# adthoms/dcora

Hardware: AMD Instinct MI355X
Metric: RBCD iterations/sec, sphere2500 5-agent split (higher is better)
Workload: dtype f64

## Files before the change

dcora_amd/__init__.py:

```python
import ctypes as C
import gzip
import os
import shutil
import tempfile

import numpy as np

from . import capi
from .capi import DcoraError, Dims, ROptParams, ROptResult, RbcdOptions, F, unF, check

__all__ = ["QuadraticProblem", "QuadraticOptimizer", "ROptParameters", "Dataset", "Csr", "RbcdSession", "RaRbcdSession", "DcoraError",
           "build_Q_pgo", "dual_certificate", "is_psd", "min_eig", "fast_verification", "manifold_project",
           "device_count"]


def device_count():
    return capi.lib().dcora_device_count()


class Csr:

    def __init__(self, n, rp, ci, v):
        self.n = int(n)
        self.rp = np.ascontiguousarray(rp, dtype=np.int32)
# ... 217 lines not shown
        nrm = C.c_double()
        check(capi.lib().dcora_problem_riegrad(self.h, F(Y), out.ctypes.data_as(C.c_void_p), C.byref(nrm)))
        return unF(out, self.r, self.k)

    def RieGradNorm(self, Y):
        nrm = C.c_double()
        check(capi.lib().dcora_problem_riegrad(self.h, F(Y), None, C.byref(nrm)))
        return nrm.value

    def HessVec(self, Y, V):
        out = self._out()
        check(capi.lib().dcora_problem_hessvec(self.h, F(Y), F(V), out))
        return unF(out, self.r, self.k)

    def HessVecSolverForm(self, Y, V):
        out = self._out()
        dots = np.zeros(2)
        check(capi.lib().dcora_debug_hessvec_solver_form(self.h, F(Y), F(V), out, dots))
        return unF(out, self.r, self.k), dots

    def PreCondition(self, Y, V):
        out = self._out()
        check(capi.lib().dcora_problem_precondition(self.h, F(Y), F(V), out))
        return unF(out, self.r, self.k)

    def Retract(self, Y, V):
        out = self._out()
        check(capi.lib().dcora_problem_retract(self.h, F(Y), F(V), out))
        return unF(out, self.r, self.k)

    def projectToTangentSpace(self, Y, V):
        out = self._out()
        check(capi.lib().dcora_problem_tangent_project(self.h, F(Y), F(V), out))
        return unF(out, self.r, self.k)

    def escapeSaddle(self, Xopt, theta, v, gradient_tolerance=1e-6, preconditioned_gradient_tolerance=1e-6,
                     isSecondOrder=False):
        out = self._out()
        ok = C.c_int()
        check(capi.lib().dcora_problem_escape_saddle(self.h, F(Xopt), float(theta),
                                                     np.ascontiguousarray(v, np.float64), gradient_tolerance,
                                                     preconditioned_gradient_tolerance, int(isSecondOrder), out,
                                                     C.byref(ok)))
        return (unF(out, self.r, self.k) if ok.value else None)

    def time_qapply(self, reps=100):
        ms, by = C.c_double(), C.c_double()
        check(capi.lib().dcora_problem_time_qapply(self.h, reps, C.byref(ms), C.byref(by)))
        return ms.value, by.value


def _time_precond(self, reps=100):
    ms, by = C.c_double(), C.c_double()
    check(capi.lib().dcora_problem_time_precond(self.h, reps, C.byref(ms), C.byref(by)))
    return ms.value, by.value


QuadraticProblem.time_precond = _time_precond


def _precond_info(self):
    info = np.zeros(5)
    check(capi.lib().dcora_problem_precond_info(self.h, info))
    return {"kind": {0: "none", 1: "dense", 2: "sparse"}[int(info[0])], "launches": int(info[1]),
            "nnzL": int(info[2]), "setup_ms": float(info[3]), "stored_doubles_per_apply": float(info[4])}


QuadraticProblem.precond_info = _precond_info


def _qapply_info(self):
    info = np.zeros(4)
    check(capi.lib().dcora_problem_qapply_info(self.h, info))
    return {"kernel": "k_spmm_bsrq" if info[0] else "k_spmm", "nnz": int(info[1]), "blocks": int(info[2]),
            "stored_matrix_bytes": float(info[3])}


QuadraticProblem.qapply_info = _qapply_info


def _solver_info(self):
    info = np.zeros(2)
    check(capi.lib().dcora_problem_solver_info(self.h, info))
    return {"tcg": {0: "three launches", 1: "two launches", 2: "one launch per run"}[int(info[0])]}


QuadraticProblem.solver_info = _solver_info


def time_qapply_rotating(problems, reps=60):
    arr = (C.c_void_p * len(problems))(*[getattr(p.h, 'value', p.h) for p in problems])
    ms = C.c_double()
    check(capi.lib().dcora_problem_time_qapply_rotating(arr, len(problems), reps, C.byref(ms)))
    return ms.value


def precond_cache_info():
    v = np.zeros(4)
    check(capi.lib().dcora_precond_cache_info(v))
    return {"hits": int(v[0]), "misses": int(v[1]), "entries": int(v[2]), "device_bytes": float(v[3])}


def precond_cache_clear():
    check(capi.lib().dcora_precond_cache_clear())


class QuadraticOptimizer:

    def __init__(self, problem, params=None):
        self.problem = problem
        self.params = params or ROptParameters()
        self.result = ROptResult()

    def optimize(self, Y):
        out = np.zeros(self.problem.r * self.problem.k)
        check(capi.lib().dcora_optimizer_optimize(self.problem.h, C.byref(self.params.c), F(Y), out,
                                                  C.byref(self.result)))
        return unF(out, self.problem.r, self.problem.k)

    def getOptResult(self):
        return self.result.as_dict()


def manifold_project(r, d, n, M, l=0, b=0, device=0, layout=0):
    dims = Dims(r, d, n, l, b, layout)
    k = (d + 1) * n + l + b
    out = np.zeros(r * k)
    check(capi.lib().dcora_manifold_project(C.byref(dims), F(M), out, device))
    return unF(out, r, k)


def dual_certificate(r, d, n, X, Q, l=0, b=0, device=0, layout=0):
    dims = Dims(r, d, n, l, b, layout)
    h = C.c_void_p()
    check(capi.lib().dcora_cert_dual_matrix(C.byref(dims), F(X), Q.rp, Q.ci, Q.v, device, C.byref(h)))
    return Csr(*capi.take_csr(h))


def is_psd(S, block=1):
    out = C.c_int()
    check(capi.lib().dcora_cert_is_psd(S.n, S.rp, S.ci, S.v, block, C.byref(out)))
    return bool(out.value)


def cert_prepare(Q, d, n, l=0, b=0, block=1, device=0, layout=0):
    dims = Dims(1, d, n, l, b, layout)
    check(capi.lib().dcora_cert_prepare(C.byref(dims), Q.rp, Q.ci, block, device))


def is_psd_device(S, block=1, device=0, info=False):
    out = C.c_int()
    i6 = np.zeros(8)
    check(capi.lib().dcora_cert_is_psd_device(S.n, S.rp, S.ci, S.v, block, device, C.byref(out), i6))
    if info:
        return bool(out.value), {"symbolic_ms": i6[0], "numeric_ms": i6[1], "arena_bytes": i6[2], "flops": i6[3],
                                 "levels": int(i6[4]), "launches": int(i6[5]), "logdet": i6[6],
                                 "lookup_ms": i6[7]}
    return bool(out.value)


def chol_host_selftest(S, block=1):
    out, res = C.c_int(), C.c_double()
    i4 = np.zeros(4)
    check(capi.lib().dcora_chol_host_selftest(S.n, S.rp, S.ci, S.v, block, C.byref(out), C.byref(res), i4))
    return bool(out.value), res.value, {"pieces": int(i4[0]), "levels": int(i4[1]), "arena": int(i4[2]),
                                        "flops": i4[3]}

# ... 383 lines not shown
```

dcora_amd/capi.py:

```python
import ctypes as C
import os
import subprocess

import numpy as np

_HERE = os.path.dirname(os.path.abspath(__file__))
LIB_PATH = os.path.join(_HERE, "lib", "libdcora_hip.so")
HEADER_PATH = os.path.join(os.path.dirname(_HERE), "include", "dcora_hip.h")


class DcoraError(RuntimeError):
    def __init__(self, status, msg):
        super().__init__("dcora status %d: %s" % (status, msg))
        self.status = status


class Dims(C.Structure):
    _fields_ = [("r", C.c_int), ("d", C.c_int), ("n", C.c_int), ("l", C.c_int), ("b", C.c_int), ("layout", C.c_int)]


LAYOUT_AUTO, LAYOUT_SE, LAYOUT_RA = 0, 1, 2


class ROptParams(C.Structure):
# ... 59 lines not shown
    "dcora_cert_dual_matrix": (C.c_int, [C.POINTER(Dims), _dp, _ip, _ip, _dp, C.c_int, C.POINTER(_vp)]),
    "dcora_cert_is_psd": (C.c_int, [C.c_int, _ip, _ip, _dp, C.c_int, _PI]),
    "dcora_cert_is_psd_device": (C.c_int, [C.c_int, _ip, _ip, _dp, C.c_int, C.c_int, _PI, _dp]),
    "dcora_chol_host_selftest": (C.c_int, [C.c_int, _ip, _ip, _dp, C.c_int, _PI, _PD, _dp]),
    "dcora_chol_cache_clear": (C.c_int, []),
    "dcora_cert_min_eig": (C.c_int, [C.c_int, _ip, _ip, _dp, C.c_int, C.c_double, C.c_int, C.c_ulonglong, C.c_int,
                                     _PD, _dp, C.POINTER(C.c_long)]),
    "dcora_cert_fast_verification": (C.c_int, [C.c_int, _ip, _ip, _dp, C.c_double, C.c_int, C.c_int, _PI, _PD, _dp,
                                               _PD]),
    "dcora_cert_lambda_min_certified": (C.c_int, [C.c_int, _ip, _ip, _dp, C.c_double, C.c_int, C.c_int, _PD, _PI]),
    "dcora_cert_suboptimality_gap": (C.c_int, [C.POINTER(Dims), _dp, C.c_double, _PD, _PD]),
    "dcora_dataset_load_g2o": (C.c_int, [C.c_char_p, C.POINTER(_vp)]),
    "dcora_dataset_create": (C.c_int, [C.c_int, C.c_int, C.c_int, _ip, _dp, C.POINTER(_vp)]),
    "dcora_dataset_info": (C.c_int, [_vp, _PI, _PI, _PI]),
    "dcora_dataset_copy": (C.c_int, [_vp, _ip, _dp]),
    "dcora_dataset_destroy": (C.c_int, [_vp]),
    "dcora_dataset_chordal_init": (C.c_int, [_vp, _dp]),
    "dcora_dataset_chordal_init_device": (C.c_int, [_vp, C.c_int, _dp]),
    "dcora_graph_build_Q_pgo": (C.c_int, [C.c_int, C.c_int, C.c_int, C.c_int, _ip, _dp, C.POINTER(_vp)]),
    "dcora_radataset_load_pyfg": (C.c_int, [C.c_char_p, C.POINTER(_vp)]),
    "dcora_radataset_info": (C.c_int, [_vp, _ip]),
    "dcora_radataset_create": (C.c_int, [C.c_int] * 5 + [_vp, _vp, C.c_int, _vp, _vp, C.c_int, _vp, _vp, _vp, C.POINTER(_vp)]),
    "dcora_radataset_copy": (C.c_int, [_vp] * 7),
    "dcora_radataset_ground_truth": (C.c_int, [_vp, _dp]),
    "dcora_radataset_build_Q": (C.c_int, [_vp, C.POINTER(_vp)]),
    "dcora_radataset_odometry_init": (C.c_int, [_vp, C.c_ulonglong, _dp]),
    "dcora_radataset_ownership": (C.c_int, [_vp, _vp, _vp, _vp]),
    "dcora_radataset_agent_columns": (C.c_int, [_vp, C.c_int, _ip, _vp, _PI]),
    "dcora_graph_extract_agent_blocks": (C.c_int, [C.c_int, _ip, _ip, _dp, C.c_int, _ip, C.POINTER(_vp),
                                                   C.POINTER(_vp)]),
    "dcora_radataset_destroy": (C.c_int, [_vp]),
    "dcora_graph_precond_regularization": (C.c_int, [C.c_int, _ip, _ip, _dp, C.c_int, _PD]),
    "dcora_rbcd_options_default": (None, [C.POINTER(RbcdOptions)]),
    "dcora_rbcd_create": (C.c_int, [_vp, C.POINTER(RbcdOptions), C.POINTER(_vp)]),
    "dcora_rbcd_destroy": (C.c_int, [_vp]),
    "dcora_rbcd_set_X": (C.c_int, [_vp, _dp]),
    "dcora_rbcd_get_X": (C.c_int, [_vp, _dp]),
    "dcora_rbcd_iterate": (C.c_int, [_vp, C.c_int, _PD, _PD, _vp, _PI]),
    "dcora_rbcd_run": (C.c_int, [_vp, C.c_int, C.c_double, _PI, _vp, _vp, _vp]),
    "dcora_rbcd_iterate_set": (C.c_int, [_vp, _ip, C.c_int, C.c_int]),
    "dcora_rbcd_set_acceleration": (C.c_int, [_vp, C.c_int]),
    "dcora_rbcd_agent_colours": (C.c_int, [_vp, _ip, _PI]),
    "dcora_rbcd_evaluate": (C.c_int, [_vp, _PD, _PD, _vp, _PI]),
    "dcora_rbcd_agent_iterate": (C.c_int, [_vp, C.c_int, C.c_int]),
    "dcora_rbcd_agent_get_X": (C.c_int, [_vp, C.c_int, _dp]),
    "dcora_rbcd_agent_set_X": (C.c_int, [_vp, C.c_int, _dp]),
    "dcora_rbcd_agent_update_neighbor": (C.c_int, [_vp, C.c_int, C.c_int, C.c_int, _ip, _dp, C.c_int]),
    "dcora_rbcd_agent_last_skipped": (C.c_int, [_vp, C.c_int, _PI]),
    "dcora_rbcd_agent_info": (C.c_int, [_vp, C.c_int, _PI, _PI, _PI]),
    "dcora_rbcd_last_result": (C.c_int, [_vp, C.POINTER(ROptResult)]),
    "dcora_rbcd_profile_tcg_runs": (C.c_int, [_vp, C.c_int]),
    "dcora_rbcd_profile_tcg_read": (C.c_int, [_vp, _dp]),
    "dcora_rbcd_X_device_ptr": (C.c_int, [_vp, C.POINTER(_vp)]),
    "dcora_rbcd_public_count": (C.c_int, [_vp, C.c_int, _PI]),
    "dcora_rbcd_public_indices": (C.c_int, [_vp, C.c_int, _ip]),
    "dcora_rbcd_pack_public_dev": (C.c_int, [_vp, C.c_int, _vp]),
    "dcora_rbcd_unpack_public_dev": (C.c_int, [_vp, C.c_int, _vp]),
    "dcora_rbcd_phase_nonselected": (C.c_int, [_vp, C.c_int]),
    "dcora_rbcd_phase_selected": (C.c_int, [_vp, C.c_int]),
    "dcora_rbcd_phase_evaluate_dev": (C.c_int, [_vp, _vp]),
    "dcora_rbcd_synchronize": (C.c_int, [_vp]),
    "dcora_exchange_create": (C.c_int, [_vp, C.c_char_p, C.POINTER(_vp)]),
    "dcora_exchange_destroy": (C.c_int, [_vp]),
    "dcora_exchange_create_ra": (C.c_int, [_vp, C.c_char_p, C.POINTER(_vp)]),
    "dcora_exchange_info": (C.c_int, [_vp, _dp]),
    "dcora_exchange_link_report": (C.c_int, [_vp, _dp]),
    "dcora_exchange_post": (C.c_int, [_vp, _ip, C.c_int]),
    "dcora_exchange_wait": (C.c_int, [_vp, _ip, C.c_int]),
    "dcora_exchange_evaluate": (C.c_int, [_vp, _PD, _PD, _vp, _PI]),
    "dcora_exchange_rbcd_iterate": (C.c_int, [_vp, C.c_int, _PD, _PD, _vp, _PI]),
    "dcora_exchange_rbcd_tick": (C.c_int, [_vp, _ip, C.c_int, C.c_int]),
    "dcora_exchange_set_X": (C.c_int, [_vp, _dp]),
    "dcora_exchange_gather_X": (C.c_int, [_vp, _dp]),
    "dcora_exchange_barrier": (C.c_int, [_vp]),
    "dcora_exchange_all_ready": (C.c_int, [_vp, C.c_int, _PI]),
    "dcora_exchange_certify": (C.c_int, [_vp, C.c_int, _vp, _vp, _vp, C.c_double, _PI, _PD, _PD, _dp,
                                         C.POINTER(C.c_longlong), _PI]),
    "dcora_exchange_host_selftest": (C.c_int, [C.c_char_p, C.c_int, C.c_int, C.c_int, C.c_int, _PD]),
    "dcora_debug_exchange_leave_stale": (C.c_int, [C.c_char_p, C.c_int, C.c_int]),
    "dcora_debug_exchange_probe_fault": (C.c_int, [C.c_int]),
    "dcora_cert_prepare": (C.c_int, [C.POINTER(Dims), _ip, _ip, C.c_int, C.c_int]),
    "dcora_debug_tcg_run_fault": (C.c_int, [C.c_int]),
    "dcora_debug_tcg_run_fault_at": (C.c_int, [C.c_int, C.c_int]),
    "dcora_problem_solver_info": (C.c_int, [_vp, _dp]),
    "dcora_ra_rbcd_create": (C.c_int, [_vp, C.POINTER(RbcdOptions), C.POINTER(_vp)]),
    "dcora_ra_rbcd_destroy": (C.c_int, [_vp]),
    "dcora_ra_rbcd_info": (C.c_int, [_vp, _PI, _vp]),
    "dcora_ra_rbcd_set_X": (C.c_int, [_vp, _dp]),
    "dcora_ra_rbcd_get_X": (C.c_int, [_vp, _dp]),
    "dcora_ra_rbcd_iterate": (C.c_int, [_vp, C.c_int, _PD, _PD, _vp, _PI]),
    "dcora_ra_rbcd_evaluate": (C.c_int, [_vp, _PD, _PD, _vp, _PI]),
    "dcora_ra_rbcd_run": (C.c_int, [_vp, C.c_int, C.c_double, _PI, _vp, _vp, _vp]),
    "dcora_ra_rbcd_last_result": (C.c_int, [_vp, C.POINTER(ROptResult)]),
    "dcora_problem_time_qapply": (C.c_int, [_vp, C.c_int, _PD, _PD]),
    "dcora_problem_time_qapply_rotating": (C.c_int, [C.POINTER(_vp), C.c_int, C.c_int, _PD]),
    "dcora_problem_qapply_info": (C.c_int, [_vp, _dp]),
    "dcora_problem_time_precond": (C.c_int, [_vp, C.c_int, _PD, _PD]),
    "dcora_problem_precond_info": (C.c_int, [_vp, _dp]),
    "dcora_precond_cache_info": (C.c_int, [_dp]),
    "dcora_precond_cache_clear": (C.c_int, []),
    "dcora_robust_params_default": (None, [C.POINTER(RobustParams)]),
    "dcora_robust_weights": (C.c_int, [C.POINTER(RobustParams), C.c_int, C.c_int, _dp, _dp]),
    "dcora_chi2inv": (C.c_int, [C.c_double, C.c_int, _PD]),
    "dcora_robust_error_threshold_at_quantile": (C.c_int, [C.c_double, C.c_int, _PD]),
    "dcora_robust_single_rotation_averaging": (C.c_int, [C.c_int, C.c_int, _dp, _vp, C.c_double, _dp, _ip]),
    "dcora_robust_single_pose_averaging": (C.c_int, [C.c_int, C.c_int, _dp, _dp, _vp, _vp, C.c_double, _dp, _dp, _ip]),
    "dcora_agent_neighbor_transforms": (C.c_int, [C.c_int, C.c_int, _ip, _dp, _dp, _dp, _dp, _dp]),
    "dcora_agent_robust_neighbor_transform": (C.c_int, [C.c_int, C.c_int, _dp, C.c_int, C.c_int, _dp, _PI, _PI]),
    "dcora_log_trajectory": (C.c_int, [C.c_char_p, C.c_int, C.c_int, _dp]),
    "dcora_fixed_stiefel_variable": (C.c_int, [C.c_int, C.c_int, _dp]),
    "dcora_agent_initialize_in_global_frame": (C.c_int, [C.POINTER(Dims), _dp, _dp, _dp, _dp]),
    "dcora_measurement_errors": (C.c_int, [_vp, C.c_int, _dp, _dp, C.c_int]),
    "dcora_solve_pgo": (C.c_int, [_vp, C.POINTER(ROptParams), _vp, _dp, C.POINTER(ROptResult), C.c_int]),
    "dcora_solve_robust_pgo": (C.c_int, [_vp, C.POINTER(ROptParams), C.POINTER(RobustParams), _vp, _vp, _dp, _vp,
                                         C.c_int]),
    "dcora_round_align_trajectory": (C.c_int, [C.POINTER(Dims), _dp, _vp, C.c_int, _dp, _vp, _vp, C.c_int]),
    "dcora_round_project_solution_raslam": (C.c_int, [C.POINTER(Dims), _dp, _dp, C.c_int]),
}

_lib = None


def lib():
    global _lib
    if _lib is None:
        if not os.path.exists(LIB_PATH):
            raise DcoraError(-1, "libdcora_hip.so is not built (run __graft_entry__.build()); there is no fallback")
        L = C.CDLL(LIB_PATH)
        for name, (res, args) in SIGNATURES.items():
            fn = getattr(L, name)
            fn.restype = res
            fn.argtypes = args
        _lib = L
    return _lib


def check(status):
    if status != 0:
        raise DcoraError(status, lib().dcora_last_error().decode() or lib().dcora_status_string(status).decode())


def F(a):
    return np.ascontiguousarray(np.asarray(a, dtype=np.float64).T).reshape(-1)


def unF(flat, rows, cols):
    return np.asarray(flat).reshape(cols, rows).T.copy()


def take_csr(h):
    L = lib()
    n, nnz = C.c_int(), C.c_int()
    check(L.dcora_csr_info(h, C.byref(n), C.byref(nnz)))
    rp = np.zeros(n.value + 1, np.int32)
    ci = np.zeros(max(nnz.value, 1), np.int32)
    v = np.zeros(max(nnz.value, 1), np.float64)
    check(L.dcora_csr_copy(h, rp, ci, v))
    L.dcora_csr_destroy(h)
    return n.value, rp, ci[:nnz.value].copy(), v[:nnz.value].copy()
```

dcora_amd/csrc/capi.hip:

```cpp
#include <cstdio>
#include <cstring>
#include <new>

#include "../../include/dcora_hip.h"
#include "cert.h"
#include "device_chol.h"
#include "device_problem.h"
#include "host_graph.h"
#include "ra_rbcd.h"
#include "rbcd.h"
#include "precond_cache.h"
#include "exchange.h"
#include "host_robust.h"
#include "robust.h"
#include "round.h"

namespace dcora {
const std::string &get_last_error();
}
using namespace dcora;

struct dcora_problem_s {
  DeviceProblem p;
};
// ... 147 lines not shown
}
int dcora_manifold_project(const dcora_dims *dims, const double *M, double *out, int device) {
  if (!dims || !M || !out) return bad("null argument");
  if (!layout_ok(dims)) return bad("dims: layout SE needs l = b = 0");
  int ndev = 0;
  if (hipGetDeviceCount(&ndev) != hipSuccess || ndev <= 0) {
    set_last_error("no HIP device available: libdcora_hip has no CPU fallback");
    return DCORA_ERR_NO_DEVICE;
  }
  DCORA_HIP(hipSetDevice(device));
  const ManiDesc m = make_mani(*dims);
  const size_t N = (size_t)m.r * m.k;
  DevBuf<double> a, b;
  DCORA_HIP(a.alloc(N));
  DCORA_HIP(b.alloc(N));
  DCORA_HIP(hipMemcpy(a.p, M, N * sizeof(double), hipMemcpyHostToDevice));
  launch_polar(nullptr, m, 1.0, a.p, 0.0, nullptr, 0.0, nullptr, b.p);
  DCORA_HIP(hipDeviceSynchronize());
  DCORA_HIP(hipMemcpy(out, b.p, N * sizeof(double), hipMemcpyDeviceToHost));
  return DCORA_OK;
}
int dcora_optimizer_optimize(dcora_problem_t p, const dcora_ropt_params *params, const double *X0, double *Xout,
                             dcora_ropt_result *result) {
  if (!p || !params || !X0 || !Xout) return bad("null argument");
  DCORA_TRY
  return p->p.optimize(*params, X0, Xout, result);
  DCORA_CATCH
}
int dcora_problem_time_qapply(dcora_problem_t p, int reps, double *avg_ms, double *bytes) {
  return p ? p->p.time_qapply(reps, avg_ms, bytes) : bad("null");
}

int dcora_problem_time_qapply_rotating(const dcora_problem_t *ps, int count, int reps, double *avg_ms) {
  if (!ps || count < 1 || !avg_ms) return bad("null");
  for (int i = 0; i < count; ++i)
    if (!ps[i]) return bad("null problem");
  DCORA_TRY
  DeviceProblem &P0 = ps[0]->p;
  DCORA_HIP(hipSetDevice(P0.device));
  std::vector<hipStream_t> keep(count);
  for (int i = 0; i < count; ++i) {
    DCORA_HIP(hipStreamSynchronize(ps[i]->p.st));
    keep[i] = ps[i]->p.st;
    ps[i]->p.st = P0.st;
  }
  hipEvent_t e0, e1;
  DCORA_HIP(hipEventCreate(&e0));
  DCORA_HIP(hipEventCreate(&e1));
  for (int i = 0; i < count; ++i) ps[i]->p.enqueue_egrad(ps[i]->p.X0.p, ps[i]->p.EG0.p, nullptr);
  DCORA_HIP(hipEventRecord(e0, P0.st));
  for (int i = 0; i < reps; ++i) {
    DeviceProblem &P = ps[i % count]->p;
    P.enqueue_egrad(P.X0.p, P.EG0.p, nullptr);
  }
  DCORA_HIP(hipEventRecord(e1, P0.st));
  DCORA_HIP(hipEventSynchronize(e1));
  float ms = 0;
  DCORA_HIP(hipEventElapsedTime(&ms, e0, e1));
  (void)hipEventDestroy(e0);
  (void)hipEventDestroy(e1);
  for (int i = 0; i < count; ++i) ps[i]->p.st = keep[i];
  *avg_ms = (double)ms / reps;
  return DCORA_OK;
  DCORA_CATCH
}
int dcora_problem_qapply_info(dcora_problem_t p, double *info) {
  if (!p || !info) return bad("null");
  const DeviceProblem &P = p->p;
  info[0] = P.has_bsr ? 1 : 0;
  info[1] = (double)P.Q.nnz;
  info[2] = P.has_bsr ? (double)P.Qb.nblocks : 0.0;
  info[3] = P.has_bsr ? P.Qb.nblocks * (8.0 * (P.m.d + 1) * (P.m.d + 1) + 4.0) + 4.0 * (P.m.n + 1)
                      : 12.0 * P.Q.nnz + 4.0 * (P.m.k + 1);
  return DCORA_OK;
}

int dcora_problem_solver_info(dcora_problem_t p, double *info) {
  if (!p || !info) return bad("null");
  const DeviceProblem &P = p->p;
  info[0] = !P.use_pc() ? 0 : (P.tcg_run_ok ? 2 : 1);
  return DCORA_OK;
}
int dcora_debug_tcg_run_fault(int runs) {
  g_tcg_run_fault_skip.store(0);
  g_tcg_run_fault.store(runs < 0 ? 0 : runs);
  return DCORA_OK;
}
int dcora_debug_tcg_run_fault_at(int skip, int runs) {
  g_tcg_run_fault_skip.store(skip < 0 ? 0 : skip);
  g_tcg_run_fault.store(runs < 0 ? 0 : runs);
  return DCORA_OK;
}
int dcora_problem_time_precond(dcora_problem_t p, int reps, double *avg_ms, double *bytes) {
  return p ? p->p.time_precond(reps, avg_ms, bytes) : bad("null");
}
int dcora_problem_precond_info(dcora_problem_t p, double *info) {
  if (!p || !info) return bad("null");
  const DeviceProblem &P = p->p;
  info[0] = !P.has_precond ? 0 : (P.sparse_precond ? 2 : 1);
  info[1] = !P.has_precond ? 0 : (P.sparse_precond ? P.sp.launches() : 1);
  info[2] = (double)P.precond_nnzL;
  info[3] = P.precond_setup_ms;
  info[4] = !P.has_precond ? 0 : (P.sparse_precond ? P.sp.weights_per_apply : (double)P.m.k * P.m.k);
  return DCORA_OK;
}

extern "C" int dcora_debug_sparse_weights_digest(dcora_problem_t p, double *out4) {
  if (!p || !out4) return bad("null");
  const DeviceProblem &P = p->p;
  if (!P.sparse_precond || !P.sp.im) return bad("the problem has no sparse preconditioner");
  const DevBuf<double> &v = P.sp.im->vals;
  std::vector<double> h(v.n);
  DCORA_HIP(hipSetDevice(P.device));
  DCORA_HIP(hipMemcpy(h.data(), v.p, v.n * sizeof(double), hipMemcpyDeviceToHost));
  long double s0 = 0, s1 = 0, s2 = 0;
  for (size_t i = 0; i < h.size(); ++i) {
    s0 += h[i];
    s1 += std::fabs(h[i]);
    s2 += h[i] * (double)(i % 97 + 1);
  }
  out4[0] = (double)h.size();
  out4[1] = (double)s0;
  out4[2] = (double)s1;
  out4[3] = (double)s2;
  return DCORA_OK;
}

namespace {
double tridiag_largest(const std::vector<double> &a, const std::vector<double> &b, int m) {
  double lo = a[0], hi = a[0];
  for (int i = 0; i < m; ++i) {
    const double rad = (i > 0 ? std::fabs(b[i - 1]) : 0.0) + (i + 1 < m ? std::fabs(b[i]) : 0.0);
    lo = std::min(lo, a[i] - rad);
    hi = std::max(hi, a[i] + rad);
  }
  auto count_below = [&](double x) {
    int c = 0;
    double d = a[0] - x;
    if (d < 0) ++c;
    for (int i = 1; i < m; ++i) {
      if (d == 0) d = 1e-300;
      d = a[i] - x - b[i - 1] * b[i - 1] / d;
      if (d < 0) ++c;
    }
    return c;
  };
  for (int it = 0; it < 200 && hi - lo > 1e-15 * std::max(std::fabs(hi), std::fabs(lo)); ++it) {
    const double mid = 0.5 * (lo + hi);
    if (count_below(mid) >= m) hi = mid; else lo = mid;
  }
  return 0.5 * (lo + hi);
}
}
int dcora_cert_lambda_min_certified(int k, const int *rp, const int *ci, const double *v, double eta, int block,
                                    int max_iterations, double *lambda_min, int *iterations) {
  if (!rp || !ci || !v || !lambda_min) return bad("null argument");
  DCORA_TRY
  const HostCsr S = view_csr(k, rp, ci, v);
  SparseChol chol;
  if (!chol.factor(csr_shift_diag(S, eta), block)) {
    set_last_error("lambda_min_certified: S + eta I is not positive definite (the certificate was not accepted)");
    return DCORA_ERR_NOT_PD;
  }
  const int mmax = std::max(2, std::min(max_iterations, k));
  std::vector<std::vector<double>> V;
  std::vector<double> alpha, beta, w((size_t)k);
  std::vector<double> q((size_t)k);
  uint64_t sdd = 0x9E3779B97F4A7C15ull;
  double n2 = 0;
  for (int i = 0; i < k; ++i) {
    sdd = sdd * 6364136223846793005ull + 1442695040888963407ull;
// ... 1404 lines not shown
```

dcora_amd/csrc/device_problem.hip:

```cpp
#include <atomic>

#include "device_problem.h"
#include "env.h"
#include "device_chol.h"
#include "precond_cache.h"

#include <algorithm>
#include <chrono>
#include <cmath>
#include <cstdio>
#include <cstdlib>
#include <cstring>
#include <map>
#include <mutex>
#include <thread>

namespace dcora {

static thread_local std::string g_last_error;
void set_last_error(const std::string &s) { g_last_error = s; }
const std::string &get_last_error() { return g_last_error; }
int hip_fail(hipError_t e, const char *what, const char *file, int line) {
  char buf[512];
  std::snprintf(buf, sizeof buf, "HIP error %d (%s) at %s:%d in %s", (int)e, hipGetErrorString(e), file, line, what);
// ... 147 lines not shown
    set_last_error("Q dimension does not match (d+1) n + l + b");
    return DCORA_ERR_BAD_ARG;
  }
  device = device_;
  int ndev = 0;
  hipError_t e = hipGetDeviceCount(&ndev);
  if (e != hipSuccess || ndev <= 0) {
    set_last_error("no HIP device available: libdcora_hip has no CPU fallback");
    return DCORA_ERR_NO_DEVICE;
  }
  DCORA_HIP(hipSetDevice(device));
  if (shared) {
    st = shared;
    own_stream = false;
  } else {
    const int rcs = stream_acquire(device, &st);
    if (rcs) return rcs;
    own_stream = true;
  }
  lap("stream");
  int rc = Q.upload(Qh);
  if (rc) return rc;
  lap("Q upload");
  const bool want_bsr = m.n >= 8192;
  if (m.se && m.r <= 8 && m.n > 0 && want_bsr && !env::generic_solver()) {
    rc = Qb.upload(bsr_from_csr(Qh, m.d + 1));
    if (rc) return rc;
    has_bsr = true;
  }
  const size_t N = (size_t)nelem();
  const size_t NS = (size_t)m.n * m.d * m.d + m.l + 1;
  fused = fused_supported(m) && Qh.nnz() > 0 && !env::generic_solver();
  group = group_supported(m) && !env::generic_solver();
  {
    struct Slot {
      DevBuf<double> *b;
      size_t n;
    };
    std::vector<Slot> slots;
    for (DevBuf<double> *b : {&G, &X0, &X1, &EG0, &EG1, &RG0, &RG1, &delta, &eta, &Heta, &res, &z, &Hd, &W, &Zt})
      slots.push_back({b, N});
    slots.push_back({&delta2, N});
    if (fused) {
      slots.push_back({&res2, N});
      slots.push_back({&Zpart, (size_t)fused_nsplit(m) * N});
    }
    slots.push_back({&S0, NS});
    slots.push_back({&S1, NS});
    for (DevBuf<double> *b : {&pB, &pC, &p1, &p2, &p3}) slots.push_back({b, (size_t)4 * kMaxPartials});
    slots.push_back({&pA, 2 * (size_t)kBsrMaxGrid});
    slots.push_back({&scal, 64});
    auto pad = [](size_t n) { return (n + 31) & ~(size_t)31; };
    size_t total = 0;
    for (const Slot &sl : slots) total += pad(sl.n);
    DCORA_HIP(arena.alloc(total));
    DCORA_HIP(hipMemsetAsync(arena.p, 0, total * sizeof(double), st));
    size_t off = 0;
    for (const Slot &sl : slots) {
      sl.b->borrow(arena.p + off, sl.n);
      off += pad(sl.n);
    }
  }
  DCORA_HIP(ctl.alloc(1));
  {
    const int rc2 = host_flags_acquire(&hf, &hf_dev, &hf_slot);
    if (rc2) return rc2;
  }
  DCORA_HIP(hipStreamSynchronize(st));
  lap("workspace");
  if (Gh) {
    rc = set_G_host(Gh);
    if (rc) return rc;
  }
  if (reg >= 0) {
    rc = build_preconditioner(Qh, reg);
    if (rc) return rc;
  }
  lap("precond");
  if (fused && has_precond && !sparse_precond && !has_bsr && Q.n_long == 0 && env::solver_tcg() >= 0) {
    hipDeviceProp_t prop;
    DCORA_HIP(hipGetDeviceProperties(&prop, device));
    tcg_run_ok = tcg_run_supported(m, ldm, prop.multiProcessorCount, tcg_run_max_rows_nnz(m, Qh.rp.data()));
    if (tcg_run_ok) {
      DCORA_HIP(tcg_sync.alloc((size_t)tcg_run_sync_words()));
      DCORA_HIP(hipMemsetAsync(tcg_sync.p, 0, sizeof(unsigned) * (size_t)tcg_run_sync_words(), st));
    }
  }
  return DCORA_OK;
}

int DeviceProblem::set_G_host(const double *Gh) {
  DCORA_HIP(hipSetDevice(device));
  if (Gh) {
    DCORA_HIP(hipMemcpy(G.p, Gh, (size_t)nelem() * sizeof(double), hipMemcpyHostToDevice));
    has_G = true;
  } else {
    DCORA_HIP(hipMemset(G.p, 0, (size_t)nelem() * sizeof(double)));
    has_G = false;
  }
  return DCORA_OK;
}

int precond_prebuild_dense(const std::vector<const HostCsr *> &Qs, double reg, int block, int device) {
  if (env::precond_mode() == 2 || env::factor_on_host() || env::precond_cache_mb() <= 0) return DCORA_OK;
  std::map<int, std::vector<size_t>> by_k;
  std::vector<PrecondKey> keys(Qs.size());
  for (size_t i = 0; i < Qs.size(); ++i) {
    const int k = Qs[i]->n;
    const bool want_sparse = env::precond_mode() ? false : (k > kDensePrecondMaxK);
    if (want_sparse || k < 1) continue;
    keys[i] = make_precond_key(*Qs[i], reg, block, device, false);
    PrecondEntry ent;
    if (precond_cache_find(keys[i], &ent, false)) continue;
    bool dup = false;
    for (size_t j : by_k[k]) dup = dup || keys[j] == keys[i];
    if (!dup) by_k[k].push_back(i);
  }
  DCORA_HIP(hipSetDevice(device));
  for (auto &grp : by_k) {
    const std::vector<size_t> &idx = grp.second;
    if (idx.size() < 2) continue;
    const auto t0 = std::chrono::steady_clock::now();
    const int k = grp.first, ldm = ((k + 127) / 128) * 128;
    std::vector<HostCsr> Ms(idx.size());
    std::vector<const HostCsr *> As;
    std::vector<std::shared_ptr<DevBuf<double>>> bufs;
    std::vector<double *> outs;
    std::vector<long> nnzL(idx.size(), 0);
    std::vector<std::thread> th;
    for (size_t q = 0; q < idx.size(); ++q) Ms[q] = csr_shift_diag(*Qs[idx[q]], reg);
    for (size_t q = 0; q < idx.size(); ++q)
      th.emplace_back([&, q] {
        CholSymbolic sym;
        chol_symbolic(Ms[q], block, &sym);
        long nz = 0;
        for (const CholPiece &pc : sym.pieces) nz += (long)pc.c * (pc.c + 1) / 2 + (long)pc.m * pc.c;
        nnzL[q] = nz;
      });
    struct Join {
      std::vector<std::thread> &t;
      ~Join() {
        for (std::thread &x : t)
          if (x.joinable()) x.join();
      }
    } join_guard{th};
    for (size_t q = 0; q < idx.size(); ++q) {
      auto buf = std::make_shared<DevBuf<double>>();
      DCORA_HIP(buf->alloc((size_t)k * ldm + 16));
      bufs.push_back(buf);
      outs.push_back(buf->p);
    }
    for (const HostCsr &M : Ms) As.push_back(&M);
    std::vector<char> pd;
    const int rc = device_dense_spd_inverse_batch(As, device, outs, ldm, &pd);
    if (rc) return rc;
    for (std::thread &x : th) x.join();
    const double ms = std::chrono::duration<double, std::milli>(std::chrono::steady_clock::now() - t0).count();
    for (size_t q = 0; q < idx.size(); ++q) {
      if (!pd[q]) continue;
      PrecondEntry ent;
      ent.ldm = ldm;
      ent.dense = bufs[q];
      ent.bytes = bufs[q]->n * sizeof(double);
      ent.build_ms = ms / (double)idx.size();
      ent.nnzL = nnzL[q];
      ent.prebuilt = true;
      precond_cache_insert(keys[idx[q]], ent);
    }
// ... 356 lines not shown
    enqueue_precond(X0.p, RG0.p, z.p);
    dir = z.p;
  }
  launch_retract(st, m, buf1(X0.p), dir, -prm.RGD_stepsize, buf1(X1.p), 0, buf1(RG0.p), nullptr, nullptr, Gate{});
  double f1 = 0, g1 = 0;
  rc = eval_dev(X1.p, &f1, &g1);
  if (rc) return rc;
  last_res_.success = 1;
  last_res_.fInit = f0;
  last_res_.gradNormInit = g0;
  last_res_.fOpt = f1;
  last_res_.gradNormOpt = g1;
  last_res_.elapsedMs = std::chrono::duration<double, std::milli>(std::chrono::steady_clock::now() - t0).count();
  last_res_.tCGStatus = TR_MAXITER;
  last_res_.outer_iterations = 1;
  last_res_.inner_iterations = 0;
  last_res_.accepted_steps = 1;
  cur_after_fetch_ = 1;
  return DCORA_OK;
}

namespace {
template <class Pred>
bool spin_until(Pred p, double timeout_s) {
  const auto t0 = std::chrono::steady_clock::now();
  unsigned it = 0;
  while (!p()) {
    if ((++it & 1023u) == 0) {
      if (std::chrono::duration<double>(std::chrono::steady_clock::now() - t0).count() > timeout_s) return false;
    }
#if defined(__x86_64__)
    __builtin_ia32_pause();
#endif
  }
  return true;
}
}

int DeviceProblem::profile_tcg_read(double *launches, double *total_us) {
  DCORA_HIP(hipSetDevice(device));
  DCORA_HIP(hipStreamSynchronize(st));
  double us = 0;
  for (size_t i = 0; i + 1 < run_events_used; i += 2) {
    float ms = 0;
    if (hipEventElapsedTime(&ms, run_events[i], run_events[i + 1]) == hipSuccess) us += 1e3 * ms;
  }
  *launches = (double)(run_events_used / 2);
  *total_us = us;
  run_events_used = 0;
  return DCORA_OK;
}

bool DeviceProblem::use_pc() const {
  const int forced = env::solver_bc();
  if (sparse_precond || !has_precond) return false;
  if (forced < 0) return false;
  if (!forced && !fused_pc_preferred(m, ldm)) return false;
  return fused_pc_ready(m, ldm);
}

struct DeviceProblem::RtrForm {
  DeviceProblem &p;
  TcgForm form;
  int &seq;
  const int solve_first;
  SolverCtl *const c;
  const CsrDev Qv;
  const BsrDev Qbv;
  const double *const Gp;
  const long N;
  const int nA, nP, nV, nPB;
  const bool sparse;
  const SpFold sfg;
  const bool hess_fused;
  const int nPG;
  const double *const Mi;
  const bool folded;
  const SpFold sf;
  const int nsl;
  const int nZ;
  const bool gf, gfb;
  unsigned *const sync_p;
  const int nsync;
  double *const dbuf[2];
  double *const rbuf[2];

  RtrForm(DeviceProblem &p_, TcgForm f, int &seq_)
      : p(p_), form(f), seq(seq_), solve_first(seq_ + 1), c(p.ctl.p), Qv(p.Q.view()),
        Qbv(p.has_bsr ? p.Qb.view() : BsrDev{}), Gp(p.has_G ? p.G.p : nullptr), N(p.nelem()), nA(p.npA()),
        nP(p.npPose()), nV(p.npVec()), nPB(fused_pose_blocks(p.m)), sparse(p.sparse_precond),
        sfg(f == TcgForm::generic && sparse ? p.sp.fold_generic() : SpFold()),
        hess_fused(f == TcgForm::generic && p.hess_one_launch()),
        nPG(sparse ? fused_update_grid(p.m) : fused_precond_grid(p.m)), Mi(sparse ? nullptr : p.Minv.p),
        folded(sparse && p.sp.foldable()), sf(folded ? p.sp.fold() : SpFold{}), nsl(sparse ? 1 : -1),
        nZ(f == TcgForm::pc || f == TcgForm::run ? fused_pc_blocks(p.m) : nPB),
        gf(f != TcgForm::generic && !p.has_bsr && p.Q.n_long == 0), gfb(f != TcgForm::generic && p.has_bsr),
        sync_p(f == TcgForm::run ? p.tcg_sync.p : nullptr), nsync(f == TcgForm::run ? tcg_run_sync_words() : 0),
        dbuf{p.delta.p, p.delta2.p}, rbuf{p.res.p, p.res2.p} {}

  bool outer_done() const { return p.hf->outer_done_seq >= solve_first; }
  bool stopped(int tcg_first) const { return p.hf->tcg_done_seq >= tcg_first || outer_done(); }
  int nAe() const { return gf ? nPB : nA; }

  int eval(int sel) {
    const auto g = [&] {
      ++seq;
      return sel ? Gate{c, seq, 1} : Gate{};
    };
    const Buf2 kNoBuf{{nullptr, nullptr}};
    if (form == TcgForm::generic) {
      p.enq_qapply(p.Xb(), sel, Gp, p.EGb(), sel, p.pA.p, g());
      launch_rgrad(p.st, p.m, p.Xb(), p.EGb(), p.RGb(), p.Sb(), sel, p.pB.p, g());
      return nP;
    }
    if (gf) return launch_fused_grad(p.st, p.m, Qv, p.Xb(), Gp, p.EGb(), p.RGb(), p.Sb(), sel, p.pA.p, p.pB.p, nullptr, g());
    if (gfb)
      return launch_fused_grad_bsr(p.st, p.m.r, p.m.d, Qbv, p.Xb(), Gp, kNoBuf, p.RGb(), p.Sb(), sel, p.pA.p, p.pB.p,
                                   nullptr, g());
    p.enq_qapply(p.Xb(), sel, Gp, p.EGb(), sel, p.pA.p, g());
    return p.enq_rgrad(p.Xb(), p.EGb(), p.RGb(), p.Sb(), sel, p.pB.p, g());
  }

  int first() {
    switch (form) {
      case TcgForm::generic: {
        launch_tcg_begin(p.st, N, p.RGb(), p.eta.p, p.Heta.p, p.res.p, c, ++seq);
        const int s = seq;
        p.enq_minv(buf1(p.res.p), p.Zt.p, nullptr, 0, Gate{c, ++seq, 1});
        launch_tangent(p.st, p.m, p.Xb(), p.Zt.p, p.z.p, p.res.p, p.p3.p, nullptr, 0, c, p.hf_dev, ++seq, 1, 0);
        return s;
      }
      case TcgForm::run: {
        const int s = launch_run();
        if (s != 0) return s;
        p.tcg_run_ok = false;
        form = TcgForm::pc;
      }
        [[fallthrough]];
      case TcgForm::pc:
        if (launch_fused_pc(p.st, p.m, p.ldm, Mi, p.RGb(), p.Xb(), nullptr, nullptr, p.eta.p, p.Heta.p, nullptr, rbuf[0],
                            p.z.p, nullptr, 0, p.p3.p, c, p.hf_dev, ++seq, 0, 1) < 0) {
          set_last_error("k_fused_pc could not be launched on this device");
          return -1;
        }
        return seq;
      case TcgForm::split:
        launch_fused_precond(p.st, p.m, p.ldm, Mi, p.RGb(), nullptr, nullptr, p.eta.p, p.Heta.p, nullptr, rbuf[0],
                             p.Zpart.p, nullptr, 0, p.p2.p, c, p.hf_dev, ++seq, 0, 1, sf);
        return seq;
    }
    return -1;
  }
  int launch_run() {
    hipEvent_t e1 = nullptr;
    if (p.profile_tcg_runs) {
      while (p.run_events.size() < p.run_events_used + 2) {
        hipEvent_t e = nullptr;
        if (hipEventCreate(&e) != hipSuccess) {
          set_last_error("hipEventCreate failed (k_tcg_run profile)");
          return -1;
        }
        p.run_events.push_back(e);
      }
      (void)hipEventRecord(p.run_events[p.run_events_used], p.st);
      e1 = p.run_events[p.run_events_used + 1];
      p.run_events_used += 2;
    }
    if (launch_tcg_run(p.st, p.m, p.ldm, Mi, Qv, p.RGb(), p.Xb(), p.Sb(), dbuf[0], dbuf[1], p.Hd.p, p.eta.p, p.Heta.p,
                       p.z.p, p.p1.p, p.p3.p, p.pC.p, p.tcg_sync.p, c, p.hf_dev, ++seq) < 0) {
      if (e1) p.run_events_used -= 2;
      return 0;
    }
    if (e1) (void)hipEventRecord(e1, p.st);
    return seq;
  }
  void rest(bool rejected) {
    if (form != TcgForm::split) return;
    if (sparse && rejected) {
      launch_fused_finish(p.st, p.m, p.Xb(), p.W.p, rbuf[0], p.z.p, nullptr, 0, p.p3.p, c, p.hf_dev, ++seq, 0, 1, 1,
                          SpFold{});
      return;
    }
    if (sparse) p.sp.apply(p.st, p.m.r, buf1(rbuf[0]), p.Zpart.p, Gate{c, ++seq, 1}, folded);
    launch_fused_finish(p.st, p.m, p.Xb(), p.Zpart.p, rbuf[0], p.z.p, nullptr, 0, p.p3.p, c, p.hf_dev, ++seq, 0, 1, nsl,
                        sf, sparse ? p.W.p : nullptr);
  }

  int replay(Buf2 R, double *Z, bool levels_only, int tcg_first) {
    const int seq_step = seq;
    bool timed = false;
    const std::function<bool()> verdict = [&]() {
      if (!spin_until([&] { return p.hf->go_seq >= seq_step || stopped(tcg_first); }, 20.0)) {
        timed = true;
        return false;
      }
      return !stopped(tcg_first);
    };
    p.sp.apply(p.st, p.m.r, R, Z, Gate{c, ++seq, 2}, levels_only, &verdict);
    if (timed) return -1;
    return stopped(tcg_first) ? 0 : 1;
  }

  int tcg_iter(int j, int max_inner, int tcg_first) {
    const int par = j & 1;
    if (form == TcgForm::generic) {
      double *const dcur = dbuf[par];
      int nP1 = nP;
      if (hess_fused) {
        nP1 = launch_spmm_dir_fix(p.st, p.m, Qv, p.Xb(), p.Sb(), p.z.p, dbuf[par ^ 1], dcur, p.Hd.p, p.p3.p, nP, p.p1.p,
                                  c, ++seq, j);
      } else {
        launch_spmm_dir(p.st, p.m.r, Qv, p.z.p, dbuf[par ^ 1], dcur, p.W.p, p.p3.p, nP, c, ++seq, j);
        launch_hessfix(p.st, p.m, p.Xb(), p.Sb(), dcur, p.W.p, p.Hd.p, p.p1.p, Gate{c, ++seq, 2});
      }
      launch_tcg_update1(p.st, N, dcur, p.Hd.p, p.eta.p, p.Heta.p, p.res.p, p.p1.p, nP1, p.p2.p, c, p.hf_dev, ++seq, j,
                         p.m.r, sfg);
      if (sfg.y) {
        const int go = replay(buf1(p.res.p), p.Zt.p, true, tcg_first);
        if (go <= 0) return go;
      } else {
        p.enq_minv(buf1(p.res.p), p.Zt.p, p.p2.p, nV, Gate{c, ++seq, 2});
      }
      launch_tangent(p.st, p.m, p.Xb(), p.Zt.p, p.z.p, p.res.p, p.p3.p, p.p2.p, nV, c, p.hf_dev, ++seq, 2, j, sfg);
      if (j == max_inner - 1) launch_tcg_update2(p.st, N, p.z.p, dcur, p.p3.p, nP, c, p.hf_dev, ++seq, j);
      return 1;
    }
    const int nP1 = launch_fused_hess(p.st, p.m, Qv, p.z.p, dbuf[par ^ 1], dbuf[par], p.Xb(), p.Sb(), p.Hd.p, p.p3.p,
                                      nZ, p.p1.p, c, ++seq, j, p.has_bsr ? &Qbv : nullptr);
    if (form == TcgForm::pc) {
      launch_fused_pc(p.st, p.m, p.ldm, Mi, p.RGb(), p.Xb(), dbuf[par], p.Hd.p, p.eta.p, p.Heta.p, rbuf[par],
                      rbuf[par ^ 1], p.z.p, p.p1.p, nP1, p.p3.p, c, p.hf_dev, ++seq, j, 0, p.pC.p);
      return 1;
    }
    launch_fused_precond(p.st, p.m, p.ldm, Mi, p.RGb(), dbuf[par], p.Hd.p, p.eta.p, p.Heta.p, rbuf[par], rbuf[par ^ 1],
                         p.Zpart.p, p.p1.p, nP1, p.p2.p, c, p.hf_dev, ++seq, j, 0, sf);
    if (sparse) {
      const int go = replay(buf1(rbuf[par ^ 1]), p.Zpart.p, folded, tcg_first);
      if (go <= 0) return go;
    }
    launch_fused_finish(p.st, p.m, p.Xb(), p.Zpart.p, rbuf[par ^ 1], p.z.p, p.p2.p, nPG, p.p3.p, c, p.hf_dev, ++seq, j,
                        0, nsl, sf);
    return 1;
  }

  int trial() {
    switch (form) {
      case TcgForm::generic:
        launch_retract(p.st, p.m, p.Xb(), p.eta.p, 1.0, p.Xb(), 1, p.RGb(), p.Heta.p, p.pC.p, Gate{c, ++seq, 1});
        return nP;
      case TcgForm::split:
        return p.enq_retract(p.Xb(), p.eta.p, 1.0, p.Xb(), 1, p.RGb(), p.Heta.p, p.pC.p, Gate{c, ++seq, 1});
      default:
        return nZ;
    }
  }
};

int DeviceProblem::rtr_dev(const dcora_ropt_params &prm, TcgForm form) {
  constexpr int kLookahead = 2;
  const auto t0 = std::chrono::steady_clock::now();
  t0_ms_ = std::chrono::duration<double, std::milli>(t0.time_since_epoch()).count();
  const bool single = (prm.RTR_iterations == 1);
  const int max_outer = single ? 12 : prm.RTR_iterations;
  const int max_inner = prm.RTR_tCG_iterations;
  if (seq_ > 1500000000) {
    DCORA_HIP(hipStreamSynchronize(st));
    hf->last_seq_done = 0;
    hf->tcg_done_seq = 0;
    hf->outer_done_seq = 0;
    hf->go_seq = 0;
    hf->reject_seq = 0;
    seq_ = 0;
  }
  int &seq = seq_;
  RtrForm f(*this, form, seq);
  CtlInit ci;
  ci.enable = 1;
  ci.tol = prm.gradnorm_tol;
  ci.Delta = prm.RTR_initial_radius;
  ci.maxDelta = single ? prm.RTR_initial_radius : 5 * prm.RTR_initial_radius;
  ci.max_outer = max_outer;
  ci.stop_on_accept = single ? 1 : 0;
  ci.max_inner = max_inner;
  auto timed_out = [&]() {
    set_last_error("rtr_dev: device did not make progress (spin timeout)");
    return DCORA_ERR_HIP;
  };
  auto first_failed = [&]() -> int {
    DCORA_HIP(hipStreamSynchronize(st));
    return DCORA_ERR_HIP;
  };
  auto time_is_up = [&]() {
    return std::chrono::duration<double>(std::chrono::steady_clock::now() - t0).count() > 5.0;
  };
  auto run_gave_up = [&]() { return f.form == TcgForm::run && hf->tcg_abort_seq >= f.solve_first; };

  int nG = f.eval(0);
  launch_rtr_init(st, pA.p, f.nAe(), pB.p, nG, f.c, hf_dev, ++seq, ci, f.sync_p, f.nsync);
  int last_pace_seq = seq;
  std::vector<int> last_seq((size_t)std::max(1, max_inner));
  int next_first_seq = time_is_up() ? 0 : f.first();
  int last_run_seq = 0;
  for (int outer = 0; outer < max_outer || (f.form == TcgForm::run && last_run_seq > 0); ++outer) {
    const bool tail = outer >= max_outer;
    if (!tail && next_first_seq < 0) return first_failed();
    const int need_seq = tail ? last_run_seq : last_pace_seq;
    if (!spin_until([&] { return hf->last_seq_done >= need_seq || f.outer_done() || run_gave_up(); }, 20.0))
      return timed_out();
    if (tail && !run_gave_up()) break;
    if (run_gave_up()) {
      DCORA_HIP(hipStreamSynchronize(st));
      const int armed = INT_MAX;
      DCORA_HIP(hipMemcpy(&f.c->outer_done_stamp, &armed, sizeof(int), hipMemcpyHostToDevice));
      if (hf->last_seq_done < last_pace_seq) --outer;
      hf->tcg_abort_seq = 0;
      tcg_run_ok = false;
      f.form = TcgForm::pc;
      next_first_seq = f.first();
      if (next_first_seq < 0) return first_failed();
    }
    if (f.outer_done()) break;
    if (next_first_seq == 0) break;
    const int tcg_first_seq = next_first_seq;
    last_run_seq = f.form == TcgForm::run ? tcg_first_seq : 0;
    f.rest(outer > 0 && hf->reject_seq == last_pace_seq);
    for (int j = 0; j < max_inner && f.form != TcgForm::run; ++j) {
      if (j >= kLookahead) {
        const int need = last_seq[j - kLookahead];
        if (!spin_until([&] { return hf->last_seq_done >= need || f.stopped(tcg_first_seq); }, 20.0))
          return timed_out();
      }
      if (hf->tcg_done_seq >= tcg_first_seq) break;
      const int go = f.tcg_iter(j, max_inner, tcg_first_seq);
      if (go < 0) return timed_out();
      if (go == 0) break;
      last_seq[j] = seq;
    }
    const int nR = f.trial();
    nG = f.eval(1);
    launch_rtr_decide(st, pA.p, f.nAe(), pB.p, nG, pC.p, nR, f.c, hf_dev, ++seq, f.sync_p, f.nsync);
    last_pace_seq = seq;
    if (outer + 1 < max_outer) next_first_seq = time_is_up() ? 0 : f.first();
  }
  pending_ = true;
  return DCORA_OK;
}

int DeviceProblem::escape_saddle(const double *Xopt, double theta, const double *v, double gtol, double pgtol,
                                 bool second_order, double *Xout, int *success) {
  if (!has_precond) {
    set_last_error("escapeSaddle needs the preconditioner");
    return DCORA_ERR_NO_PRECONDITIONER;
  }
  DCORA_HIP(hipSetDevice(device));
  const int r = m.r, k = m.k;
  std::vector<double> Xp((size_t)r * k, 0.0), Xd((size_t)r * k, 0.0);
  for (int j = 0; j < k; ++j) {
    for (int t = 0; t < r - 1; ++t) Xp[(size_t)j * r + t] = Xopt[(size_t)j * (r - 1) + t];
    Xd[(size_t)j * r + (r - 1)] = v[j];
  }
  int rc = upload(Xp.data(), X0.p, nelem());
  if (rc) return rc;
  rc = upload(Xd.data(), eta.p, nelem());
  if (rc) return rc;
  DCORA_HIP(hipStreamSynchronize(st));
  double FX = 0;
  rc = eval_dev(X0.p, &FX, nullptr);
  if (rc) return rc;
  const double alpha_min = 1e-6;
  double alpha = second_order ? std::max(16 * alpha_min, 100 * gtol / std::fabs(theta)) : 1.0;
  std::vector<double> alphas, fvals;
  *success = 0;
  while (alpha >= alpha_min) {
    launch_retract(st, m, buf1(X0.p), eta.p, alpha, buf1(X1.p), 0, buf1(RG0.p), nullptr, nullptr, Gate{});
    enqueue_egrad(X1.p, EG1.p, pA.p);
    launch_rgrad(st, m, buf1(X1.p), buf1(EG1.p), buf1(RG1.p), buf1(S1.p), 0, pB.p, Gate{});
    enqueue_precond(X1.p, RG1.p, z.p);
    launch_dot(st, nelem(), z.p, z.p, p3.p);
    launch_sum_partials(st, pA.p, npA(), 2, 2, scal.p);
    launch_sum_partials(st, pB.p, npPose(), 1, 1, scal.p + 2);
    launch_sum_partials(st, p3.p, npVec(), 1, 1, scal.p + 3);
    double s[4];
    rc = download(scal.p, s, 4);
    if (rc) return rc;
    const double FXt = 0.5 * s[0] + s[1], gn = std::sqrt(s[2]), pgn = std::sqrt(s[3]);
    alphas.push_back(alpha);
    fvals.push_back(FXt);
    if (FXt < FX && gn > gtol && pgn > pgtol) {
      *success = 1;
      return download(X1.p, Xout, nelem());
    }
    alpha /= 2;
  }
  const size_t idx = std::min_element(fvals.begin(), fvals.end()) - fvals.begin();
  if (fvals[idx] < FX) {
    launch_retract(st, m, buf1(X0.p), eta.p, alphas[idx], buf1(X1.p), 0, buf1(RG0.p), nullptr, nullptr, Gate{});
    *success = 1;
    return download(X1.p, Xout, nelem());
  }
  return DCORA_OK;
}

int DeviceProblem::time_qapply(int reps, double *avg_ms, double *bytes) {
  DCORA_HIP(hipSetDevice(device));
  hipEvent_t e0, e1;
  DCORA_HIP(hipEventCreate(&e0));
  DCORA_HIP(hipEventCreate(&e1));
  for (int i = 0; i < 3; ++i) enqueue_egrad(X0.p, EG0.p, nullptr);
  DCORA_HIP(hipEventRecord(e0, st));
  for (int i = 0; i < reps; ++i) enqueue_egrad(X0.p, EG0.p, nullptr);
  DCORA_HIP(hipEventRecord(e1, st));
  DCORA_HIP(hipEventSynchronize(e1));
  float ms = 0;
  DCORA_HIP(hipEventElapsedTime(&ms, e0, e1));
  (void)hipEventDestroy(e0);
  (void)hipEventDestroy(e1);
  *avg_ms = (double)ms / reps;
  *bytes = 12.0 * Q.nnz + 4.0 * (m.k + 1) + 16.0 * m.r * m.k + (has_G ? 8.0 * m.r * m.k : 0.0);
  return DCORA_OK;
}

}

namespace dcora {
int DeviceProblem::time_precond(int reps, double *avg_ms, double *bytes) {
// ... 49 lines not shown
```

dcora_amd/csrc/kernels.h:

```cpp
#pragma once
#include <hip/hip_runtime.h>

#include <atomic>
#include <climits>
#include <vector>

namespace dcora {

constexpr int kMaxPartials = 1024;
constexpr int kBsrMaxGrid = 4096;
constexpr int kBlock = 256;

struct ManiDesc {
  int r, d, n, l, b, k, se;
  __host__ __device__ int rot_col(int i) const { return se ? i * (d + 1) : i * d; }
  __host__ __device__ int sphere_col(int i) const { return d * n + i; }
  __host__ __device__ int num_euc() const { return se ? n : n + b; }
  __host__ __device__ int euc_col(int e) const { return se ? e * (d + 1) + d : d * n + l + e; }
};
inline ManiDesc make_mani(int r, int d, int n, int l, int b, int layout = 0) {
  ManiDesc m;
  m.r = r; m.d = d; m.n = n; m.l = l; m.b = b;
  m.se = (layout == 2) ? 0 : ((l == 0 && b == 0) ? 1 : 0);
  m.k = (d + 1) * n + l + b;
// ... 85 lines not shown
struct SpFold {
  double *y = nullptr;
  const int *in_pos = nullptr, *out_pos = nullptr;
  int h = 0;
  const int *hub_idx = nullptr;
  const double *hub_U = nullptr, *hub_x2 = nullptr;
};
void launch_tangent(hipStream_t st, const ManiDesc &m, Buf2 X, const double *V, double *out, const double *R,
                    double *partials, const double *p2, int np2, SolverCtl *ctl, HostFlags *hf, int seq,
                    int gate, int iter, SpFold sf = SpFold());
void launch_hessfix(hipStream_t st, const ManiDesc &m, Buf2 X, Buf2 Sblk, const double *V, const double *W,
                    double *HV, double *partials, Gate g);
void launch_retract(hipStream_t st, const ManiDesc &m, Buf2 X, const double *V, double alpha, Buf2 out,
                    int selOut, Buf2 grad, const double *HV, double *partials, Gate g);
void launch_polar(hipStream_t st, const ManiDesc &m, double c0, const double *A, double c1, const double *B,
                  double c2, const double *C, double *out);

void launch_nesterov(hipStream_t st, const ManiDesc &m, int mode, int restart, int skip_lo, int skip_hi, double alpha,
                     double gamma, double *X, double *V, double *Y, double *XPrev, double *Yloc,
                     const double *Xloc);

void launch_dense_apply(hipStream_t st, int r, int k, int ldm, const double *Minv, Buf2 R, double *Z,
                        const double *p2, int np2, Gate g);

int vec_grid(long nelem);
struct CtlInit {
  int enable = 0;
  double tol = 0, Delta = 0, maxDelta = 0;
  int max_outer = 0, stop_on_accept = 0, max_inner = 0;
};
void launch_rtr_init(hipStream_t st, const double *pA, int npA, const double *pB, int npB, SolverCtl *ctl,
                     HostFlags *hf, int seq, CtlInit ci = CtlInit(), unsigned *tcg_sync = nullptr, int nsync = 0);
void launch_tcg_begin(hipStream_t st, long nelem, Buf2 grad, double *eta, double *Heta, double *res,
                      SolverCtl *ctl, int seq);
void launch_tcg_update1(hipStream_t st, long nelem, const double *delta, const double *Hd, double *eta,
                        double *Heta, double *res, const double *p1, int np1, double *p2, SolverCtl *ctl,
                        HostFlags *hf, int seq, int iter, int r = 1, SpFold sf = SpFold());
void launch_tcg_update2(hipStream_t st, long nelem, const double *z, double *delta, const double *p3, int np3,
                        SolverCtl *ctl, HostFlags *hf, int seq, int iter);
void launch_rtr_decide(hipStream_t st, const double *pA, int npA, const double *pB, int npB, const double *pC,
                       int npC, SolverCtl *ctl, HostFlags *hf, int seq, unsigned *tcg_sync = nullptr, int nsync = 0);

void launch_axpby(hipStream_t st, long nelem, double a, const double *x, double b, const double *y, double *out);
void launch_sum_partials(hipStream_t st, const double *partials, int np, int stride, int count, double *out);
void launch_dot(hipStream_t st, long nelem, const double *x, const double *y, double *partials);
void launch_gather_cols(hipStream_t st, int r, int ncols, const int *src_col, const double *X, double *out);
void launch_scatter_cols(hipStream_t st, int r, int ncols, const int *dst_col, const double *in, double *X);
void launch_block_dots(hipStream_t st, int r, int nagents, const int *col_start, const double *A, const double *B,
                       double *out);

void launch_lambda_blocks(hipStream_t st, const ManiDesc &m, const double *X, const double *XQ, double *Lblk);
void launch_lanczos_proj(hipStream_t st, int n, int nv, const double *V, const double *w, double *partials);
void launch_lanczos_sub(hipStream_t st, int n, int nv, const double *V, const double *h, double *w);
constexpr int kLanczosFuseParts = 256;
void launch_lanczos_sub_sum(hipStream_t st, int n, int nv, const double *V, const double *partials, int npart,
                            double *hout, double *w, double *dotpart);
void launch_lanczos_keep(hipStream_t st, int nv, const double *h, double *hout);
constexpr double kLanczosDead = 1e-10;
void launch_lanczos_next(hipStream_t st, int n, const double *partials, int npart, double *beta_out, int *flag,
                         const double *w, double *vnext, const double *hrow, int nv);
void launch_scale_shift(hipStream_t st, int n, double shift, const double *x, double *y);
void launch_scale(hipStream_t st, int n, const double *alpha_dev_inv_sqrt ,
                  const double *w, double *out);

bool fused_supported(const ManiDesc &m);
bool group_supported(const ManiDesc &m);
int fused_pose_blocks(const ManiDesc &m);
int fused_nsplit(const ManiDesc &m);
int fused_precond_grid(const ManiDesc &m);
int fused_update_grid(const ManiDesc &m);
int launch_fused_hess(hipStream_t st, const ManiDesc &m, const CsrDev &Q, const double *z, const double *d_old,
                       double *d_new, Buf2 X, Buf2 S, double *Hd, const double *p3, int np3, double *p1,
                       SolverCtl *ctl, int seq, int iter,
                      const BsrDev *Ab = nullptr );
void launch_fused_precond(hipStream_t st, const ManiDesc &m, int ldm, const double *Minv, Buf2 grad,
                          const double *delta, const double *Hd, double *eta, double *Heta, const double *res_old,
                          double *res_new, double *Zpart, const double *p1, int np1, double *p2, SolverCtl *ctl,
                          HostFlags *hf, int seq, int iter, int first, SpFold sf = SpFold());
int fused_pc_blocks(const ManiDesc &m);
bool tcg_run_supported(const ManiDesc &m, int ldm, int cus, int max_rows_nnz);
int tcg_run_sync_words();
extern std::atomic<int> g_tcg_run_fault;
extern std::atomic<int> g_tcg_run_fault_skip;
int tcg_run_max_rows_nnz(const ManiDesc &m, const int *rowptr);
int launch_tcg_run(hipStream_t st, const ManiDesc &m, int ldm, const double *Minv, const CsrDev &Q, Buf2 grad, Buf2 X,
                   Buf2 S, double *d0, double *d1, double *Hd, double *eta, double *Heta, double *z, double *p1r,
                   double *p3, double *pC, unsigned *sync, SolverCtl *ctl, HostFlags *hf, int seq);
bool fused_pc_preferred(const ManiDesc &m, int ldm);
bool fused_pc_ready(const ManiDesc &m, int ldm);
int launch_fused_pc(hipStream_t st, const ManiDesc &m, int ldm, const double *Minv, Buf2 grad, Buf2 X,
                    const double *delta, const double *Hd, double *eta, double *Heta, const double *res_old,
                    double *res_new, double *z, const double *p1, int np1, double *p3, SolverCtl *ctl, HostFlags *hf,
                    int seq, int iter, int first, double *pC = nullptr );
void launch_fused_finish(hipStream_t st, const ManiDesc &m, Buf2 X, const double *Zpart, const double *res,
                         double *z, const double *p2, int np2, double *p3, SolverCtl *ctl, HostFlags *hf, int seq,
                         int iter, int first, int nsplit = -1 , SpFold sf = SpFold(),
                         double *zraw = nullptr );
int launch_fused_grad_bsr(hipStream_t st, int r, int d, const BsrDev &A, Buf2 X, const double *G, Buf2 EG, Buf2 RG, Buf2 S,
                          int sel, double *pA, double *pB, double *posenorm, Gate g,
                          const int *agent_start = nullptr, int agents = 0, int *wg_per_agent = nullptr);
int launch_fused_grad(hipStream_t st, const ManiDesc &m, const CsrDev &Q, Buf2 X, const double *G, Buf2 EG, Buf2 RG,
                      Buf2 Sblk, int sel, double *pA, double *pB, double *posenorm, Gate g);
int launch_g_rgrad(hipStream_t st, const ManiDesc &m, Buf2 X, Buf2 EG, Buf2 RG, Buf2 Sblk, int sel, double *partials,
                   double *posenorm, Gate g);
void launch_ctl_init(hipStream_t st, SolverCtl *c, double tol, double Delta, double maxDelta, int max_outer,
                     int stop_on_accept, int max_inner);
void launch_eval_finish(hipStream_t st, int R, const int *pose_start, const double *posenorm, const double *pA,
                        int npA, EvalOut *out_dev, int seq, double *split_scratch = nullptr, int nposes = 0,
                        const double *agent_partials = nullptr, int wg_per_agent = 0);
int eval_split_doubles();
int launch_g_retract(hipStream_t st, const ManiDesc &m, Buf2 X, const double *V, double alpha, Buf2 out, int selOut,
                     Buf2 grad, const double *HV, double *partials, Gate g);
void launch_g_nesterov(hipStream_t st, const ManiDesc &m, int mode, int restart, int skip_lo, int skip_hi,
                       double alpha, double gamma, double *X, double *V, double *Y, double *XPrev, double *Yloc,
                       Buf2 Xloc, const SolverCtl *ctl, double *inner_Yloc = nullptr);

#if defined(__HIPCC__)
template <int CTRL>
__device__ __forceinline__ double dpp_move(double v) {
  int lo = __double2loint(v), hi = __double2hiint(v);
  lo = __builtin_amdgcn_update_dpp(0, lo, CTRL, 0xF, 0xF, true);
  hi = __builtin_amdgcn_update_dpp(0, hi, CTRL, 0xF, 0xF, true);
  return __hiloint2double(hi, lo);
}
__device__ __forceinline__ double readlane_f64(double v, int lane) {
  const int lo = __builtin_amdgcn_readlane(__double2loint(v), lane);
  const int hi = __builtin_amdgcn_readlane(__double2hiint(v), lane);
  return __hiloint2double(hi, lo);
}
__device__ __forceinline__ double wave_sum_dpp(double v) {
  v += dpp_move<0xB1>(v);
  v += dpp_move<0x4E>(v);
  v += dpp_move<0x141>(v);
  v += dpp_move<0x140>(v);
  return (readlane_f64(v, 0) + readlane_f64(v, 16)) + (readlane_f64(v, 32) + readlane_f64(v, 48));
}
__device__ __forceinline__ double wave_sum(double v) { return wave_sum_dpp(v); }
__device__ __forceinline__ double block_sum(double v, double *sm) {
  v = wave_sum(v);
  const int w = threadIdx.x >> 6, nw = (blockDim.x + 63) >> 6;
  __syncthreads();
  if ((threadIdx.x & 63) == 0) sm[w] = v;
  __syncthreads();
  double t = 0;
  for (int i = 0; i < nw; ++i) t += sm[i];
  return t;
}
__device__ __forceinline__ double sum_partials(const double *p, int np, int stride, int off, double *sm) {
  double v = 0;
  for (int i = threadIdx.x; i < np; i += blockDim.x) v += p[(size_t)i * stride + off];
  return block_sum(v, sm);
}
__device__ __forceinline__ void host_store(volatile int *p, int v) {
  __hip_atomic_store(const_cast<int *>(p), v, __ATOMIC_RELAXED, __HIP_MEMORY_SCOPE_SYSTEM);
}

__device__ __forceinline__ bool gated(const SolverCtl *ctl, int seq, int gate) {
  if (ctl == nullptr || gate == 0) return false;
  if (seq > ctl->outer_done_stamp) return true;
  if (gate == 2 && seq > ctl->tcg_done_stamp) return true;
  return false;
}
struct GateWords {
  int outer, tcg;
};
__device__ __forceinline__ GateWords gate_words(const SolverCtl *ctl) {
  GateWords w{0x7fffffff, 0x7fffffff};
  if (ctl) {
    w.outer = ctl->outer_done_stamp;
    w.tcg = ctl->tcg_done_stamp;
// ... 16 lines not shown
```

dcora_amd/csrc/kernels.hip:

```cpp
#include "kernels.h"
#include "tcg_rules.h"

namespace dcora {

template <int N>
__device__ __forceinline__ void sum_partials_n(const double *const (&p)[N], const int (&np)[N], const int (&st)[N],
                                               const int (&off)[N], double *sm, double (&out)[N]) {
  double v[N];
#pragma unroll
  for (int q = 0; q < N; ++q) v[q] = ((int)threadIdx.x < np[q]) ? p[q][(size_t)threadIdx.x * st[q] + off[q]] : 0.0;
#pragma unroll
  for (int q = 0; q < N; ++q)
    for (int i = threadIdx.x + blockDim.x; i < np[q]; i += blockDim.x) v[q] += p[q][(size_t)i * st[q] + off[q]];
#pragma unroll
  for (int q = 0; q < N; ++q) v[q] = wave_sum(v[q]);
  const int w = threadIdx.x >> 6, nw = (blockDim.x + 63) >> 6;
  __syncthreads();
  if ((threadIdx.x & 63) == 0)
#pragma unroll
    for (int q = 0; q < N; ++q) sm[q * 4 + w] = v[q];
  __syncthreads();
#pragma unroll
  for (int q = 0; q < N; ++q) {
    double t = 0;
    for (int i = 0; i < nw; ++i) t += sm[q * 4 + i];
    out[q] = t;
  }
}

int vec_grid(long nelem) {
  long g = (nelem + kBlock - 1) / kBlock;
  if (g < 1) g = 1;
  if (g > kMaxPartials) g = kMaxPartials;
  return (int)g;
}

constexpr int kSpmmTile = 1536;

int spmm_grid(int nrows, int r) {
  const int RB = kBlock / r;
  long nrb = (nrows + RB - 1) / RB;
  if (nrb < 1) nrb = 1;
  if (nrb > kMaxPartials) nrb = kMaxPartials;
  return (int)nrb;
}

template <bool DOTS>
__global__ __launch_bounds__(kBlock) void k_spmm(int r, CsrDev A, Buf2 Xb, int selX, const double *__restrict__ G,
                                                 Buf2 Yb, int selY, double *__restrict__ partials, Gate g,
                                                 int main_grid) {
  if (gated(g.ctl, g.seq, g.gate)) return;
  __shared__ int s_ci[kSpmmTile];
  __shared__ double s_v[kSpmmTile];
  __shared__ double s_red[16];
  const double *__restrict__ X = pick(Xb, g.ctl, selX);
  double *__restrict__ Y = pick(Yb, g.ctl, selY);
  const int RB = kBlock / r;
  const int nrb = (A.nrows + RB - 1) / RB;
  const int lj = threadIdx.x / r, t = threadIdx.x - lj * r;
  double d0 = 0, d1 = 0;
  if ((int)blockIdx.x >= main_grid) {
    const int li = ((int)blockIdx.x - main_grid) / kLongSplit, sl = ((int)blockIdx.x - main_grid) % kLongSplit;
    const int j = A.long_rows[li];
    const int rb0 = A.rp[j], re0 = A.rp[j + 1];
    const int per = (re0 - rb0 + kLongSplit - 1) / kLongSplit;
    const int pb = rb0 + sl * per, pe = min(re0, pb + per);
    double acc = 0;
    if (lj < RB) {
      for (int p = pb + lj; p < pe; p += 8 * RB) {
        int c8[8];
        double w8[8], x8[8];
#pragma unroll
        for (int q = 0; q < 8; ++q) {
          const int pp = p + q * RB;
          const bool ok = pp < pe;
          c8[q] = A.ci[ok ? pp : rb0];
          w8[q] = ok ? A.v[pp] : 0.0;
        }
#pragma unroll
        for (int q = 0; q < 8; ++q) x8[q] = X[(size_t)c8[q] * r + t];
#pragma unroll
        for (int q = 0; q < 8; ++q) acc += w8[q] * x8[q];
      }
    }
    double *s_part = s_v;
    __shared__ int s_last;
    __syncthreads();
    s_part[threadIdx.x] = (lj < RB) ? acc : 0.0;
    __syncthreads();
    if ((int)threadIdx.x < r) {
      double y = 0;
      for (int q = 0; q < RB; ++q) y += s_part[q * r + threadIdx.x];
      __hip_atomic_store(A.long_part + ((size_t)li * kLongSplit + sl) * 16 + threadIdx.x, y, __ATOMIC_RELAXED,
                         __HIP_MEMORY_SCOPE_AGENT);
    }
    __threadfence();
    __syncthreads();
    if (threadIdx.x == 0)
      s_last = (__hip_atomic_fetch_add(A.long_cnt + li, 1, __ATOMIC_ACQ_REL, __HIP_MEMORY_SCOPE_AGENT) ==
                kLongSplit - 1);
    __syncthreads();
    if (!s_last) return;
    if (threadIdx.x == 0) __hip_atomic_store(A.long_cnt + li, 0, __ATOMIC_RELAXED, __HIP_MEMORY_SCOPE_AGENT);
    if ((int)threadIdx.x < r) {
      double y = 0;
      for (int q = 0; q < kLongSplit; ++q)
        y += __hip_atomic_load(A.long_part + ((size_t)li * kLongSplit + q) * 16 + threadIdx.x, __ATOMIC_RELAXED,
                               __HIP_MEMORY_SCOPE_AGENT);
      const size_t o = (size_t)j * r + threadIdx.x;
      if (DOTS) {
        const double x = X[o];
// ... 1333 lines not shown
  const double Delta = ctl->Delta;
  double h0 = 0, dl0 = 0, et0 = 0, he0 = 0, rs0 = 0;
  int jp0 = -1;
  const long col0 = in0 ? i0 / r : 0;
  if (in0) {
    h0 = Hd[i0];
    dl0 = delta[i0];
    et0 = eta[i0];
    he0 = Heta[i0];
    rs0 = res[i0];
    if (sf.y) jp0 = sf.in_pos[col0];
  }
  asm volatile("" ::"v"(pv), "v"(h0), "v"(dl0), "v"(et0), "v"(he0), "v"(rs0), "v"(jp0), "s"(gw.outer), "s"(gw.tcg));
  if (gated(gw, ctl, seq, 2)) return;
  for (int i = threadIdx.x + blockDim.x; i < np1; i += blockDim.x) pv += p1[i];
  const double d_Hd = block_sum(pv, s_red);
  const double alpha = tcg_alpha(z_r, d_Hd);
  const double e_Pe_new = tcg_e_Pe_new(alpha, d_Pd, e_Pe, e_Pd);
  const bool boundary = tcg_boundary(d_Hd, e_Pe_new, Delta);
  const double step = boundary ? tcg_tau(d_Pd, e_Pe, e_Pd, Delta) : alpha;
  if (!boundary && blockIdx.x == 0 && threadIdx.x == 0) host_store(&hf->go_seq, seq);
  double acc = 0;
  if (in0) {
    eta[i0] = et0 + step * dl0;
    Heta[i0] = he0 + step * h0;
    if (!boundary) {
      const double rr = rs0 + alpha * h0;
      res[i0] = rr;
      acc += rr * rr;
      if (sf.y && jp0 >= 0) sf.y[(size_t)jp0 * r + (i0 - col0 * r)] = rr;
    }
  }
  for (long i = i0 + (long)gridDim.x * kBlock; i < nelem; i += (long)gridDim.x * kBlock) {
    const double h = Hd[i];
    eta[i] += step * delta[i];
    Heta[i] += step * h;
    if (!boundary) {
      const double rr = res[i] + alpha * h;
      res[i] = rr;
      acc += rr * rr;
      if (sf.y) {
        const long col = i / r;
        const int jp = sf.in_pos[col];
        if (jp >= 0) sf.y[(size_t)jp * r + (i - col * r)] = rr;
      }
    }
  }
  const double tot = block_sum(acc, s_red);
  if (threadIdx.x == 0) p2[blockIdx.x] = tot;
  if (blockIdx.x == 0 && threadIdx.x == 0) {
    ctl->alpha = alpha;
    ctl->e_Pe_n = e_Pe_new;
    if (boundary) tcg_end_run(ctl, hf, seq, tcg_boundary_status(d_Hd), iter + 1);
  }
}

__global__ __launch_bounds__(kBlock) void k_tcg_update2(long nelem, const double *__restrict__ z,
                                                        double *__restrict__ delta, const double *__restrict__ p3,
                                                        int np3, SolverCtl *ctl, HostFlags *hf, int seq, int iter) {
  if (gated(ctl, seq, 2)) return;
  __shared__ double s_red[16];
  const int par = iter & 1;
  const double z_r_new = sum_partials(p3, np3, 1, 0, s_red);
  const double beta = tcg_beta(z_r_new, ctl->z_r[par]);
  for (long i = (long)blockIdx.x * kBlock + threadIdx.x; i < nelem; i += (long)gridDim.x * kBlock)
    delta[i] = -z[i] + beta * delta[i];
  if (blockIdx.x == 0 && threadIdx.x == 0) {
    tcg_put_dir(ctl, par ^ 1, tcg_dir_next(z_r_new, beta, ctl->alpha, ctl->d_Pd[par], ctl->e_Pd[par]), ctl->e_Pe_n);
    if (iter + 1 >= ctl->max_inner) tcg_end_run_at_cap(ctl, hf, seq, iter + 1);
    host_store(&hf->last_seq_done, seq);
  }
}

__global__ __launch_bounds__(kBlock) void k_rtr_decide(const double *pA, int npA, const double *pB, int npB,
                                                       const double *pC, int npC, SolverCtl *ctl, HostFlags *hf,
                                                       int seq, unsigned *tcg_sync, int nsync) {
  if (gated(ctl, seq, 1)) return;
  __shared__ double s_red[20];
  for (int i = threadIdx.x; i < nsync; i += kBlock) tcg_sync[i] = 0u;
  const double *const ps[5] = {pA, pA, pB, pC, pC};
  const int nps[5] = {npA, npA, npB, npC, npC}, sts[5] = {2, 2, 1, 2, 2}, offs[5] = {0, 1, 0, 0, 1};
  double sums[5];
  sum_partials_n<5>(ps, nps, sts, offs, s_red, sums);
  const double fq = sums[0], fg = sums[1], g2 = sums[2], eg = sums[3], eh = sums[4];
  if (threadIdx.x == 0) {
    const double f2 = 0.5 * fq + fg;
    const double rho = (ctl->f1 - f2) / (-(eg + 0.5 * eh));
    ctl->f2 = f2;
    ctl->rho = rho;
    if (rho > 0.75) {
      if (ctl->tcg_status == TR_NEGCURVTURE || ctl->tcg_status == TR_EXCREGION) ctl->Delta = fmin(2.0 * ctl->Delta, ctl->maxDelta);
    } else if (rho < 0.25) {
      ctl->Delta *= 0.25;
    }
    const bool accept = (rho > 0.1) && isfinite(rho);
    if (accept) {
      ctl->cur ^= 1;
      ctl->f1 = f2;
      ctl->ngf = sqrt(g2);
      ctl->accepted += 1;
      ctl->last_accepted = 1;
    } else {
      ctl->last_accepted = 0;
      host_store(&hf->reject_seq, seq);
    }
    ctl->outer_it += 1;
    if (ctl->ngf < ctl->tol || ctl->outer_it >= ctl->max_outer || (ctl->stop_on_accept && accept)) {
      ctl->outer_done_stamp = seq;
      host_store(&hf->outer_done_seq, seq);
    }
    host_store(&hf->last_seq_done, seq);
  }
}

void launch_rtr_init(hipStream_t st, const double *pA, int npA, const double *pB, int npB, SolverCtl *ctl,
                     HostFlags *hf, int seq, CtlInit ci, unsigned *tcg_sync, int nsync) {
  hipLaunchKernelGGL(k_rtr_init, dim3(1), dim3(kBlock), 0, st, pA, npA, pB, npB, ctl, hf, seq, ci, tcg_sync, nsync);
}
void launch_tcg_begin(hipStream_t st, long nelem, Buf2 grad, double *eta, double *Heta, double *res,
                      SolverCtl *ctl, int seq) {
  hipLaunchKernelGGL(k_tcg_begin, dim3(vec_grid(nelem)), dim3(kBlock), 0, st, nelem, grad, eta, Heta, res, ctl,
                     seq);
}
void launch_tcg_update1(hipStream_t st, long nelem, const double *delta, const double *Hd, double *eta,
                        double *Heta, double *res, const double *p1, int np1, double *p2, SolverCtl *ctl,
                        HostFlags *hf, int seq, int iter, int r, SpFold sf) {
  hipLaunchKernelGGL(k_tcg_update1, dim3(vec_grid(nelem)), dim3(kBlock), 0, st, nelem, delta, Hd, eta, Heta, res,
                     p1, np1, p2, ctl, hf, seq, iter, r, sf);
}
void launch_tcg_update2(hipStream_t st, long nelem, const double *z, double *delta, const double *p3, int np3,
                        SolverCtl *ctl, HostFlags *hf, int seq, int iter) {
  hipLaunchKernelGGL(k_tcg_update2, dim3(vec_grid(nelem)), dim3(kBlock), 0, st, nelem, z, delta, p3, np3, ctl, hf,
                     seq, iter);
}
void launch_rtr_decide(hipStream_t st, const double *pA, int npA, const double *pB, int npB, const double *pC,
                       int npC, SolverCtl *ctl, HostFlags *hf, int seq, unsigned *tcg_sync, int nsync) {
  hipLaunchKernelGGL(k_rtr_decide, dim3(1), dim3(kBlock), 0, st, pA, npA, pB, npB, pC, npC, ctl, hf, seq, tcg_sync,
                     nsync);
}

__global__ __launch_bounds__(kBlock) void k_axpby(long nelem, double a, const double *__restrict__ x, double b,
                                                  const double *__restrict__ y, double *__restrict__ out) {
  for (long i = (long)blockIdx.x * kBlock + threadIdx.x; i < nelem; i += (long)gridDim.x * kBlock)
    out[i] = a * x[i] + (y ? b * y[i] : 0.0);
}
void launch_axpby(hipStream_t st, long nelem, double a, const double *x, double b, const double *y, double *out) {
  hipLaunchKernelGGL(k_axpby, dim3(vec_grid(nelem)), dim3(kBlock), 0, st, nelem, a, x, b, y, out);
}

__global__ __launch_bounds__(kBlock) void k_sum_partials(const double *partials, int np, int stride, int count,
                                                         double *out) {
  __shared__ double s_red[16];
  for (int c = 0; c < count; ++c) {
    const double s = sum_partials(partials, np, stride, c, s_red);
    if (threadIdx.x == 0) out[c] = s;
  }
}
void launch_sum_partials(hipStream_t st, const double *partials, int np, int stride, int count, double *out) {
  hipLaunchKernelGGL(k_sum_partials, dim3(1), dim3(kBlock), 0, st, partials, np, stride, count, out);
}

__global__ __launch_bounds__(kBlock) void k_dot(long nelem, const double *__restrict__ x,
                                                const double *__restrict__ y, double *__restrict__ partials) {
  __shared__ double s_red[16];
  double acc = 0;
  for (long i = (long)blockIdx.x * kBlock + threadIdx.x; i < nelem; i += (long)gridDim.x * kBlock)
    acc += x[i] * y[i];
  const double t = block_sum(acc, s_red);
  if (threadIdx.x == 0) partials[blockIdx.x] = t;
}
void launch_dot(hipStream_t st, long nelem, const double *x, const double *y, double *partials) {
  hipLaunchKernelGGL(k_dot, dim3(vec_grid(nelem)), dim3(kBlock), 0, st, nelem, x, y, partials);
}

__global__ __launch_bounds__(kBlock) void k_gather_cols(int r, int ncols, const int *__restrict__ src,
                                                        const double *__restrict__ X, double *__restrict__ out) {
  const long N = (long)ncols * r;
  for (long i = (long)blockIdx.x * kBlock + threadIdx.x; i < N; i += (long)gridDim.x * kBlock) {
    const int c = (int)(i / r), t = (int)(i - (long)c * r);
    out[i] = X[(size_t)src[c] * r + t];
  }
}
__global__ __launch_bounds__(kBlock) void k_scatter_cols(int r, int ncols, const int *__restrict__ dst,
                                                         const double *__restrict__ in, double *__restrict__ X) {
  const long N = (long)ncols * r;
  for (long i = (long)blockIdx.x * kBlock + threadIdx.x; i < N; i += (long)gridDim.x * kBlock) {
    const int c = (int)(i / r), t = (int)(i - (long)c * r);
    X[(size_t)dst[c] * r + t] = in[i];
  }
}
void launch_gather_cols(hipStream_t st, int r, int ncols, const int *src_col, const double *X, double *out) {
  if (ncols <= 0) return;
  hipLaunchKernelGGL(k_gather_cols, dim3(vec_grid((long)ncols * r)), dim3(kBlock), 0, st, r, ncols, src_col, X, out);
}
void launch_scatter_cols(hipStream_t st, int r, int ncols, const int *dst_col, const double *in, double *X) {
// ... 147 lines not shown
```

dcora_amd/csrc/solver_fused.hip:

```cpp
#include <algorithm>
#include <stdexcept>
#include <atomic>
#include <type_traits>
#include <vector>
#include <cstdlib>
#include <cstring>

#include "kernels.h"
#include "tcg_rules.h"

namespace dcora {

namespace {

constexpr int GW = 8;

__device__ __forceinline__ double f_partial4_load(const double *__restrict__ p, int np) {
  const int l = (int)(threadIdx.x & 63u);
  const double a = (l < np) ? p[l] : 0.0, b = (l + 64 < np) ? p[l + 64] : 0.0;
  const double c = (l + 128 < np) ? p[l + 128] : 0.0, d = (l + 192 < np) ? p[l + 192] : 0.0;
  return (a + b) + (c + d);
}
__device__ __forceinline__ int f_partial_index(int np) { return np <= 64 ? (int)(threadIdx.x & 63u) : (int)threadIdx.x; }
__device__ __forceinline__ double f_partial_total(double v, int np, double *sm) {
// ... 265 lines not shown
  ld_row<D>(X + o, r, tt, pact, Y);
  double S[D][D];
#pragma unroll
  for (int a = 0; a < D; ++a)
#pragma unroll
    for (int b = 0; b < D; ++b) S[a][b] = (g < npose) ? Sblk[(size_t)(pose0 + g) * D * D + a + b * D] : 0.0;
  for (int i = threadIdx.x + kBlock; i < np3; i += kBlock) myp += p3[i];
  if (seq > st_o || seq > st_t) return;
  __syncthreads();
  constexpr int GB = 16;
  double ga[GB], gz[GB], gw[GB];
  const int lo0 = myb - pbeg;
  const int hi0 = min(mye, pbeg + kHessTile) - pbeg;
#pragma unroll
  for (int q = 0; q < GB; ++q) {
    const bool ok = act && (lo0 + q < hi0);
    const size_t oo = ok ? (size_t)s_ci[lo0 + q] * r + t : 0;
    gw[q] = ok ? s_v[lo0 + q] : 0.0;
    gz[q] = z[oo];
    ga[q] = (iter > 0) ? d_old[oo] : 0.0;
  }
  const double z_r_new = p3_wave ? wave_sum(myp) : f_partial_total(myp, np3, s_red);
  double beta = 0;
  if (iter > 0) beta = tcg_beta(z_r_new, c_zr);
  if (blockIdx.x == 0 && threadIdx.x == 0) {
    if (iter == 0)
      tcg_put_dir(ctl, 0, tcg_dir_start(z_r_new), 0.0);
    else
      tcg_put_dir(ctl, par, tcg_dir_next(z_r_new, beta, c_alpha, c_dPd, c_ePd), c_ePen);
  }
  double acc = 0;
#pragma unroll
  for (int q = 0; q < GB; ++q) acc += gw[q] * (beta * ga[q] - gz[q]);
  for (int base = pbeg; base < pend; base += kHessTile) {
    const int cnt = min(kHessTile, pend - base);
    if (base != pbeg) {
      __syncthreads();
      for (int i = threadIdx.x; i < cnt; i += kBlock) {
        s_ci[i] = Q.ci[base + i];
        s_v[i] = Q.v[base + i];
      }
      __syncthreads();
    }
    int lo = max(myb, base) - base;
    const int hi = min(mye, base + cnt) - base;
    if (base == pbeg) lo += GB;
    for (int p = lo; p < hi; p += 8) {
      double a8[8], b8[8], w8[8];
#pragma unroll
      for (int q = 0; q < 8; ++q) {
        const bool ok = p + q < hi;
        const size_t oo = ok ? (size_t)s_ci[p + q] * r + t : 0;
        w8[q] = ok ? s_v[p + q] : 0.0;
        b8[q] = z[oo];
        a8[q] = (iter > 0) ? d_old[oo] : 0.0;
      }
#pragma unroll
      for (int q = 0; q < 8; ++q) acc += w8[q] * (beta * a8[q] - b8[q]);
    }
  }
  if (act) {
    const double dn = (iter > 0) ? beta * d_own - z_own : -z_own;
    d_new[oown] = dn;
    s_W[e] = acc;
    s_D[e] = dn;
  }
  __syncthreads();
  Row<D> V, W;
#pragma unroll
  for (int a = 0; a < DH; ++a) {
    W.e[a] = pact ? s_W[(g * DH + a) * r + tt] : 0.0;
    V.e[a] = pact ? s_D[(g * DH + a) * r + tt] : 0.0;
  }
  row_sub_AS<D>(W, V, S);
  row_tangent<D>(Y, W);
  st_row<D>(Hd + o, r, tt, pact, W);
  double dacc = 0;
#pragma unroll
  for (int a = 0; a < DH; ++a) dacc += V.e[a] * W.e[a];
  const double tot = block_sum(dacc, s_red);
  if (threadIdx.x == 0) p1[blockIdx.x] = tot;
}

template <int D>
__global__ __launch_bounds__(kBlock) void k_fused_grad(ManiDesc m, CsrDev Q, Buf2 Xb, const double *__restrict__ G,
                                                       Buf2 EGb, Buf2 RGb, Buf2 Sb, int sel,
                                                       double *__restrict__ pA, double *__restrict__ pB,
                                                       double *__restrict__ posenorm, Gate g) {
  if (gated(g.ctl, g.seq, g.gate)) return;
  __shared__ int s_ci[kHessTile];
  __shared__ double s_v[kHessTile];
  __shared__ double s_W[kBlock], s_X[kBlock];
  __shared__ double s_red[16];
  constexpr int DH = D + 1;
  const int idx = g.ctl ? ((g.ctl->cur ^ sel) & 1) : 0;
  const double *__restrict__ X = Xb.p[idx];
  double *__restrict__ EG = EGb.p[idx];
  double *__restrict__ RG = RGb.p[idx];
  double *__restrict__ Sblk = Sb.p[idx];
  const int r = m.r;
  const int PB = fused_pb(r, DH);
  const int pose0 = blockIdx.x * PB;
  const int npose = min(PB, m.n - pose0);
  const int j0 = pose0 * DH, ncol = npose * DH, nout = ncol * r;
  const int e = threadIdx.x;
  const bool act = e < nout;
  const int lc = e / r, t = e - lc * r;
  const int j = j0 + lc;
  const int pbeg = Q.rp[j0], pend = Q.rp[j0 + ncol];
  const int myb = act ? Q.rp[j] : 0, mye = act ? Q.rp[j + 1] : 0;
  const size_t oown = (size_t)j * r + t;
  const double x_own = act ? X[oown] : 0.0;
  const double g_own = (act && G) ? G[oown] : 0.0;
  double acc = 0;
  for (int base = pbeg; base < pend; base += kHessTile) {
    const int cnt = min(kHessTile, pend - base);
    if (base != pbeg) __syncthreads();
    {
      constexpr int SU = kHessTile / kBlock;
      int ci_r[SU];
      double v_r[SU];
      const int last = max(pend - 1, 0);
#pragma unroll
      for (int u = 0; u < SU; ++u) {
        const int i = min(base + (int)threadIdx.x + u * kBlock, last);
        ci_r[u] = Q.ci[i];
        v_r[u] = Q.v[i];
      }
#pragma unroll
      for (int u = 0; u < SU; ++u) {
        const int i = threadIdx.x + u * kBlock;
        if (i < cnt) {
          s_ci[i] = ci_r[u];
          s_v[i] = v_r[u];
        }
      }
    }
    __syncthreads();
    const int lo = max(myb, base) - base, hi = min(mye, base + cnt) - base;
    for (int p = lo; p < hi; p += 8) {
      double b8[8], w8[8];
#pragma unroll
      for (int q = 0; q < 8; ++q) {
        const bool ok = p + q < hi;
        const size_t oo = ok ? (size_t)s_ci[p + q] * r + t : 0;
        w8[q] = ok ? s_v[p + q] : 0.0;
        b8[q] = X[oo];
      }
#pragma unroll
      for (int q = 0; q < 8; ++q) acc += w8[q] * b8[q];
    }
  }
  double d0 = 0, d1 = 0;
  if (act) {
    const double eg = acc + g_own;
    EG[oown] = eg;
    s_W[e] = eg;
    s_X[e] = x_own;
    d0 = acc * x_own;
    d1 = x_own * g_own;
  }
  __syncthreads();
  const int gp = threadIdx.x >> 3, tt = threadIdx.x & (GW - 1);
  const bool pact = (gp < npose) && (tt < r);
  const int pose = pose0 + gp;
  const size_t o = (size_t)pose * DH * r;
  Row<D> Y, E;
#pragma unroll
  for (int a = 0; a < DH; ++a) {
    E.e[a] = pact ? s_W[(gp * DH + a) * r + tt] : 0.0;
    Y.e[a] = pact ? s_X[(gp * DH + a) * r + tt] : 0.0;
  }
  double S[D][D];
  grp_sym_gram<D>(Y, E, S);
  if (Sblk && gp < npose && tt == 0)
#pragma unroll
    for (int a = 0; a < D; ++a)
#pragma unroll
      for (int b = 0; b < D; ++b) Sblk[(size_t)pose * D * D + a + b * D] = S[a][b];
  row_sub_AS<D>(E, Y, S);
  double pa = 0;
#pragma unroll
  for (int a = 0; a < DH; ++a) pa += E.e[a] * E.e[a];
  if (posenorm) {
    const double ps = grp_sum(pa);
    if (gp < npose && tt == 0) posenorm[pose] = ps;
  }
  st_row<D>(RG + o, r, tt, pact, E);
  const double t0 = block_sum(d0, s_red);
  const double t1 = block_sum(d1, s_red);
  const double t2 = block_sum(pact ? pa : 0.0, s_red);
  if (threadIdx.x == 0) {
    pA[2 * blockIdx.x] = t0;
    pA[2 * blockIdx.x + 1] = t1;
    pB[blockIdx.x] = t2;
  }
}

template <int D>
__global__ __launch_bounds__(kBlock) void k_fused_hess_bsr(ManiDesc m, BsrDev A, const double *__restrict__ z,
                                                           const double *__restrict__ d_old,
                                                           double *__restrict__ d_new, Buf2 Xb, Buf2 Sb,
                                                           double *__restrict__ Hd, const double *__restrict__ p3,
                                                           int np3, double *__restrict__ p1, SolverCtl *ctl, int seq,
                                                           int iter) {
  const int par = iter & 1;
  const int st_o = ctl->outer_done_stamp, st_t = ctl->tcg_done_stamp, cur = ctl->cur & 1;
  const double c_zr = ctl->z_r[par ^ 1], c_alpha = ctl->alpha, c_dPd = ctl->d_Pd[par ^ 1], c_ePd = ctl->e_Pd[par ^ 1],
               c_ePen = ctl->e_Pe_n;
  constexpr int DH = D + 1, BS = DH * DH;
  __shared__ double s_bv[kBsrTile * BS];
  __shared__ int s_bc[kBsrTile];
  __shared__ double s_red[16];
  const int r = m.r;
  const int pose0 = blockIdx.x * kPosesPerBlock;
  const int g = threadIdx.x >> 3, tt = threadIdx.x & (GW - 1);
  const int pose = pose0 + g;
  const bool inr = pose < m.n;
  const bool pact = inr && (tt < r);
  const size_t o = (size_t)pose * DH * r;
  const int pi3 = f_partial_index(np3);
  double myp = (pi3 < np3) ? p3[pi3] : 0.0;
  const int pend_pose = min(m.n, pose0 + kPosesPerBlock);
  const int bbeg = A.bp[pose0], bend = A.bp[pend_pose];
  const int myb = inr ? A.bp[pose] : 0, mye = inr ? A.bp[pose + 1] : 0;
  Row<D> Zo, Do, Y;
  ld_row<D>(z + o, r, tt, pact, Zo);
  if (iter > 0) {
    ld_row<D>(d_old + o, r, tt, pact, Do);
  } else {
#pragma unroll
    for (int a = 0; a < DH; ++a) Do.e[a] = 0.0;
  }
  const double *__restrict__ X = Xb.p[cur];
  const double *__restrict__ Sblk = Sb.p[cur];
  ld_row<D>(X + o, r, tt, pact, Y);
  double S[D][D];
#pragma unroll
  for (int a = 0; a < D; ++a)
#pragma unroll
    for (int b = 0; b < D; ++b) S[a][b] = inr ? Sblk[(size_t)pose * D * D + a + b * D] : 0.0;
  for (int i = threadIdx.x + kBlock; i < np3; i += kBlock) myp += p3[i];
  if (seq > st_o || seq > st_t) return;
  const double z_r_new = f_partial_total(myp, np3, s_red);
  double beta = 0;
  if (iter > 0) beta = tcg_beta(z_r_new, c_zr);
  if (blockIdx.x == 0 && threadIdx.x == 0) {
    if (iter == 0)
      tcg_put_dir(ctl, 0, tcg_dir_start(z_r_new), 0.0);
    else
      tcg_put_dir(ctl, par, tcg_dir_next(z_r_new, beta, c_alpha, c_dPd, c_ePd), c_ePen);
  }
  Row<D> W, V;
#pragma unroll
  for (int a = 0; a < DH; ++a) W.e[a] = 0.0;
  for (int base = bbeg; base < bend; base += kBsrTile) {
    const int cnt = min(kBsrTile, bend - base);
    __syncthreads();
    {
      constexpr int SU = (kBsrTile * BS / 2 + kBlock - 1) / kBlock;
      const double2 *__restrict__ src = reinterpret_cast<const double2 *>(A.bv + (size_t)base * BS);
      const int n2 = cnt * BS / 2;
      double2 v_r[SU];
      const int bc_r = A.bc[base + min((int)threadIdx.x, cnt - 1)];
      if ((BS & 1) == 0) {
#pragma unroll
        for (int u = 0; u < SU; ++u) v_r[u] = src[min((int)threadIdx.x + u * kBlock, n2 - 1)];
#pragma unroll
        for (int u = 0; u < SU; ++u) {
          const int i = threadIdx.x + u * kBlock;
          if (i < n2) reinterpret_cast<double2 *>(s_bv)[i] = v_r[u];
        }
      } else {
        for (int i = threadIdx.x; i < cnt * BS; i += kBlock) s_bv[i] = A.bv[(size_t)base * BS + i];
      }
      if ((int)threadIdx.x < cnt) s_bc[threadIdx.x] = bc_r;
      for (int i = threadIdx.x + kBlock; i < cnt; i += kBlock) s_bc[i] = A.bc[base + i];
    }
    __syncthreads();
    const int lo = max(myb, base) - base, hi = min(mye, base + cnt) - base;
// ... 558 lines not shown
    const int nu = (nstep + kPcNW - 1) / kPcNW;
    int u0 = 0;
    if constexpr (FIRST) {
      rows(pre, 0, nstep);
      u0 = MB;
    }
#pragma unroll 1
    for (; u0 < nu; u0 += MB) {
      double2 mm[MB][NR];
#pragma unroll
      for (int u = 0; u < MB; ++u) {
#pragma unroll
        for (int q = 0; q < NR; ++q)
          mm[u][q] = pc_ld16(rs_m, voff_l,
                             (unsigned)(((size_t)(j0 + q) * ldm + c0 + (size_t)(wave_u + kPcNW * (u0 + u)) * 128) * 8));
      }
      rows(mm, u0, nstep);
    }
  };
  chunk(0, std::true_type{});
  if constexpr (MULTI) {
#pragma unroll 1
    for (int c0 = chk; c0 < k; c0 += chk) chunk(c0, std::false_type{});
  }
#pragma unroll
  for (int q = 0; q < NR; ++q)
#pragma unroll
    for (int t = 0; t < RM; ++t) {
      const double v = row16_sum_dpp(acc[q][t]);
      if ((lane & 15) == 0) s_P[q * RM + t][wave * 4 + (lane >> 4)] = v;
    }
  {
    const double v = row16_sum_dpp(nrm2);
    if ((lane & 15) == 0) s_P[NR * RM][wave * 4 + (lane >> 4)] = v;
  }
  __syncthreads();
  if ((int)threadIdx.x <= NR * RM) {
    double v = 0;
#pragma unroll
    for (int w = 0; w < 4 * kPcNW; ++w) v += s_P[threadIdx.x][w];
    s_Z[threadIdx.x] = v;
  }
  __syncthreads();
  if (!first) {
    const double nr = sqrt(s_Z[NR * RM]);
    if (tcg_residual_done(nr, c_n0)) {
      if (blockIdx.x == 0 && threadIdx.x == 0) tcg_end_run(ctl, hf, seq, tcg_residual_status(c_n0), iter + 1);
      retract_tail();
      return;
    }
  }
  if (wave == 0) {
    Row<D> Zr, Rr;
#pragma unroll
    for (int a = 0; a < DH; ++a) {
      Zr.e[a] = pact ? s_Z[(g * DH + a) * RM + tt] : 0.0;
      Rr.e[a] = pact ? s_R[(g * DH + a) * RM + tt] : 0.0;
    }
    row_tangent<D>(Y, Zr);
    st_row<D>(z + o, r, tt, pact, Zr);
    double zacc = 0;
#pragma unroll
    for (int a = 0; a < DH; ++a) zacc += Zr.e[a] * Rr.e[a];
    const double tot = wave_sum(zacc);
    if (lane == 0) p3[blockIdx.x] = tot;
  }
  if (blockIdx.x == 0 && threadIdx.x == 0) {
    if (!first && iter + 1 >= c_max_inner) tcg_end_run_at_cap(ctl, hf, seq, iter + 1);
    host_store(&hf->last_seq_done, seq);
  }
  if (!first && iter + 1 >= c_max_inner) retract_tail();
}

constexpr int kRunShards = 32, kRunCopies = 64, kRunStride = 32;
constexpr int kRunSyncWords = (kRunShards + 1 + kRunCopies + 1) * kRunStride;
constexpr int kRunQCap = 1024;
struct TcgRunArgs {
  ManiDesc m;
  int ldm;
  const double *Minv;
  CsrDev Q;
  Buf2 grad, X, S;
  double *d0, *d1, *Hd, *eta, *Heta, *z, *p1r, *p3, *pC;
  unsigned *sync;
  SolverCtl *ctl;
  HostFlags *hf;
  int seq, pbA;
  int fault;
#ifdef DCORA_RUN_STAMPS
  long long *stamps;
#endif
};
#ifdef DCORA_RUN_STAMPS
#define RUN_STAMP(i)                                                            \
  do {                                                                          \
    if (a.stamps && blockIdx.x == 0 && threadIdx.x == 0 && (i) < 64) a.stamps[(i)] = wall_clock64(); \
  } while (0)
#else
#define RUN_STAMP(i) \
  do {                \
  } while (0)
#endif
__device__ __forceinline__ double ld_coh(const double *p) {
  return __hip_atomic_load(p, __ATOMIC_RELAXED, __HIP_MEMORY_SCOPE_AGENT);
}
__device__ __forceinline__ void st_coh(double *p, double v) {
  __hip_atomic_store(p, v, __ATOMIC_RELAXED, __HIP_MEMORY_SCOPE_AGENT);
}
__device__ __forceinline__ double2 pc_ld16_coh(__amdgpu_buffer_rsrc_t rs, unsigned voff, unsigned soff) {
  const pc_v4u v = __builtin_amdgcn_raw_buffer_load_b128(rs, voff, soff, 16);
  return __builtin_bit_cast(double2, v);
}
constexpr unsigned kRunAbortBit = 0x80000000u;
__device__ __forceinline__ bool run_grid_step(unsigned *sync, unsigned step, int *s_ok) {
  __builtin_amdgcn_s_waitcnt(0);
  __syncthreads();
  if (threadIdx.x == 0) {
    unsigned *shard = sync, *top = sync + kRunShards * kRunStride, *done = top + kRunStride,
             *abort_w = done + kRunCopies * kRunStride;
    const int i = blockIdx.x, G = gridDim.x, sh = i % kRunShards;
    const unsigned in_shard = (unsigned)((G - sh + kRunShards - 1) / kRunShards), want = step + 1;
    const unsigned shards_used = (unsigned)(G < kRunShards ? G : kRunShards);
    const unsigned a = __hip_atomic_fetch_add(shard + sh * kRunStride, 1u, __ATOMIC_RELAXED, __HIP_MEMORY_SCOPE_AGENT);
    if (a + 1 == want * in_shard) {
      const unsigned b = __hip_atomic_fetch_add(top, 1u, __ATOMIC_RELAXED, __HIP_MEMORY_SCOPE_AGENT);
      if (!(b & kRunAbortBit) && b + 1 == want * shards_used)
        for (int c = 0; c < kRunCopies; ++c)
          __hip_atomic_store(done + c * kRunStride, want, __ATOMIC_RELAXED, __HIP_MEMORY_SCOPE_AGENT);
    }
    long long t0 = wall_clock64();
    const unsigned *p = done + (i % kRunCopies) * kRunStride;
    int ok = 1;
    unsigned spins = 0;
    while (__hip_atomic_load(p, __ATOMIC_RELAXED, __HIP_MEMORY_SCOPE_AGENT) < want) {
      __builtin_amdgcn_s_sleep(1);
      if ((++spins & 63u) == 0) {
        if (__hip_atomic_load(abort_w, __ATOMIC_RELAXED, __HIP_MEMORY_SCOPE_AGENT) != 0u) {
          ok = 0;
          break;
        }
        if (wall_clock64() - t0 > 200000) {
          unsigned cur = __hip_atomic_load(top, __ATOMIC_RELAXED, __HIP_MEMORY_SCOPE_AGENT);
          bool gave_up = false;
          for (;;) {
            if (cur & kRunAbortBit) {
              gave_up = true;
              break;
            }
            if (cur >= want * shards_used) break;
            if (__hip_atomic_compare_exchange_strong(top, &cur, cur | kRunAbortBit, __ATOMIC_RELAXED, __ATOMIC_RELAXED,
                                                     __HIP_MEMORY_SCOPE_AGENT)) {
              gave_up = true;
              break;
            }
          }
          if (gave_up) {
            __hip_atomic_store(abort_w, 1u, __ATOMIC_RELAXED, __HIP_MEMORY_SCOPE_AGENT);
            ok = 0;
            break;
          }
          t0 = wall_clock64();
        }
      }
    }
    *s_ok = ok;
  }
  __syncthreads();
  return *s_ok != 0;
}

template <int D, int R, int NS>
__global__ __launch_bounds__(kPcBlock) void k_tcg_run(TcgRunArgs a) {
  constexpr int DH = D + 1, PB = 2, NR = PB * DH, RM = R;
  extern __shared__ double s_res[];
  __shared__ double s_P[NR * RM + 1][4 * kPcNW];
  __shared__ double s_Z[NR * RM + 1], s_R[NR * RM], s_W[NR * RM], s_D[NR * RM], s_H[NR * RM];
  __shared__ double s_red[16];
  __shared__ int s_ci[kRunQCap];
  __shared__ double s_v[kRunQCap];
  __shared__ int s_ok;
  SolverCtl *ctl = a.ctl;
  const int seq = a.seq;
  RUN_STAMP(0);
  const int st_o = ctl->outer_done_stamp, cur = ctl->cur & 1;
  if (seq > st_o) return;
  const double c_Delta = ctl->Delta, c_ngf = ctl->ngf;
  const int c_max_inner = ctl->max_inner;
  const ManiDesc m = a.m;
  constexpr int r = R;
  const int k = m.k, ldm = a.ldm;
  const int pose0 = blockIdx.x * PB;
  const int npose = min(PB, m.n - pose0);
  const int j0 = pose0 * DH, nrow = npose * DH;
  const int wave = threadIdx.x >> 6, lane = threadIdx.x & 63;
  const int wave_u = __builtin_amdgcn_readfirstlane(wave);
  const int e = threadIdx.x;
  const bool own = e < nrow * r;
  const size_t oown = (size_t)j0 * r + e;
  const int lc = e / r, t = e - lc * r;
  const int g = threadIdx.x >> 3, tt = threadIdx.x & (GW - 1);
  const bool pact = (g < npose) && (tt < r);
  const size_t o = (size_t)(pose0 + min(g, npose - 1)) * DH * r;
  const double *__restrict__ grad = a.grad.p[cur];
  const double *__restrict__ X = a.X.p[cur];
  const unsigned vec_bytes = (unsigned)((size_t)r * k * sizeof(double));
  const __amdgpu_buffer_rsrc_t rs_g = __builtin_amdgcn_make_buffer_rsrc(const_cast<double *>(grad), 0, vec_bytes, 0x00020000);
  const __amdgpu_buffer_rsrc_t rs_h = __builtin_amdgcn_make_buffer_rsrc(a.Hd, 0, vec_bytes, 0x00020000);
  const __amdgpu_buffer_rsrc_t rs_m = __builtin_amdgcn_make_buffer_rsrc(
      const_cast<double *>(a.Minv), 0, (unsigned)((size_t)k * ldm * sizeof(double)), 0x00020000);
  const unsigned voff_t = threadIdx.x * 16u, voff_l = (unsigned)lane * 16u;
  double2 mreg[NS][NR];
#pragma unroll
  for (int u = 0; u < NS; ++u)
#pragma unroll
    for (int q = 0; q < NR; ++q)
      mreg[u][q] = pc_ld16(rs_m, voff_l, (unsigned)(((size_t)(j0 + q) * ldm + (size_t)(wave_u + kPcNW * u) * 128) * 8));
  double2 xg[kPcSB];
#pragma unroll
  for (int u = 0; u < kPcSB; ++u) xg[u] = pc_ld16(rs_g, voff_t, (unsigned)u * kPcBlock * 16u);
  const int pbeg = a.Q.rp[j0], pend = a.Q.rp[j0 + nrow];
  for (int i = threadIdx.x; i < pend - pbeg; i += kPcBlock) {
    s_ci[i] = a.Q.ci[pbeg + i];
    s_v[i] = a.Q.v[pbeg + i];
  }
  const int myb = own ? a.Q.rp[j0 + lc] - pbeg : 0, mye = own ? a.Q.rp[j0 + lc + 1] - pbeg : 0;
  Row<D> Y;
  ld_row<D>(X + o, r, tt, pact, Y);
  double S[D][D];
  {
    const double *__restrict__ Sblk = a.S.p[cur];
#pragma unroll
    for (int aa = 0; aa < D; ++aa)
#pragma unroll
      for (int b = 0; b < D; ++b) S[aa][b] = (g < npose) ? Sblk[(size_t)(pose0 + g) * D * D + aa + b * D] : 0.0;
  }
  double o_r = own ? grad[oown] : 0.0, o_eta = 0, o_Heta = 0, o_d = 0, o_h = 0;
  const int cpad = ((k + 127) / 128) * 128;
  const long Nc = (long)k * r;
  const int npair = (int)((Nc + 1) >> 1);
  const int nstep = cpad / 128;
  double zr = 0, dPd = 0, ePe = 0, ePd = 0, alpha = 0, ePen = 0;
  const double n0 = c_ngf;
  int status = TR_MAXITER, iters_done = 0;
  unsigned gstep = 0;
  double acc[NR][RM];
  double nrm2 = 0;
  auto product = [&]() {
#pragma unroll
    for (int q = 0; q < NR; ++q)
#pragma unroll
      for (int tq = 0; tq < RM; ++tq) acc[q][tq] = 0;
#pragma unroll
    for (int u = 0; u < NS; ++u) {
      const int sidx = wave_u + kPcNW * u;
      if (sidx < nstep) {
        const double *__restrict__ xs = s_res + (size_t)(sidx * 128 + 2 * lane) * r;
        double x0[RM], x1[RM];
#pragma unroll
        for (int tq = 0; tq < RM; ++tq) {
          x0[tq] = xs[tq];
          x1[tq] = xs[r + tq];
        }
#pragma unroll
        for (int tq = 0; tq < RM; ++tq)
#pragma unroll
          for (int q = 0; q < NR; ++q) acc[q][tq] = fma(x0[tq], mreg[u][q].x, fma(x1[tq], mreg[u][q].y, acc[q][tq]));
      }
    }
#pragma unroll
    for (int q = 0; q < NR; ++q)
#pragma unroll
      for (int tq = 0; tq < RM; ++tq) {
        const double v = row16_sum_dpp(acc[q][tq]);
        if ((lane & 15) == 0) s_P[q * RM + tq][wave * 4 + (lane >> 4)] = v;
      }
    {
      const double v = row16_sum_dpp(nrm2);
      if ((lane & 15) == 0) s_P[NR * RM][wave * 4 + (lane >> 4)] = v;
    }
    __syncthreads();
    if ((int)threadIdx.x <= NR * RM) {
      double v = 0;
#pragma unroll
      for (int w = 0; w < 4 * kPcNW; ++w) v += s_P[threadIdx.x][w];
      s_Z[threadIdx.x] = v;
    }
    __syncthreads();
  };
  auto project_z = [&]() {
    if (wave == 0) {
      Row<D> Zr, Rr;
#pragma unroll
      for (int aa = 0; aa < DH; ++aa) {
        Zr.e[aa] = pact ? s_Z[(g * DH + aa) * RM + tt] : 0.0;
        Rr.e[aa] = pact ? s_R[(g * DH + aa) * RM + tt] : 0.0;
      }
      row_tangent<D>(Y, Zr);
      if (pact)
#pragma unroll
        for (int aa = 0; aa < DH; ++aa) st_coh(a.z + o + aa * r + tt, Zr.e[aa]);
      double zacc = 0;
#pragma unroll
      for (int aa = 0; aa < DH; ++aa) zacc += Zr.e[aa] * Rr.e[aa];
      const double tot = wave_sum(zacc);
      if (lane == 0) st_coh(a.p3 + blockIdx.x, tot);
    }
  };
  auto finish = [&]() {
    if (blockIdx.x == 0 && threadIdx.x == 0) {
      ctl->alpha = alpha;
      ctl->e_Pe_n = ePen;
      ctl->norm_r0 = n0;
      ctl->z_r[0] = ctl->z_r[1] = zr;
      ctl->d_Pd[0] = ctl->d_Pd[1] = dPd;
      ctl->e_Pe[0] = ctl->e_Pe[1] = ePe;
      ctl->e_Pd[0] = ctl->e_Pd[1] = ePd;
      tcg_end_run(ctl, a.hf, seq, status, iters_done);
      host_store(&a.hf->last_seq_done, seq);
    }
    __syncthreads();
    double a0 = 0, a1 = 0;
    if (own) {
      a.eta[oown] = o_eta;
      a.Heta[oown] = o_Heta;
      const double gr = grad[oown];
      a0 = o_eta * gr;
      a1 = o_eta * o_Heta;
      s_R[lc * RM + t] = o_eta;
    }
    __syncthreads();
    if (wave == 0) {
      Row<D> Yn = Y;
#pragma unroll
      for (int aa = 0; aa < DH; ++aa) Yn.e[aa] += 1.0 * (pact ? s_R[(g * DH + aa) * RM + tt] : 0.0);
      row_qf<D>(Yn);
      st_row<D>(a.X.p[cur ^ 1] + o, r, tt, pact, Yn);
    }
    const double t0 = block_sum(a0, s_red);
    const double t1 = block_sum(a1, s_red);
    if (threadIdx.x == 0) {
      a.pC[2 * blockIdx.x] = t0;
      a.pC[2 * blockIdx.x + 1] = t1;
    }
  };
  auto give_up = [&]() {
    if (threadIdx.x == 0) {
      ctl->outer_done_stamp = seq - 1;
      host_store(&a.hf->tcg_abort_seq, seq);
    }
  };
#pragma unroll
  for (int u = 0; u < kPcSB; ++u) {
    const int i = u * kPcBlock + (int)threadIdx.x;
    if (i < npair) {
      const double2 x = xg[u];
      nrm2 = fma(x.x, x.x, nrm2);
      nrm2 = fma(x.y, x.y, nrm2);
      reinterpret_cast<double2 *>(s_res)[i] = x;
    }
  }
  for (long i = 2L * npair + threadIdx.x; i < (long)cpad * r; i += kPcBlock) s_res[i] = 0.0;
  if (own) s_R[lc * RM + t] = o_r;
  __syncthreads();
  RUN_STAMP(1);
  product();
  project_z();
  RUN_STAMP(2);
  if (c_max_inner <= 0) {
    status = TR_MAXITER;
    finish();
    return;
  }
  if (a.fault && blockIdx.x == 0) return;
  if (!run_grid_step(a.sync, gstep++, &s_ok)) return give_up();
  RUN_STAMP(3);
  for (int iter = 0;; ++iter) {
    const int par = iter & 1;
    double *__restrict__ d_new = par ? a.d1 : a.d0;
    const double *__restrict__ d_old = par ? a.d0 : a.d1;
    {
      constexpr int kRunGB = 24;
      double ga[kRunGB], gz[kRunGB];
      double z_own = 0;
      if (own) {
        z_own = ld_coh(a.z + oown);
#pragma unroll
        for (int q = 0; q < kRunGB; ++q) {
          const bool ok = myb + q < mye;
          const size_t oo = ok ? (size_t)s_ci[myb + q] * r + t : 0;
          gz[q] = ld_coh(a.z + oo);
          ga[q] = (iter > 0) ? ld_coh(d_old + oo) : 0.0;
        }
      }
      const int np3 = gridDim.x;
      const int l = lane;
      const double pa = (l < np3) ? ld_coh(a.p3 + l) : 0.0, pb = (l + 64 < np3) ? ld_coh(a.p3 + l + 64) : 0.0;
      const double pcc = (l + 128 < np3) ? ld_coh(a.p3 + l + 128) : 0.0, pd = (l + 192 < np3) ? ld_coh(a.p3 + l + 192) : 0.0;
      const double z_r_new = wave_sum((pa + pb) + (pcc + pd));
      double beta = 0;
      if (iter > 0) beta = tcg_beta(z_r_new, zr);
      const TcgDir dir = iter == 0 ? tcg_dir_start(z_r_new) : tcg_dir_next(z_r_new, beta, alpha, dPd, ePd);
      zr = dir.z_r;
      ePd = dir.e_Pd;
      dPd = dir.d_Pd;
      ePe = iter == 0 ? 0.0 : ePen;
      double accw = 0, dn = 0;
      if (own) {
#pragma unroll
        for (int q = 0; q < kRunGB; ++q) {
          const double w = (myb + q < mye) ? s_v[myb + q] : 0.0;
          accw += w * (beta * ga[q] - gz[q]);
        }
        for (int p = myb + kRunGB; p < mye; p += 8) {
          double a8[8], b8[8], w8[8];
#pragma unroll
          for (int q = 0; q < 8; ++q) {
            const bool ok = p + q < mye;
            const size_t oo = ok ? (size_t)s_ci[p + q] * r + t : 0;
            w8[q] = ok ? s_v[p + q] : 0.0;
            b8[q] = ld_coh(a.z + oo);
            a8[q] = (iter > 0) ? ld_coh(d_old + oo) : 0.0;
          }
#pragma unroll
          for (int q = 0; q < 8; ++q) accw += w8[q] * (beta * a8[q] - b8[q]);
        }
        dn = (iter > 0) ? beta * o_d - z_own : -z_own;
        st_coh(d_new + oown, dn);
        o_d = dn;
        s_W[e] = accw;
        s_D[e] = dn;
      }
      __syncthreads();
      if (wave == 0) {
        Row<D> V, W;
#pragma unroll
        for (int aa = 0; aa < DH; ++aa) {
          W.e[aa] = pact ? s_W[(g * DH + aa) * r + tt] : 0.0;
          V.e[aa] = pact ? s_D[(g * DH + aa) * r + tt] : 0.0;
        }
        row_sub_AS<D>(W, V, S);
        row_tangent<D>(Y, W);
        if (pact)
#pragma unroll
          for (int aa = 0; aa < DH; ++aa) {
            st_coh(a.Hd + o + aa * r + tt, W.e[aa]);
            s_H[(g * DH + aa) * r + tt] = W.e[aa];
          }
        double dacc = 0;
#pragma unroll
        for (int aa = 0; aa < DH; ++aa) dacc += V.e[aa] * W.e[aa];
        if (!pact) dacc = 0;
        const double rs = row16_sum_dpp(dacc);
        if (lane == 0) st_coh(a.p1r + blockIdx.x, rs);
      }
      __syncthreads();
      if (own) o_h = s_H[e];
    }
    RUN_STAMP(4 + 7 * iter);
    if (!run_grid_step(a.sync, gstep++, &s_ok)) return give_up();
    RUN_STAMP(5 + 7 * iter);
    double2 xh[kPcSB];
#pragma unroll
    for (int u = 0; u < kPcSB; ++u) xh[u] = pc_ld16_coh(rs_h, voff_t, (unsigned)u * kPcBlock * 16u);
    double d_Hd;
    {
      const int rows_per = a.pbA / 2, nrows = gridDim.x, nblk = (nrows + rows_per - 1) / rows_per;
      double part = 0;
      if (lane < nblk) {
        const int b0 = lane * rows_per;
        double wsum[4] = {0, 0, 0, 0};
#pragma unroll
        for (int w = 0; w < 4; ++w) {
          double rs4[4];
#pragma unroll
          for (int q = 0; q < 4; ++q) {
            const int ri = w * 4 + q;
            rs4[q] = (ri < rows_per && b0 + ri < nrows) ? ld_coh(a.p1r + b0 + ri) : 0.0;
          }
          wsum[w] = (rs4[0] + rs4[1]) + (rs4[2] + rs4[3]);
        }
        double tsum = 0;
#pragma unroll
        for (int w = 0; w < 4; ++w) tsum += wsum[w];
        part = tsum;
      }
      d_Hd = wave_sum(part);
    }
    const double c_zr = zr, c_dPd = dPd, c_ePe = ePe, c_ePd = ePd;
    alpha = tcg_alpha(c_zr, d_Hd);
    const double e_Pe_new = tcg_e_Pe_new(alpha, c_dPd, c_ePe, c_ePd);
    const bool boundary = tcg_boundary(d_Hd, e_Pe_new, c_Delta);
    const double step = boundary ? tcg_tau(c_dPd, c_ePe, c_ePd, c_Delta) : alpha;
    ePen = e_Pe_new;
    if (own) {
      o_eta = o_eta + step * o_d;
      o_Heta = o_Heta + step * o_h;
    }
    if (boundary) {
      status = tcg_boundary_status(d_Hd);
      iters_done = iter + 1;
      finish();
      return;
    }
    if (own) {
      const double rr = fma(alpha, o_h, o_r);
      o_r = rr;
      s_R[lc * RM + t] = rr;
    }
    RUN_STAMP(6 + 7 * iter);
    nrm2 = 0;
#pragma unroll
    for (int u = 0; u < kPcSB; ++u) {
      const int i = u * kPcBlock + (int)threadIdx.x;
      if (i < npair) {
        double2 x = reinterpret_cast<double2 *>(s_res)[i];
        x.x = fma(alpha, xh[u].x, x.x);
        x.y = fma(alpha, xh[u].y, x.y);
        nrm2 = fma(x.x, x.x, nrm2);
        nrm2 = fma(x.y, x.y, nrm2);
        reinterpret_cast<double2 *>(s_res)[i] = x;
      }
    }
    __syncthreads();
    RUN_STAMP(7 + 7 * iter);
    product();
    RUN_STAMP(8 + 7 * iter);
    {
      if (tcg_residual_done(sqrt(s_Z[NR * RM]), n0)) {
        status = tcg_residual_status(n0);
        iters_done = iter + 1;
        finish();
        return;
      }
    }
    project_z();
    if (iter + 1 >= c_max_inner) {
      iters_done = iter + 1;
      finish();
      return;
    }
    RUN_STAMP(9 + 7 * iter);
    if (!run_grid_step(a.sync, gstep++, &s_ok)) return give_up();
    RUN_STAMP(10 + 7 * iter);
  }
}


template <int D>
__global__ __launch_bounds__(kBlock) void k_g_rgrad(ManiDesc m, Buf2 Xb, Buf2 EGb, Buf2 RGb, Buf2 Sb, int sel,
                                                    double *__restrict__ partials, double *__restrict__ posenorm,
                                                    Gate g) {
  if (gated(g.ctl, g.seq, g.gate)) return;
  __shared__ double s_red[16];
  constexpr int DH = D + 1;
  const int idx = g.ctl ? ((g.ctl->cur ^ sel) & 1) : 0;
  const double *__restrict__ X = Xb.p[idx];
  const double *__restrict__ EG = EGb.p[idx];
  double *__restrict__ RG = RGb.p[idx];
  double *__restrict__ Sblk = Sb.p[idx];
  const int r = m.r;
  const int t = threadIdx.x & (GW - 1);
  double acc = 0;
  for (int pose0 = blockIdx.x * kPosesPerBlock; pose0 < m.n; pose0 += gridDim.x * kPosesPerBlock) {
    const int pose = pose0 + (threadIdx.x >> 3);
    const bool active = (pose < m.n) && (t < r);
    const size_t o = (size_t)pose * DH * r;
    Row<D> Y, E;
    ld_row<D>(X + o, r, t, active, Y);
    ld_row<D>(EG + o, r, t, active, E);
    double S[D][D];
    grp_sym_gram<D>(Y, E, S);
    if (Sblk && pose < m.n && t == 0)
#pragma unroll
      for (int a = 0; a < D; ++a)
#pragma unroll
        for (int b = 0; b < D; ++b) Sblk[(size_t)pose * D * D + a + b * D] = S[a][b];
    row_sub_AS<D>(E, Y, S);
    double pa = 0;
#pragma unroll
    for (int a = 0; a < DH; ++a) pa += E.e[a] * E.e[a];
    acc += pa;
    if (posenorm) {
      const double ps = grp_sum(pa);
      if (pose < m.n && t == 0) posenorm[pose] = ps;
    }
    if (RG) st_row<D>(RG + o, r, t, active, E);
  }
  const double tot = block_sum(acc, s_red);
  if (threadIdx.x == 0 && partials) partials[blockIdx.x] = tot;
}

template <int D>
__global__ __launch_bounds__(kBlock) void k_g_retract(ManiDesc m, Buf2 Xb, const double *__restrict__ V,
                                                      double alpha, Buf2 Ob, int selOut, Buf2 gradb,
                                                      const double *__restrict__ HV, double *__restrict__ partials,
                                                      Gate g) {
  if (gated(g.ctl, g.seq, g.gate)) return;
  __shared__ double s_red[16];
  constexpr int DH = D + 1;
  const int cur = g.ctl ? (g.ctl->cur & 1) : 0;
  const double *__restrict__ X = Xb.p[cur];
  double *__restrict__ out = Ob.p[g.ctl ? ((cur ^ selOut) & 1) : 0];
  const double *__restrict__ grad = partials ? gradb.p[cur] : nullptr;
  const int r = m.r;
  const int t = threadIdx.x & (GW - 1);
  double a0 = 0, a1 = 0;
  for (int pose0 = blockIdx.x * kPosesPerBlock; pose0 < m.n; pose0 += gridDim.x * kPosesPerBlock) {
    const int pose = pose0 + (threadIdx.x >> 3);
    const bool active = (pose < m.n) && (t < r);
    const size_t o = (size_t)pose * DH * r;
    Row<D> Y, Vr;
    ld_row<D>(X + o, r, t, active, Y);
    ld_row<D>(V + o, r, t, active, Vr);
    if (partials) {
      Row<D> Gr, Hr;
      ld_row<D>(grad + o, r, t, active, Gr);
      ld_row<D>(HV + o, r, t, active, Hr);
#pragma unroll
      for (int a = 0; a < DH; ++a) {
        a0 += Vr.e[a] * Gr.e[a];
        a1 += Vr.e[a] * Hr.e[a];
      }
    }
#pragma unroll
    for (int a = 0; a < DH; ++a) Y.e[a] += alpha * Vr.e[a];
    row_qf<D>(Y);
    st_row<D>(out + o, r, t, active, Y);
// ... 520 lines not shown
  }
#undef DCORA_LAUNCH_PRECOND
}
int fused_pc_pb(const ManiDesc &m) { return m.n <= 768 ? 2 : 4; }
int fused_pc_blocks(const ManiDesc &m) {
  const int pb = fused_pc_pb(m);
  return (m.n + pb - 1) / pb;
}
constexpr int kPcLdsCap = 128 * 1024;
static int pc_chunk(const ManiDesc &m, int ldm) { return std::min((kPcLdsCap / (8 * m.r)) / 128 * 128, ldm); }
bool fused_pc_preferred(const ManiDesc &m, int ldm) {
  return m.k <= pc_chunk(m, ldm) && (long)m.r * m.k <= 2L * kPcSB * kPcBlock && m.r <= 7;
}
template <int D, int PB, int R, bool MULTI>
static int pc_launch(hipStream_t st, const ManiDesc &m, int ldm, const double *Minv, Buf2 grad, Buf2 X,
                     const double *delta, const double *Hd, double *eta, double *Heta, const double *res_old,
                     double *res_new, double *z, const double *p1, int np1, double *p3, SolverCtl *ctl, HostFlags *hf,
                     int seq, int iter, int first, double *pC, bool prepare_only) {
  static std::atomic<unsigned long long> tried{0}, ok{0};
  int dev = 0;
  if (hipGetDevice(&dev) != hipSuccess || dev < 0 || dev >= 64) return -1;
  const unsigned long long bit = 1ull << dev;
  if (!(tried.load(std::memory_order_acquire) & bit)) {
    const hipError_t e = hipFuncSetAttribute(reinterpret_cast<const void *>(&k_fused_pc<D, PB, R, MULTI>),
                                             hipFuncAttributeMaxDynamicSharedMemorySize, kPcLdsCap);
    if (e == hipSuccess)
      ok.fetch_or(bit, std::memory_order_release);
    else
      (void)hipGetLastError();
    tried.fetch_or(bit, std::memory_order_release);
  }
  const int chk = pc_chunk(m, ldm);
  const size_t lds = (size_t)chk * m.r * sizeof(double);
  if (!(ok.load(std::memory_order_acquire) & bit) && lds > 64 * 1024) return -1;
  const int grid = (m.n + PB - 1) / PB;
  if (prepare_only) return grid;
  hipLaunchKernelGGL((k_fused_pc<D, PB, R, MULTI>), dim3(grid), dim3(kPcBlock), lds, st, m, ldm, chk, Minv, grad, X,
                     delta, Hd, eta, Heta, res_old, res_new, z, p1, np1, p3, ctl, hf, seq, iter, first, pC);
  if (hipGetLastError() != hipSuccess) return -1;
  return grid;
}
static int fused_pc_dispatch(hipStream_t st, const ManiDesc &m, int ldm, const double *Minv, Buf2 grad, Buf2 X,
                             const double *delta, const double *Hd, double *eta, double *Heta, const double *res_old,
                             double *res_new, double *z, const double *p1, int np1, double *p3, SolverCtl *ctl,
                             HostFlags *hf, int seq, int iter, int first, double *pC, bool prepare_only) {
#define DCORA_PC(D_, PB_, R_, MULTI_)                                                                                \
  return pc_launch<D_, PB_, R_, MULTI_>(st, m, ldm, Minv, grad, X, delta, Hd, eta, Heta, res_old, res_new, z, p1, np1, \
                                        p3, ctl, hf, seq, iter, first, pC, prepare_only)
#define DCORA_PC_FIXED_R(D_, PB_, MULTI_)      \
  do {                                          \
    if (D_ == 3 && m.r == 3) DCORA_PC(D_, PB_, 3, MULTI_); \
    if (D_ == 3 && m.r == 4) DCORA_PC(D_, PB_, 4, MULTI_); \
    if (D_ == 3 && m.r == 5) DCORA_PC(D_, PB_, 5, MULTI_); \
    if (D_ == 3 && m.r == 6) DCORA_PC(D_, PB_, 6, MULTI_); \
    if (D_ == 3 && m.r == 7) DCORA_PC(D_, PB_, 7, MULTI_); \
  } while (0)
#define DCORA_PC_R(D_, PB_, MULTI_)             \
  do {                                          \
    DCORA_PC_FIXED_R(D_, PB_, MULTI_);          \
    DCORA_PC(D_, PB_, 0, MULTI_);               \
  } while (0)
  const int pb = fused_pc_pb(m);
  const bool multi = m.k > pc_chunk(m, ldm);
  if (m.d == 3) {
    if (pb == 2 && !multi) DCORA_PC_R(3, 2, false);
    if (pb == 2) DCORA_PC_R(3, 2, true);
    if (m.r == 3) DCORA_PC(3, 4, 3, true);
    if (m.r == 4) DCORA_PC(3, 4, 4, true);
    if (m.r == 5) DCORA_PC(3, 4, 5, true);
    if (m.r == 6) DCORA_PC(3, 4, 6, true);
    return -1;
  }
  if (pb == 2 && !multi) DCORA_PC(2, 2, 0, false);
  if (pb == 2) DCORA_PC(2, 2, 0, true);
  DCORA_PC(2, 4, 0, true);
#undef DCORA_PC_R
#undef DCORA_PC_FIXED_R
#undef DCORA_PC
}
constexpr int kRunNS = 4;
int tcg_run_sync_words() { return kRunSyncWords; }
std::atomic<int> g_tcg_run_fault{0};
std::atomic<int> g_tcg_run_fault_skip{0};
int tcg_run_max_rows_nnz(const ManiDesc &m, const int *rp) {
  const int dh = m.d + 1;
  int worst = 0;
  for (int p0 = 0; p0 < m.n; p0 += 2) {
    const int j0 = p0 * dh, j1 = std::min(m.n, p0 + 2) * dh;
    worst = std::max(worst, rp[j1] - rp[j0]);
  }
  return worst;
}
bool tcg_run_supported(const ManiDesc &m, int ldm, int cus, int max_rows_nnz) {
  if (!m.se || m.d != 3 || m.r < 4 || m.r > 6) return false;
  if (fused_pb(m.r, m.d + 1) % 2 != 0) return false;
  if (!fused_pc_preferred(m, ldm) || fused_pc_pb(m) != 2) return false;
  const int grid = (m.n + 1) / 2;
  if (grid > cus || grid > 256) return false;
  if (m.k > kRunNS * kPcNW * 128) return false;
  const int rows_per = fused_pb(m.r, m.d + 1) / 2;
  if ((grid + rows_per - 1) / rows_per > 64) return false;
  return max_rows_nnz <= kRunQCap;
}
template <int R>
static int tcg_run_launch(hipStream_t st, const TcgRunArgs &a) {
  static std::atomic<unsigned long long> tried{0}, ok{0};
  int dev = 0;
  if (hipGetDevice(&dev) != hipSuccess || dev < 0 || dev >= 64) return -1;
  const unsigned long long bit = 1ull << dev;
  if (!(tried.load(std::memory_order_acquire) & bit)) {
    const hipError_t e = hipFuncSetAttribute(reinterpret_cast<const void *>(&k_tcg_run<3, R, kRunNS>),
                                             hipFuncAttributeMaxDynamicSharedMemorySize, kPcLdsCap);
    if (e == hipSuccess)
      ok.fetch_or(bit, std::memory_order_release);
    else
      (void)hipGetLastError();
    tried.fetch_or(bit, std::memory_order_release);
  }
  const int cpad = ((a.m.k + 127) / 128) * 128;
  const size_t lds = (size_t)cpad * R * sizeof(double);
  if (!(ok.load(std::memory_order_acquire) & bit) && lds > 40 * 1024) return -1;
  const int grid = (a.m.n + 1) / 2;
  hipLaunchKernelGGL((k_tcg_run<3, R, kRunNS>), dim3(grid), dim3(kPcBlock), lds, st, a);
  if (hipGetLastError() != hipSuccess) return -1;
  return grid;
}
int launch_tcg_run(hipStream_t st, const ManiDesc &m, int ldm, const double *Minv, const CsrDev &Q, Buf2 grad, Buf2 X,
                   Buf2 S, double *d0, double *d1, double *Hd, double *eta, double *Heta, double *z, double *p1r,
                   double *p3, double *pC, unsigned *sync, SolverCtl *ctl, HostFlags *hf, int seq) {
  int fault = 0;
  bool skipped = false;
  for (int sk = g_tcg_run_fault_skip.load(); sk > 0;)
    if (g_tcg_run_fault_skip.compare_exchange_weak(sk, sk - 1)) {
      skipped = true;
      break;
    }
  for (int left = skipped ? 0 : g_tcg_run_fault.load(); left > 0;)
    if (g_tcg_run_fault.compare_exchange_weak(left, left - 1)) {
      fault = 1;
      break;
    }
  TcgRunArgs a{m, ldm, Minv, Q, grad, X, S, d0, d1, Hd, eta, Heta, z, p1r, p3, pC, sync, ctl, hf, seq,
               fused_pb(m.r, m.d + 1), fault};
#ifdef DCORA_RUN_STAMPS
  {
    static long long *buf = nullptr;
    if (!buf) (void)hipHostMalloc((void **)&buf, 64 * sizeof(long long), hipHostMallocMapped);
    static int count = 0;
    if (buf && count > 0) {
      static double acc[64];
      static int n = 0;
      long long s0 = buf[0];
      if (buf[3] > s0 && buf[5 + 7 * 3] > 0) {
        for (int i = 0; i < 40; ++i) acc[i] += (double)(buf[i] - s0) * 0.01;
        ++n;
      }
      for (int i = 0; i < 64; ++i) buf[i] = 0;
      if (n == 500) {
        fprintf(stderr, "k_tcg_run stamps (us from start, workgroup 0, mean of %d runs with >= 4 iterations):", n);
        for (int i = 0; i < 34; ++i) fprintf(stderr, " %.2f", acc[i] / n);
        fprintf(stderr, "\n");
        n = -1000000;
      }
    }
    ++count;
    a.stamps = buf;
  }
#endif
  if (m.r == 4) return tcg_run_launch<4>(st, a);
  if (m.r == 5) return tcg_run_launch<5>(st, a);
  if (m.r == 6) return tcg_run_launch<6>(st, a);
  return -1;
}
int launch_fused_pc(hipStream_t st, const ManiDesc &m, int ldm, const double *Minv, Buf2 grad, Buf2 X,
                    const double *delta, const double *Hd, double *eta, double *Heta, const double *res_old,
                    double *res_new, double *z, const double *p1, int np1, double *p3, SolverCtl *ctl, HostFlags *hf,
                    int seq, int iter, int first, double *pC) {
  return fused_pc_dispatch(st, m, ldm, Minv, grad, X, delta, Hd, eta, Heta, res_old, res_new, z, p1, np1, p3, ctl, hf,
                           seq, iter, first, pC, false);
}
bool fused_pc_ready(const ManiDesc &m, int ldm) {
  Buf2 none{};
  return fused_pc_dispatch(nullptr, m, ldm, nullptr, none, none, nullptr, nullptr, nullptr, nullptr, nullptr, nullptr,
                           nullptr, nullptr, 0, nullptr, nullptr, nullptr, 0, 0, 0, nullptr, true) >= 0;
}
void launch_fused_finish(hipStream_t st, const ManiDesc &m, Buf2 X, const double *Zpart, const double *res,
                         double *z, const double *p2, int np2, double *p3, SolverCtl *ctl, HostFlags *hf, int seq,
                         int iter, int first, int nsplit, SpFold sf, double *zraw) {
  const int grid = fused_pose_blocks(m);
  const int ns = nsplit > 0 ? nsplit : fused_nsplit(m);
  if (m.d == 3)
    hipLaunchKernelGGL(k_fused_finish<3>, dim3(grid), dim3(kBlock), 0, st, m, ns, X, Zpart, res, z, p2, np2, p3, ctl,
                       hf, seq, iter, first, sf, zraw);
  else
    hipLaunchKernelGGL(k_fused_finish<2>, dim3(grid), dim3(kBlock), 0, st, m, ns, X, Zpart, res, z, p2, np2, p3, ctl,
                       hf, seq, iter, first, sf, zraw);
}

int launch_g_rgrad(hipStream_t st, const ManiDesc &m, Buf2 X, Buf2 EG, Buf2 RG, Buf2 Sblk, int sel, double *partials,
                   double *posenorm, Gate g) {
  const int grid = group_grid(m.n);
  if (m.d == 3)
    hipLaunchKernelGGL(k_g_rgrad<3>, dim3(grid), dim3(kBlock), 0, st, m, X, EG, RG, Sblk, sel, partials, posenorm, g);
  else
    hipLaunchKernelGGL(k_g_rgrad<2>, dim3(grid), dim3(kBlock), 0, st, m, X, EG, RG, Sblk, sel, partials, posenorm, g);
  return grid;
}
int launch_fused_grad(hipStream_t st, const ManiDesc &m, const CsrDev &Q, Buf2 X, const double *G, Buf2 EG, Buf2 RG,
                      Buf2 Sblk, int sel, double *pA, double *pB, double *posenorm, Gate g) {
  const int grid = fused_pose_blocks(m);
  if (m.d == 3)
    hipLaunchKernelGGL(k_fused_grad<3>, dim3(grid), dim3(kBlock), 0, st, m, Q, X, G, EG, RG, Sblk, sel, pA, pB, posenorm,
                       g);
  else
    hipLaunchKernelGGL(k_fused_grad<2>, dim3(grid), dim3(kBlock), 0, st, m, Q, X, G, EG, RG, Sblk, sel, pA, pB, posenorm,
                       g);
  return grid;
}
int launch_g_retract(hipStream_t st, const ManiDesc &m, Buf2 X, const double *V, double alpha, Buf2 out, int selOut,
                     Buf2 grad, const double *HV, double *partials, Gate g) {
  const int grid = group_grid(m.n);
  if (m.d == 3)
    hipLaunchKernelGGL(k_g_retract<3>, dim3(grid), dim3(kBlock), 0, st, m, X, V, alpha, out, selOut, grad, HV,
                       partials, g);
  else
    hipLaunchKernelGGL(k_g_retract<2>, dim3(grid), dim3(kBlock), 0, st, m, X, V, alpha, out, selOut, grad, HV,
                       partials, g);
  return grid;
}
void launch_g_nesterov(hipStream_t st, const ManiDesc &m, int mode, int restart, int skip_lo, int skip_hi,
                       double alpha, double gamma, double *X, double *V, double *Y, double *XPrev, double *Yloc,
                       Buf2 Xloc, const SolverCtl *ctl, double *inner_Yloc) {
  GNesterovArgs a{mode, restart, skip_lo, skip_hi, alpha, gamma, X, V, Y, XPrev, Yloc, inner_Yloc, Xloc, ctl};
  const int grid = group_grid(m.n);
  if (m.d == 3)
    hipLaunchKernelGGL(k_g_nesterov<3>, dim3(grid), dim3(kBlock), 0, st, m, a);
  else
    hipLaunchKernelGGL(k_g_nesterov<2>, dim3(grid), dim3(kBlock), 0, st, m, a);
}

}
```

dcora_amd/csrc/tcg_rules.h:

```cpp
#pragma once
#include "kernels.h"

namespace dcora {

constexpr double kTcgKappa = 0.1;
constexpr double kTcgTheta = 1.0;
static_assert(kTcgTheta == 1.0, "tcg_residual_done takes |r0|^theta as |r0|");

struct TcgDir {
  double z_r, e_Pd, d_Pd;
};
__device__ __forceinline__ TcgDir tcg_dir_start(double z_r) { return TcgDir{z_r, 0.0, z_r}; }
__device__ __forceinline__ double tcg_beta(double z_r_new, double z_r_old) { return z_r_new / z_r_old; }
__device__ __forceinline__ TcgDir tcg_dir_next(double z_r_new, double beta, double alpha, double d_Pd, double e_Pd) {
  return TcgDir{z_r_new, beta * (e_Pd + alpha * d_Pd), z_r_new + beta * beta * d_Pd};
}
__device__ __forceinline__ void tcg_put_dir(SolverCtl *ctl, int slot, const TcgDir &v, const double &e_Pe) {
  ctl->z_r[slot] = v.z_r;
  ctl->e_Pd[slot] = v.e_Pd;
  ctl->d_Pd[slot] = v.d_Pd;
  ctl->e_Pe[slot] = e_Pe;
}

__device__ __forceinline__ double tcg_alpha(double z_r, double d_Hd) { return z_r / d_Hd; }
__device__ __forceinline__ double tcg_e_Pe_new(double alpha, double d_Pd, double e_Pe, double e_Pd) {
  return e_Pe + 2.0 * alpha * e_Pd + alpha * alpha * d_Pd;
}
__device__ __forceinline__ bool tcg_boundary(double d_Hd, double e_Pe_new, double Delta) {
  return (d_Hd <= 0) || (e_Pe_new >= Delta * Delta);
}
__device__ __forceinline__ double tcg_tau(double d_Pd, double e_Pe, double e_Pd, double Delta) {
  return (-e_Pd + sqrt(e_Pd * e_Pd + d_Pd * (Delta * Delta - e_Pe))) / d_Pd;
}
__device__ __forceinline__ int tcg_boundary_status(double d_Hd) { return d_Hd <= 0 ? TR_NEGCURVTURE : TR_EXCREGION; }

__device__ __forceinline__ bool tcg_residual_done(double norm_r, double norm_r0) {
  return norm_r <= norm_r0 * fmin(norm_r0, kTcgKappa);
}
__device__ __forceinline__ int tcg_residual_status(double norm_r0) { return kTcgKappa < norm_r0 ? TR_LCON : TR_SCON; }

__device__ __forceinline__ void tcg_begin_run(SolverCtl *ctl, double norm_r0) {
  ctl->norm_r0 = norm_r0;
  ctl->tcg_status = TR_MAXITER;
  ctl->tcg_iters = 0;
  ctl->tcg_done_stamp = INT_MAX;
}
__device__ __forceinline__ void tcg_end_run_at_cap(SolverCtl *ctl, HostFlags *hf, int seq, int iters) {
  ctl->tcg_iters = iters;
  ctl->inner_total += iters;
  ctl->tcg_done_stamp = seq;
  host_store(&hf->tcg_done_seq, seq);
}
__device__ __forceinline__ void tcg_end_run(SolverCtl *ctl, HostFlags *hf, int seq, int status, int iters) {
  ctl->tcg_status = status;
  tcg_end_run_at_cap(ctl, hf, seq, iters);
}

__device__ __forceinline__ void ctl_arm(SolverCtl *c, const CtlInit &ci) {
  c->f2 = c->rho = 0;
  c->Delta = ci.Delta;
  c->maxDelta = ci.maxDelta;
  c->tol = ci.tol;
  c->cur = 0;
  c->outer_it = 0;
  c->max_outer = ci.max_outer;
  c->accepted = 0;
  c->last_accepted = 0;
  c->stop_on_accept = ci.stop_on_accept;
  c->outer_done_stamp = INT_MAX;
  c->alpha = c->e_Pe_n = c->norm_r0 = 0;
  c->tcg_done_stamp = INT_MAX;
  c->tcg_status = TR_MAXITER;
  c->tcg_iters = 0;
  c->inner_total = 0;
  c->max_inner = ci.max_inner;
}

}
```

include/dcora_hip.h:

```cpp
#ifndef DCORA_HIP_H_
#define DCORA_HIP_H_

#ifdef __cplusplus
extern "C" {
#endif

typedef enum {
  DCORA_OK = 0,
  DCORA_ERR_BAD_ARG = 1,
  DCORA_ERR_NO_DEVICE = 2,
  DCORA_ERR_HIP = 3,
  DCORA_ERR_NOT_PD = 4,
  DCORA_ERR_NO_CONVERGENCE = 5,
  DCORA_ERR_NO_PRECONDITIONER = 6,
  DCORA_ERR_IO = 7,
  DCORA_ERR_UNSUPPORTED = 8,
  DCORA_ERR_EXCHANGE_LINK = 9
} dcora_status;

const char *dcora_status_string(int status);
const char *dcora_last_error(void);
int dcora_device_count(void);

enum {
  DCORA_LAYOUT_AUTO = 0,
  DCORA_LAYOUT_SE = 1,
  DCORA_LAYOUT_RA = 2
};
typedef struct {
  int r;
  int d;
  int n;
  int l;
  int b;
  int layout;
} dcora_dims;

typedef struct {
  int method;
  int verbose;
  double gradnorm_tol;
  double RGD_stepsize;
  int RGD_use_preconditioner;
  int RTR_iterations;
  int RTR_tCG_iterations;
  double RTR_initial_radius;
} dcora_ropt_params;
void dcora_ropt_params_default(dcora_ropt_params *p);

typedef struct {
  int success;
  double fInit, gradNormInit, fOpt, gradNormOpt, elapsedMs;
  int tCGStatus;
  int outer_iterations, inner_iterations, accepted_steps;
} dcora_ropt_result;

typedef struct dcora_problem_s *dcora_problem_t;

int dcora_problem_create(const dcora_dims *dims, const int *rowptr, const int *colidx, const double *vals,
                         const double *G, double precond_reg, int device, dcora_problem_t *out);
int dcora_problem_destroy(dcora_problem_t p);
int dcora_problem_set_linear_term(dcora_problem_t p, const double *G);
int dcora_problem_cost(dcora_problem_t p, const double *X, double *f);
int dcora_problem_eucgrad(dcora_problem_t p, const double *X, double *out);
int dcora_problem_riegrad(dcora_problem_t p, const double *X, double *out, double *norm);
int dcora_problem_hessvec(dcora_problem_t p, const double *X, const double *V, double *out);
int dcora_debug_hessvec_solver_form(dcora_problem_t p, const double *X, const double *V, double *out, double *dots);
int dcora_problem_solver_info(dcora_problem_t p, double *info);
int dcora_debug_tcg_run_fault(int runs);
int dcora_debug_tcg_run_fault_at(int skip, int runs);
int dcora_problem_precondition(dcora_problem_t p, const double *X, const double *V, double *out);
int dcora_problem_retract(dcora_problem_t p, const double *X, const double *V, double *out);
int dcora_problem_tangent_project(dcora_problem_t p, const double *X, const double *V, double *out);
int dcora_problem_escape_saddle(dcora_problem_t p, const double *Xopt, double theta, const double *v,
                                double gradient_tolerance, double preconditioned_gradient_tolerance,
                                int is_second_order, double *Xout, int *success);
int dcora_manifold_project(const dcora_dims *dims, const double *M, double *out, int device);

int dcora_optimizer_optimize(dcora_problem_t p, const dcora_ropt_params *params, const double *X0, double *Xout,
                             dcora_ropt_result *result);

typedef struct dcora_csr_s *dcora_csr_t;
int dcora_csr_info(dcora_csr_t m, int *n, int *nnz);
int dcora_csr_copy(dcora_csr_t m, int *rowptr, int *colidx, double *vals);
int dcora_csr_destroy(dcora_csr_t m);

int dcora_cert_dual_matrix(const dcora_dims *dims, const double *X, const int *rowptr, const int *colidx,
                           const double *vals, int device, dcora_csr_t *S);
int dcora_cert_is_psd(int k, const int *rowptr, const int *colidx, const double *vals, int block, int *is_psd);
int dcora_cert_is_psd_device(int k, const int *rowptr, const int *colidx, const double *vals, int block, int device,
                             int *is_psd, double *info8);
int dcora_chol_host_selftest(int k, const int *rowptr, const int *colidx, const double *vals, int block, int *is_pd,
                             double *resid, double *info4);
int dcora_chol_cache_clear(void);
int dcora_cert_min_eig(int k, const int *rowptr, const int *colidx, const double *vals, int max_iterations,
                       double min_eig_num_tol, int num_lanczos_vectors, unsigned long long seed, int device,
                       double *lambda_min, double *v, long *num_matvecs);
int dcora_cert_fast_verification(int k, const int *rowptr, const int *colidx, const double *vals, double eta,
                                 int block, int device, int *is_psd, double *theta, double *x, double *lambda_min);

int dcora_cert_suboptimality_gap(const dcora_dims *dims, const double *X, double lambda_lower_bound, double *gap,
                                 double *n_eff);
int dcora_cert_lambda_min_certified(int k, const int *rowptr, const int *colidx, const double *vals, double eta,
                                    int block, int max_iterations, double *lambda_min, int *iterations);

typedef struct dcora_dataset_s *dcora_dataset_t;
int dcora_dataset_load_g2o(const char *path, dcora_dataset_t *out);
int dcora_dataset_create(int d, int n, int m, const int *ids, const double *vals, dcora_dataset_t *out);
int dcora_dataset_info(dcora_dataset_t ds, int *d, int *n, int *m);
int dcora_dataset_copy(dcora_dataset_t ds, int *ids, double *vals);
int dcora_dataset_destroy(dcora_dataset_t ds);
int dcora_dataset_chordal_init(dcora_dataset_t ds, double *T);
int dcora_dataset_chordal_init_device(dcora_dataset_t ds, int device, double *T);
int dcora_graph_build_Q_pgo(int d, int n, int agent_id, int m, const int *ids, const double *vals, dcora_csr_t *Q);

typedef struct dcora_radataset_s *dcora_radataset_t;
int dcora_radataset_load_pyfg(const char *path, dcora_radataset_t *out);
int dcora_radataset_info(dcora_radataset_t ds, int *info);
int dcora_radataset_create(int d, int n, int l, int b, int m_pp, const int *pp_ids, const double *pp_vals, int m_pl,
                           const int *pl_ids, const double *pl_vals, int m_rg, const int *rg_ids, const double *rg_vals,
                           const double *gt, dcora_radataset_t *out);
int dcora_radataset_copy(dcora_radataset_t ds, int *pp_ids, double *pp_vals, int *pl_ids, double *pl_vals, int *rg_ids,
                         double *rg_vals);
int dcora_radataset_ground_truth(dcora_radataset_t ds, double *gt);
int dcora_radataset_build_Q(dcora_radataset_t ds, dcora_csr_t *Q);
int dcora_radataset_odometry_init(dcora_radataset_t ds, unsigned long long seed, double *X0);
int dcora_radataset_ownership(dcora_radataset_t ds, int *pose_robot, int *sphere_robot, int *landmark_robot);
int dcora_radataset_agent_columns(dcora_radataset_t ds, int robot, int *dims3, int *own, int *k_a);
int dcora_graph_extract_agent_blocks(int k, const int *rowptr, const int *colidx, const double *vals, int k_a,
                                     const int *own, dcora_csr_t *Qaa, dcora_csr_t *C);
int dcora_radataset_destroy(dcora_radataset_t ds);
int dcora_graph_precond_regularization(int k, const int *rowptr, const int *colidx, const double *vals, int device,
                                       double *reg);

typedef struct dcora_rbcd_s *dcora_rbcd_t;
typedef struct {
  int num_robots;
  int r;
  int acceleration;
  int restart_interval;
  dcora_ropt_params local;
  int rank, world_size;
  int device;
  void *stream;
} dcora_rbcd_options;
void dcora_rbcd_options_default(dcora_rbcd_options *o);

int dcora_rbcd_create(dcora_dataset_t ds, const dcora_rbcd_options *opt, dcora_rbcd_t *out);
int dcora_rbcd_destroy(dcora_rbcd_t s);
int dcora_rbcd_set_X(dcora_rbcd_t s, const double *X);
int dcora_rbcd_get_X(dcora_rbcd_t s, double *X);
int dcora_rbcd_iterate(dcora_rbcd_t s, int selected, double *cost2, double *gradnorm, double *block_norms,
                       int *next_selected);
// ... 121 lines not shown
```

Measured before the change: 4266.

## Fold RTR trial evaluation and accept/reject decision into the persistent tCG run kernel

The persistent tCG run kernel now also evaluates the trial point's gradient and cost partials, then does a grid-wide step and makes the trust-region accept/reject decision on-device. When this path is active the host skips its separate trial, evaluation and decide launches. This removes several kernel launches and their dependencies per RTR outer iteration. In exchange, sync words are double-buffered across runs, LDS use grows to fit the fused gradient, the kernel gets more arguments and coherent atomic loads, and fault-injection phases are added for testing.

```diff
diff --git a/dcora_amd/__init__.py b/dcora_amd/__init__.py
--- a/dcora_amd/__init__.py
+++ b/dcora_amd/__init__.py
@@ -323,7 +323,9 @@
 def _solver_info(self):
     info = np.zeros(2)
     check(capi.lib().dcora_problem_solver_info(self.h, info))
-    return {"tcg": {0: "three launches", 1: "two launches", 2: "one launch per run"}[int(info[0])]}
+    form = int(info[0])
+    return {"tcg": {0: "three launches", 1: "two launches", 2: "one launch per run"}[form],
+            "rtr": "one launch per iteration" if form == 2 else "launches"}
 
 
 QuadraticProblem.solver_info = _solver_info
diff --git a/dcora_amd/capi.py b/dcora_amd/capi.py
--- a/dcora_amd/capi.py
+++ b/dcora_amd/capi.py
@@ -165,6 +165,7 @@
     "dcora_cert_prepare": (C.c_int, [C.POINTER(Dims), _ip, _ip, C.c_int, C.c_int]),
     "dcora_debug_tcg_run_fault": (C.c_int, [C.c_int]),
     "dcora_debug_tcg_run_fault_at": (C.c_int, [C.c_int, C.c_int]),
+    "dcora_debug_tcg_run_fault_phase_at": (C.c_int, [C.c_int, C.c_int, C.c_int]),
     "dcora_problem_solver_info": (C.c_int, [_vp, _dp]),
     "dcora_ra_rbcd_create": (C.c_int, [_vp, C.POINTER(RbcdOptions), C.POINTER(_vp)]),
     "dcora_ra_rbcd_destroy": (C.c_int, [_vp]),
diff --git a/dcora_amd/csrc/capi.hip b/dcora_amd/csrc/capi.hip
--- a/dcora_amd/csrc/capi.hip
+++ b/dcora_amd/csrc/capi.hip
@@ -253,11 +253,15 @@
   return DCORA_OK;
 }
 int dcora_debug_tcg_run_fault(int runs) {
+  g_tcg_run_fault_phase.store(0);
   g_tcg_run_fault_skip.store(0);
   g_tcg_run_fault.store(runs < 0 ? 0 : runs);
   return DCORA_OK;
 }
-int dcora_debug_tcg_run_fault_at(int skip, int runs) {
+int dcora_debug_tcg_run_fault_at(int skip, int runs) { return dcora_debug_tcg_run_fault_phase_at(skip, runs, 0); }
+int dcora_debug_tcg_run_fault_phase_at(int skip, int runs, int phase) {
+  if (phase < 0 || phase > 2) return bad("phase: 0 tCG run, 1 evaluation, 2 decision");
+  g_tcg_run_fault_phase.store(phase);
   g_tcg_run_fault_skip.store(skip < 0 ? 0 : skip);
   g_tcg_run_fault.store(runs < 0 ? 0 : runs);
   return DCORA_OK;
diff --git a/dcora_amd/csrc/device_problem.hip b/dcora_amd/csrc/device_problem.hip
--- a/dcora_amd/csrc/device_problem.hip
+++ b/dcora_amd/csrc/device_problem.hip
@@ -253,8 +253,8 @@
     DCORA_HIP(hipGetDeviceProperties(&prop, device));
     tcg_run_ok = tcg_run_supported(m, ldm, prop.multiProcessorCount, tcg_run_max_rows_nnz(m, Qh.rp.data()));
     if (tcg_run_ok) {
-      DCORA_HIP(tcg_sync.alloc((size_t)tcg_run_sync_words()));
-      DCORA_HIP(hipMemsetAsync(tcg_sync.p, 0, sizeof(unsigned) * (size_t)tcg_run_sync_words(), st));
+      DCORA_HIP(tcg_sync.alloc(2 * (size_t)tcg_run_sync_words()));
+      DCORA_HIP(hipMemsetAsync(tcg_sync.p, 0, 2 * sizeof(unsigned) * (size_t)tcg_run_sync_words(), st));
     }
   }
   return DCORA_OK;
@@ -777,6 +777,9 @@
   const bool gf, gfb;
   unsigned *const sync_p;
   const int nsync;
+  int runs = 0;
+  int max_outer = 0;
+  bool run_decides = false;
   double *const dbuf[2];
   double *const rbuf[2];
 
@@ -790,7 +793,7 @@
         folded(sparse && p.sp.foldable()), sf(folded ? p.sp.fold() : SpFold{}), nsl(sparse ? 1 : -1),
         nZ(f == TcgForm::pc || f == TcgForm::run ? fused_pc_blocks(p.m) : nPB),
         gf(f != TcgForm::generic && !p.has_bsr && p.Q.n_long == 0), gfb(f != TcgForm::generic && p.has_bsr),
-        sync_p(f == TcgForm::run ? p.tcg_sync.p : nullptr), nsync(f == TcgForm::run ? tcg_run_sync_words() : 0),
+        sync_p(f == TcgForm::run ? p.tcg_sync.p : nullptr), nsync(f == TcgForm::run ? 2 * tcg_run_sync_words() : 0),
         dbuf{p.delta.p, p.delta2.p}, rbuf{p.res.p, p.res2.p} {}
 
   bool outer_done() const { return p.hf->outer_done_seq >= solve_first; }
@@ -816,7 +819,7 @@
     return p.enq_rgrad(p.Xb(), p.EGb(), p.RGb(), p.Sb(), sel, p.pB.p, g());
   }
 
-  int first() {
+  int first(int outer) {
     switch (form) {
       case TcgForm::generic: {
         launch_tcg_begin(p.st, N, p.RGb(), p.eta.p, p.Heta.p, p.res.p, c, ++seq);
@@ -826,7 +829,7 @@
         return s;
       }
       case TcgForm::run: {
-        const int s = launch_run();
+        const int s = launch_run(outer + 1 < max_outer);
         if (s != 0) return s;
         p.tcg_run_ok = false;
         form = TcgForm::pc;
@@ -846,7 +849,7 @@
     }
     return -1;
   }
-  int launch_run() {
+  int launch_run(bool decide) {
     hipEvent_t e1 = nullptr;
     if (p.profile_tcg_runs) {
       while (p.run_events.size() < p.run_events_used + 2) {
@@ -861,11 +864,16 @@
       e1 = p.run_events[p.run_events_used + 1];
       p.run_events_used += 2;
     }
+    const int words = tcg_run_sync_words();
+    unsigned *const mine = p.tcg_sync.p + (runs & 1) * words, *const next = p.tcg_sync.p + ((runs + 1) & 1) * words;
     if (launch_tcg_run(p.st, p.m, p.ldm, Mi, Qv, p.RGb(), p.Xb(), p.Sb(), dbuf[0], dbuf[1], p.Hd.p, p.eta.p, p.Heta.p,
-                       p.z.p, p.p1.p, p.p3.p, p.pC.p, p.tcg_sync.p, c, p.hf_dev, ++seq) < 0) {
+                       p.z.p, p.p1.p, p.p3.p, p.pC.p, Gp, p.EGb(), p.pA.p, p.pB.p, mine, next, c, p.hf_dev, ++seq,
+                       decide) < 0) {
       if (e1) p.run_events_used -= 2;
       return 0;
     }
+    ++runs;
+    run_decides = decide;
     if (e1) (void)hipEventRecord(e1, p.st);
     return seq;
   }
@@ -969,6 +977,7 @@
   }
   int &seq = seq_;
   RtrForm f(*this, form, seq);
+  f.max_outer = max_outer;
   CtlInit ci;
   ci.enable = 1;
   ci.tol = prm.gradnorm_tol;
@@ -994,7 +1003,7 @@
   launch_rtr_init(st, pA.p, f.nAe(), pB.p, nG, f.c, hf_dev, ++seq, ci, f.sync_p, f.nsync);
   int last_pace_seq = seq;
   std::vector<int> last_seq((size_t)std::max(1, max_inner));
-  int next_first_seq = time_is_up() ? 0 : f.first();
+  int next_first_seq = time_is_up() ? 0 : f.first(0);
   int last_run_seq = 0;
   for (int outer = 0; outer < max_outer || (f.form == TcgForm::run && last_run_seq > 0); ++outer) {
     const bool tail = outer >= max_outer;
@@ -1011,7 +1020,7 @@
       hf->tcg_abort_seq = 0;
       tcg_run_ok = false;
       f.form = TcgForm::pc;
-      next_first_seq = f.first();
+      next_first_seq = f.first(outer);
       if (next_first_seq < 0) return first_failed();
     }
     if (f.outer_done()) break;
@@ -1031,11 +1040,15 @@
       if (go == 0) break;
       last_seq[j] = seq;
     }
-    const int nR = f.trial();
-    nG = f.eval(1);
-    launch_rtr_decide(st, pA.p, f.nAe(), pB.p, nG, pC.p, nR, f.c, hf_dev, ++seq, f.sync_p, f.nsync);
-    last_pace_seq = seq;
-    if (outer + 1 < max_outer) next_first_seq = time_is_up() ? 0 : f.first();
+    if (f.form == TcgForm::run && f.run_decides) {
+      last_pace_seq = tcg_first_seq;
+    } else {
+      const int nR = f.trial();
+      nG = f.eval(1);
+      launch_rtr_decide(st, pA.p, f.nAe(), pB.p, nG, pC.p, nR, f.c, hf_dev, ++seq, f.sync_p, f.nsync);
+      last_pace_seq = seq;
+    }
+    if (outer + 1 < max_outer) next_first_seq = time_is_up() ? 0 : f.first(outer + 1);
   }
   pending_ = true;
   return DCORA_OK;
diff --git a/dcora_amd/csrc/kernels.h b/dcora_amd/csrc/kernels.h
--- a/dcora_amd/csrc/kernels.h
+++ b/dcora_amd/csrc/kernels.h
@@ -191,10 +191,12 @@
 int tcg_run_sync_words();
 extern std::atomic<int> g_tcg_run_fault;
 extern std::atomic<int> g_tcg_run_fault_skip;
+extern std::atomic<int> g_tcg_run_fault_phase;
 int tcg_run_max_rows_nnz(const ManiDesc &m, const int *rowptr);
 int launch_tcg_run(hipStream_t st, const ManiDesc &m, int ldm, const double *Minv, const CsrDev &Q, Buf2 grad, Buf2 X,
                    Buf2 S, double *d0, double *d1, double *Hd, double *eta, double *Heta, double *z, double *p1r,
-                   double *p3, double *pC, unsigned *sync, SolverCtl *ctl, HostFlags *hf, int seq);
+                   double *p3, double *pC, const double *G, Buf2 EG, double *pA, double *pB, unsigned *sync,
+                   unsigned *sync_next, SolverCtl *ctl, HostFlags *hf, int seq, bool decide);
 bool fused_pc_preferred(const ManiDesc &m, int ldm);
 bool fused_pc_ready(const ManiDesc &m, int ldm);
 int launch_fused_pc(hipStream_t st, const ManiDesc &m, int ldm, const double *Minv, Buf2 grad, Buf2 X,
diff --git a/dcora_amd/csrc/kernels.hip b/dcora_amd/csrc/kernels.hip
--- a/dcora_amd/csrc/kernels.hip
+++ b/dcora_amd/csrc/kernels.hip
@@ -2,31 +2,6 @@
 #include "tcg_rules.h"
 
 namespace dcora {
-
-template <int N>
-__device__ __forceinline__ void sum_partials_n(const double *const (&p)[N], const int (&np)[N], const int (&st)[N],
-                                               const int (&off)[N], double *sm, double (&out)[N]) {
-  double v[N];
-#pragma unroll
-  for (int q = 0; q < N; ++q) v[q] = ((int)threadIdx.x < np[q]) ? p[q][(size_t)threadIdx.x * st[q] + off[q]] : 0.0;
-#pragma unroll
-  for (int q = 0; q < N; ++q)
-    for (int i = threadIdx.x + blockDim.x; i < np[q]; i += blockDim.x) v[q] += p[q][(size_t)i * st[q] + off[q]];
-#pragma unroll
-  for (int q = 0; q < N; ++q) v[q] = wave_sum(v[q]);
-  const int w = threadIdx.x >> 6, nw = (blockDim.x + 63) >> 6;
-  __syncthreads();
-  if ((threadIdx.x & 63) == 0)
-#pragma unroll
-    for (int q = 0; q < N; ++q) sm[q * 4 + w] = v[q];
-  __syncthreads();
-#pragma unroll
-  for (int q = 0; q < N; ++q) {
-    double t = 0;
-    for (int i = 0; i < nw; ++i) t += sm[q * 4 + i];
-    out[q] = t;
-  }
-}
 
 int vec_grid(long nelem) {
   long g = (nelem + kBlock - 1) / kBlock;
@@ -1526,35 +1501,7 @@
   const int nps[5] = {npA, npA, npB, npC, npC}, sts[5] = {2, 2, 1, 2, 2}, offs[5] = {0, 1, 0, 0, 1};
   double sums[5];
   sum_partials_n<5>(ps, nps, sts, offs, s_red, sums);
-  const double fq = sums[0], fg = sums[1], g2 = sums[2], eg = sums[3], eh = sums[4];
-  if (threadIdx.x == 0) {
-    const double f2 = 0.5 * fq + fg;
-    const double rho = (ctl->f1 - f2) / (-(eg + 0.5 * eh));
-    ctl->f2 = f2;
-    ctl->rho = rho;
-    if (rho > 0.75) {
-      if (ctl->tcg_status == TR_NEGCURVTURE || ctl->tcg_status == TR_EXCREGION) ctl->Delta = fmin(2.0 * ctl->Delta, ctl->maxDelta);
-    } else if (rho < 0.25) {
-      ctl->Delta *= 0.25;
-    }
-    const bool accept = (rho > 0.1) && isfinite(rho);
-    if (accept) {
-      ctl->cur ^= 1;
-      ctl->f1 = f2;
-      ctl->ngf = sqrt(g2);
-      ctl->accepted += 1;
-      ctl->last_accepted = 1;
-    } else {
-      ctl->last_accepted = 0;
-      host_store(&hf->reject_seq, seq);
-    }
-    ctl->outer_it += 1;
-    if (ctl->ngf < ctl->tol || ctl->outer_it >= ctl->max_outer || (ctl->stop_on_accept && accept)) {
-      ctl->outer_done_stamp = seq;
-      host_store(&hf->outer_done_seq, seq);
-    }
-    host_store(&hf->last_seq_done, seq);
-  }
+  if (threadIdx.x == 0) rtr_decide(ctl, hf, seq, sums, ctl->tcg_status);
 }
 
 void launch_rtr_init(hipStream_t st, const double *pA, int npA, const double *pB, int npB, SolverCtl *ctl,
diff --git a/dcora_amd/csrc/solver_fused.hip b/dcora_amd/csrc/solver_fused.hip
--- a/dcora_amd/csrc/solver_fused.hip
+++ b/dcora_amd/csrc/solver_fused.hip
@@ -371,6 +371,124 @@
   if (threadIdx.x == 0) p1[blockIdx.x] = tot;
 }
 
+template <int D, bool Coh>
+__device__ __forceinline__ void fused_grad_block(const ManiDesc &m, const CsrDev &Q, const double *__restrict__ X,
+                                                 const double *__restrict__ G, double *__restrict__ EG,
+                                                 double *__restrict__ RG, double *__restrict__ Sblk,
+                                                 double *__restrict__ pA, double *__restrict__ pB,
+                                                 double *__restrict__ posenorm, int b, int *s_ci, double *s_v,
+                                                 double *s_W, double *s_X, double *s_red) {
+  const auto ldx = [](const double *q) {
+    if constexpr (Coh)
+      return __hip_atomic_load(q, __ATOMIC_RELAXED, __HIP_MEMORY_SCOPE_AGENT);
+    else
+      return *q;
+  };
+  constexpr int DH = D + 1;
+  const int r = m.r;
+  const int PB = fused_pb(r, DH);
+  const int pose0 = b * PB;
+  const int npose = min(PB, m.n - pose0);
+  const int j0 = pose0 * DH, ncol = npose * DH, nout = ncol * r;
+  const int e = threadIdx.x;
+  const bool act = e < nout;
+  const int lc = e / r, t = e - lc * r;
+  const int j = j0 + lc;
+  const int pbeg = Q.rp[j0], pend = Q.rp[j0 + ncol];
+  const int myb = act ? Q.rp[j] : 0, mye = act ? Q.rp[j + 1] : 0;
+  const size_t oown = (size_t)j * r + t;
+  const double x_own = act ? ldx(X + oown) : 0.0;
+  const double g_own = (act && G) ? G[oown] : 0.0;
+  double acc = 0;
+  for (int base = pbeg; base < pend; base += kHessTile) {
+    const int cnt = min(kHessTile, pend - base);
+    if (base != pbeg) __syncthreads();
+    {
+      constexpr int SU = kHessTile / kBlock;
+      int ci_r[SU];
+      double v_r[SU];
+      const int last = max(pend - 1, 0);
+#pragma unroll
+      for (int u = 0; u < SU; ++u) {
+        const int i = min(base + (int)threadIdx.x + u * kBlock, last);
+        ci_r[u] = Q.ci[i];
+        v_r[u] = Q.v[i];
+      }
+#pragma unroll
+      for (int u = 0; u < SU; ++u) {
+        const int i = threadIdx.x + u * kBlock;
+        if (i < cnt) {
+          s_ci[i] = ci_r[u];
+          s_v[i] = v_r[u];
+        }
+      }
+    }
+    __syncthreads();
+    const int lo = max(myb, base) - base, hi = min(mye, base + cnt) - base;
+    for (int p = lo; p < hi; p += 8) {
+      double b8[8], w8[8];
+#pragma unroll
+      for (int q = 0; q < 8; ++q) {
+        const bool ok = p + q < hi;
+        const size_t oo = ok ? (size_t)s_ci[p + q] * r + t : 0;
+        w8[q] = ok ? s_v[p + q] : 0.0;
+        b8[q] = ldx(X + oo);
+      }
+#pragma unroll
+      for (int q = 0; q < 8; ++q) acc += w8[q] * b8[q];
+    }
+  }
+  double d0 = 0, d1 = 0;
+  if (act) {
+    const double eg = acc + g_own;
+    EG[oown] = eg;
+    s_W[e] = eg;
+    s_X[e] = x_own;
+    d0 = acc * x_own;
+    d1 = x_own * g_own;
+  }
+  __syncthreads();
+  const int gp = threadIdx.x >> 3, tt = threadIdx.x & (GW - 1);
+  const bool pact = (gp < npose) && (tt < r);
+  const int pose = pose0 + gp;
+  const size_t o = (size_t)pose * DH * r;
+  Row<D> Y, E;
+#pragma unroll
+  for (int a = 0; a < DH; ++a) {
+    E.e[a] = pact ? s_W[(gp * DH + a) * r + tt] : 0.0;
+    Y.e[a] = pact ? s_X[(gp * DH + a) * r + tt] : 0.0;
+  }
+  double S[D][D];
+  grp_sym_gram<D>(Y, E, S);
+  if (Sblk && gp < npose && tt == 0)
+#pragma unroll
+    for (int a = 0; a < D; ++a)
+#pragma unroll
+      for (int c = 0; c < D; ++c) Sblk[(size_t)pose * D * D + a + c * D] = S[a][c];
+  row_sub_AS<D>(E, Y, S);
+  double pa = 0;
+#pragma unroll
+  for (int a = 0; a < DH; ++a) pa += E.e[a] * E.e[a];
+  if (posenorm) {
+    const double ps = grp_sum(pa);
+    if (gp < npose && tt == 0) posenorm[pose] = ps;
+  }
+  st_row<D>(RG + o, r, tt, pact, E);
+  const double t0 = block_sum(d0, s_red);
+  const double t1 = block_sum(d1, s_red);
+  const double t2 = block_sum(pact ? pa : 0.0, s_red);
+  if (threadIdx.x == 0) {
+    if constexpr (Coh) {
+      __hip_atomic_store(pA + 2 * b, t0, __ATOMIC_RELAXED, __HIP_MEMORY_SCOPE_AGENT);
+      __hip_atomic_store(pA + 2 * b + 1, t1, __ATOMIC_RELAXED, __HIP_MEMORY_SCOPE_AGENT);
+      __hip_atomic_store(pB + b, t2, __ATOMIC_RELAXED, __HIP_MEMORY_SCOPE_AGENT);
+    } else {
+      pA[2 * b] = t0;
+      pA[2 * b + 1] = t1;
+      pB[b] = t2;
+    }
+  }
+}
 template <int D>
 __global__ __launch_bounds__(kBlock) void k_fused_grad(ManiDesc m, CsrDev Q, Buf2 Xb, const double *__restrict__ G,
                                                        Buf2 EGb, Buf2 RGb, Buf2 Sb, int sel,
@@ -381,110 +499,11 @@
   __shared__ double s_v[kHessTile];
   __shared__ double s_W[kBlock], s_X[kBlock];
   __shared__ double s_red[16];
-  constexpr int DH = D + 1;
   const int idx = g.ctl ? ((g.ctl->cur ^ sel) & 1) : 0;
-  const double *__restrict__ X = Xb.p[idx];
-  double *__restrict__ EG = EGb.p[idx];
-  double *__restrict__ RG = RGb.p[idx];
-  double *__restrict__ Sblk = Sb.p[idx];
-  const int r = m.r;
-  const int PB = fused_pb(r, DH);
-  const int pose0 = blockIdx.x * PB;
-  const int npose = min(PB, m.n - pose0);
-  const int j0 = pose0 * DH, ncol = npose * DH, nout = ncol * r;
-  const int e = threadIdx.x;
-  const bool act = e < nout;
-  const int lc = e / r, t = e - lc * r;
-  const int j = j0 + lc;
-  const int pbeg = Q.rp[j0], pend = Q.rp[j0 + ncol];
-  const int myb = act ? Q.rp[j] : 0, mye = act ? Q.rp[j + 1] : 0;
-  const size_t oown = (size_t)j * r + t;
-  const double x_own = act ? X[oown] : 0.0;
-  const double g_own = (act && G) ? G[oown] : 0.0;
-  double acc = 0;
-  for (int base = pbeg; base < pend; base += kHessTile) {
-    const int cnt = min(kHessTile, pend - base);
-    if (base != pbeg) __syncthreads();
-    {
-      constexpr int SU = kHessTile / kBlock;
-      int ci_r[SU];
-      double v_r[SU];
-      const int last = max(pend - 1, 0);
-#pragma unroll
-      for (int u = 0; u < SU; ++u) {
-        const int i = min(base + (int)threadIdx.x + u * kBlock, last);
-        ci_r[u] = Q.ci[i];
-        v_r[u] = Q.v[i];
-      }
-#pragma unroll
-      for (int u = 0; u < SU; ++u) {
-        const int i = threadIdx.x + u * kBlock;
-        if (i < cnt) {
-          s_ci[i] = ci_r[u];
-          s_v[i] = v_r[u];
-        }
-      }
-    }
-    __syncthreads();
-    const int lo = max(myb, base) - base, hi = min(mye, base + cnt) - base;
-    for (int p = lo; p < hi; p += 8) {
-      double b8[8], w8[8];
-#pragma unroll
-      for (int q = 0; q < 8; ++q) {
-        const bool ok = p + q < hi;
-        const size_t oo = ok ? (size_t)s_ci[p + q] * r + t : 0;
-        w8[q] = ok ? s_v[p + q] : 0.0;
-        b8[q] = X[oo];
-      }
-#pragma unroll
-      for (int q = 0; q < 8; ++q) acc += w8[q] * b8[q];
-    }
-  }
-  double d0 = 0, d1 = 0;
-  if (act) {
-    const double eg = acc + g_own;
-    EG[oown] = eg;
-    s_W[e] = eg;
-    s_X[e] = x_own;
-    d0 = acc * x_own;
-    d1 = x_own * g_own;
-  }
-  __syncthreads();
-  const int gp = threadIdx.x >> 3, tt = threadIdx.x & (GW - 1);
-  const bool pact = (gp < npose) && (tt < r);
-  const int pose = pose0 + gp;
-  const size_t o = (size_t)pose * DH * r;
-  Row<D> Y, E;
-#pragma unroll
-  for (int a = 0; a < DH; ++a) {
-    E.e[a] = pact ? s_W[(gp * DH + a) * r + tt] : 0.0;
-    Y.e[a] = pact ? s_X[(gp * DH + a) * r + tt] : 0.0;
-  }
-  double S[D][D];
-  grp_sym_gram<D>(Y, E, S);
-  if (Sblk && gp < npose && tt == 0)
-#pragma unroll
-    for (int a = 0; a < D; ++a)
-#pragma unroll
-      for (int b = 0; b < D; ++b) Sblk[(size_t)pose * D * D + a + b * D] = S[a][b];
-  row_sub_AS<D>(E, Y, S);
-  double pa = 0;
-#pragma unroll
-  for (int a = 0; a < DH; ++a) pa += E.e[a] * E.e[a];
-  if (posenorm) {
-    const double ps = grp_sum(pa);
-    if (gp < npose && tt == 0) posenorm[pose] = ps;
-  }
-  st_row<D>(RG + o, r, tt, pact, E);
-  const double t0 = block_sum(d0, s_red);
-  const double t1 = block_sum(d1, s_red);
-  const double t2 = block_sum(pact ? pa : 0.0, s_red);
-  if (threadIdx.x == 0) {
-    pA[2 * blockIdx.x] = t0;
-    pA[2 * blockIdx.x + 1] = t1;
-    pB[blockIdx.x] = t2;
-  }
-}
+  fused_grad_block<D, false>(m, Q, Xb.p[idx], G, EGb.p[idx], RGb.p[idx], Sb.p[idx], pA, pB, posenorm, blockIdx.x, s_ci,
+                             s_v, s_W, s_X, s_red);
+}
+constexpr size_t kFusedGradLds = kHessTile * (sizeof(int) + sizeof(double)) + 2 * kBlock * sizeof(double);
 
 template <int D>
 __global__ __launch_bounds__(kBlock) void k_fused_hess_bsr(ManiDesc m, BsrDev A, const double *__restrict__ z,
@@ -1209,16 +1228,21 @@
   CsrDev Q;
   Buf2 grad, X, S;
   double *d0, *d1, *Hd, *eta, *Heta, *z, *p1r, *p3, *pC;
-  unsigned *sync;
+  const double *G;
+  Buf2 EG;
+  double *pA, *pB;
+  unsigned *sync, *sync_next;
   SolverCtl *ctl;
   HostFlags *hf;
   int seq, pbA;
+  int decide;
   int fault;
 #ifdef DCORA_RUN_STAMPS
   long long *stamps;
 #endif
 };
 #ifdef DCORA_RUN_STAMPS
+constexpr int kRunStampTail = 60;
 #define RUN_STAMP(i)                                                            \
   do {                                                                          \
     if (a.stamps && blockIdx.x == 0 && threadIdx.x == 0 && (i) < 64) a.stamps[(i)] = wall_clock64(); \
@@ -1302,7 +1326,7 @@
   extern __shared__ double s_res[];
   __shared__ double s_P[NR * RM + 1][4 * kPcNW];
   __shared__ double s_Z[NR * RM + 1], s_R[NR * RM], s_W[NR * RM], s_D[NR * RM], s_H[NR * RM];
-  __shared__ double s_red[16];
+  __shared__ double s_red[20];
   __shared__ int s_ci[kRunQCap];
   __shared__ double s_v[kRunQCap];
   __shared__ int s_ok;
@@ -1311,6 +1335,8 @@
   RUN_STAMP(0);
   const int st_o = ctl->outer_done_stamp, cur = ctl->cur & 1;
   if (seq > st_o) return;
+  if (blockIdx.x == 0)
+    for (int i = threadIdx.x; i < kRunSyncWords; i += kPcBlock) a.sync_next[i] = 0u;
   const double c_Delta = ctl->Delta, c_ngf = ctl->ngf;
   const int c_max_inner = ctl->max_inner;
   const ManiDesc m = a.m;
@@ -1433,18 +1459,19 @@
       if (lane == 0) st_coh(a.p3 + blockIdx.x, tot);
     }
   };
+  auto end_run = [&]() {
+    ctl->alpha = alpha;
+    ctl->e_Pe_n = ePen;
+    ctl->norm_r0 = n0;
+    ctl->z_r[0] = ctl->z_r[1] = zr;
+    ctl->d_Pd[0] = ctl->d_Pd[1] = dPd;
+    ctl->e_Pe[0] = ctl->e_Pe[1] = ePe;
+    ctl->e_Pd[0] = ctl->e_Pd[1] = ePd;
+    tcg_end_run(ctl, a.hf, seq, status, iters_done);
+    if (!a.decide) host_store(&a.hf->last_seq_done, seq);
+  };
   auto finish = [&]() {
-    if (blockIdx.x == 0 && threadIdx.x == 0) {
-      ctl->alpha = alpha;
-      ctl->e_Pe_n = ePen;
-      ctl->norm_r0 = n0;
-      ctl->z_r[0] = ctl->z_r[1] = zr;
-      ctl->d_Pd[0] = ctl->d_Pd[1] = dPd;
-      ctl->e_Pe[0] = ctl->e_Pe[1] = ePe;
-      ctl->e_Pd[0] = ctl->e_Pd[1] = ePd;
-      tcg_end_run(ctl, a.hf, seq, status, iters_done);
-      host_store(&a.hf->last_seq_done, seq);
-    }
+    if (!a.decide && blockIdx.x == 0 && threadIdx.x == 0) end_run();
     __syncthreads();
     double a0 = 0, a1 = 0;
     if (own) {
@@ -1461,13 +1488,15 @@
 #pragma unroll
       for (int aa = 0; aa < DH; ++aa) Yn.e[aa] += 1.0 * (pact ? s_R[(g * DH + aa) * RM + tt] : 0.0);
       row_qf<D>(Yn);
-      st_row<D>(a.X.p[cur ^ 1] + o, r, tt, pact, Yn);
+      if (pact)
+#pragma unroll
+        for (int aa = 0; aa < DH; ++aa) st_coh(a.X.p[cur ^ 1] + o + aa * r + tt, Yn.e[aa]);
     }
     const double t0 = block_sum(a0, s_red);
     const double t1 = block_sum(a1, s_red);
     if (threadIdx.x == 0) {
-      a.pC[2 * blockIdx.x] = t0;
-      a.pC[2 * blockIdx.x + 1] = t1;
+      st_coh(a.pC + 2 * blockIdx.x, t0);
+      st_coh(a.pC + 2 * blockIdx.x + 1, t1);
     }
   };
   auto give_up = [&]() {
@@ -1493,183 +1522,207 @@
   product();
   project_z();
   RUN_STAMP(2);
-  if (c_max_inner <= 0) {
-    status = TR_MAXITER;
-    finish();
-    return;
-  }
-  if (a.fault && blockIdx.x == 0) return;
+  if (c_max_inner > 0) {
+    if (a.fault == 1 && blockIdx.x == 0) return;
+    if (!run_grid_step(a.sync, gstep++, &s_ok)) return give_up();
+    RUN_STAMP(3);
+    for (int iter = 0;; ++iter) {
+      const int par = iter & 1;
+      double *__restrict__ d_new = par ? a.d1 : a.d0;
+      const double *__restrict__ d_old = par ? a.d0 : a.d1;
+      {
+        constexpr int kRunGB = 24;
+        double ga[kRunGB], gz[kRunGB];
+        double z_own = 0;
+        if (own) {
+          z_own = ld_coh(a.z + oown);
+#pragma unroll
+          for (int q = 0; q < kRunGB; ++q) {
+            const bool ok = myb + q < mye;
+            const size_t oo = ok ? (size_t)s_ci[myb + q] * r + t : 0;
+            gz[q] = ld_coh(a.z + oo);
+            ga[q] = (iter > 0) ? ld_coh(d_old + oo) : 0.0;
+          }
+        }
+        const int np3 = gridDim.x;
+        const int l = lane;
+        const double pa = (l < np3) ? ld_coh(a.p3 + l) : 0.0, pb = (l + 64 < np3) ? ld_coh(a.p3 + l + 64) : 0.0;
+        const double pcc = (l + 128 < np3) ? ld_coh(a.p3 + l + 128) : 0.0, pd = (l + 192 < np3) ? ld_coh(a.p3 + l + 192) : 0.0;
+        const double z_r_new = wave_sum((pa + pb) + (pcc + pd));
+        double beta = 0;
+        if (iter > 0) beta = tcg_beta(z_r_new, zr);
+        const TcgDir dir = iter == 0 ? tcg_dir_start(z_r_new) : tcg_dir_next(z_r_new, beta, alpha, dPd, ePd);
+        zr = dir.z_r;
+        ePd = dir.e_Pd;
+        dPd = dir.d_Pd;
+        ePe = iter == 0 ? 0.0 : ePen;
+        double accw = 0, dn = 0;
+        if (own) {
+#pragma unroll
+          for (int q = 0; q < kRunGB; ++q) {
+            const double w = (myb + q < mye) ? s_v[myb + q] : 0.0;
+            accw += w * (beta * ga[q] - gz[q]);
+          }
+          for (int p = myb + kRunGB; p < mye; p += 8) {
+            double a8[8], b8[8], w8[8];
+#pragma unroll
+            for (int q = 0; q < 8; ++q) {
+              const bool ok = p + q < mye;
+              const size_t oo = ok ? (size_t)s_ci[p + q] * r + t : 0;
+              w8[q] = ok ? s_v[p + q] : 0.0;
+              b8[q] = ld_coh(a.z + oo);
+              a8[q] = (iter > 0) ? ld_coh(d_old + oo) : 0.0;
+            }
+#pragma unroll
+            for (int q = 0; q < 8; ++q) accw += w8[q] * (beta * a8[q] - b8[q]);
+          }
+          dn = (iter > 0) ? beta * o_d - z_own : -z_own;
+          st_coh(d_new + oown, dn);
+          o_d = dn;
+          s_W[e] = accw;
+          s_D[e] = dn;
+        }
+        __syncthreads();
+        if (wave == 0) {
+          Row<D> V, W;
+#pragma unroll
+          for (int aa = 0; aa < DH; ++aa) {
+            W.e[aa] = pact ? s_W[(g * DH + aa) * r + tt] : 0.0;
+            V.e[aa] = pact ? s_D[(g * DH + aa) * r + tt] : 0.0;
+          }
+          row_sub_AS<D>(W, V, S);
+          row_tangent<D>(Y, W);
+          if (pact)
+#pragma unroll
+            for (int aa = 0; aa < DH; ++aa) {
+              st_coh(a.Hd + o + aa * r + tt, W.e[aa]);
+              s_H[(g * DH + aa) * r + tt] = W.e[aa];
+            }
+          double dacc = 0;
+#pragma unroll
+          for (int aa = 0; aa < DH; ++aa) dacc += V.e[aa] * W.e[aa];
+          if (!pact) dacc = 0;
+          const double rs = row16_sum_dpp(dacc);
+          if (lane == 0) st_coh(a.p1r + blockIdx.x, rs);
+        }
+        __syncthreads();
+        if (own) o_h = s_H[e];
+      }
+      RUN_STAMP(4 + 7 * iter);
+      if (!run_grid_step(a.sync, gstep++, &s_ok)) return give_up();
+      RUN_STAMP(5 + 7 * iter);
+      double2 xh[kPcSB];
+#pragma unroll
+      for (int u = 0; u < kPcSB; ++u) xh[u] = pc_ld16_coh(rs_h, voff_t, (unsigned)u * kPcBlock * 16u);
+      double d_Hd;
+      {
+        const int rows_per = a.pbA / 2, nrows = gridDim.x, nblk = (nrows + rows_per - 1) / rows_per;
+        double part = 0;
+        if (lane < nblk) {
+          const int b0 = lane * rows_per;
+          double wsum[4] = {0, 0, 0, 0};
+#pragma unroll
+          for (int w = 0; w < 4; ++w) {
+            double rs4[4];
+#pragma unroll
+            for (int q = 0; q < 4; ++q) {
+              const int ri = w * 4 + q;
+              rs4[q] = (ri < rows_per && b0 + ri < nrows) ? ld_coh(a.p1r + b0 + ri) : 0.0;
+            }
+            wsum[w] = (rs4[0] + rs4[1]) + (rs4[2] + rs4[3]);
+          }
+          double tsum = 0;
+#pragma unroll
+          for (int w = 0; w < 4; ++w) tsum += wsum[w];
+          part = tsum;
+        }
+        d_Hd = wave_sum(part);
+      }
+      const double c_zr = zr, c_dPd = dPd, c_ePe = ePe, c_ePd = ePd;
+      alpha = tcg_alpha(c_zr, d_Hd);
+      const double e_Pe_new = tcg_e_Pe_new(alpha, c_dPd, c_ePe, c_ePd);
+      const bool boundary = tcg_boundary(d_Hd, e_Pe_new, c_Delta);
+      const double step = boundary ? tcg_tau(c_dPd, c_ePe, c_ePd, c_Delta) : alpha;
+      ePen = e_Pe_new;
+      if (own) {
+        o_eta = o_eta + step * o_d;
+        o_Heta = o_Heta + step * o_h;
+      }
+      if (boundary) {
+        status = tcg_boundary_status(d_Hd);
+        iters_done = iter + 1;
+        break;
+      }
+      if (own) {
+        const double rr = fma(alpha, o_h, o_r);
+        o_r = rr;
+        s_R[lc * RM + t] = rr;
+      }
+      RUN_STAMP(6 + 7 * iter);
+      nrm2 = 0;
+#pragma unroll
+      for (int u = 0; u < kPcSB; ++u) {
+        const int i = u * kPcBlock + (int)threadIdx.x;
+        if (i < npair) {
+          double2 x = reinterpret_cast<double2 *>(s_res)[i];
+          x.x = fma(alpha, xh[u].x, x.x);
+          x.y = fma(alpha, xh[u].y, x.y);
+          nrm2 = fma(x.x, x.x, nrm2);
+          nrm2 = fma(x.y, x.y, nrm2);
+          reinterpret_cast<double2 *>(s_res)[i] = x;
+        }
+      }
+      __syncthreads();
+      RUN_STAMP(7 + 7 * iter);
+      product();
+      RUN_STAMP(8 + 7 * iter);
+      {
+        if (tcg_residual_done(sqrt(s_Z[NR * RM]), n0)) {
+          status = tcg_residual_status(n0);
+          iters_done = iter + 1;
+          break;
+        }
+      }
+      project_z();
+      if (iter + 1 >= c_max_inner) {
+        iters_done = iter + 1;
+        break;
+      }
+      RUN_STAMP(9 + 7 * iter);
+      if (!run_grid_step(a.sync, gstep++, &s_ok)) return give_up();
+      RUN_STAMP(10 + 7 * iter);
+    }
+  }
+  finish();
+  if (!a.decide) return;
+  RUN_STAMP(kRunStampTail);
+  if (a.fault == 2 && blockIdx.x == 0) return;
   if (!run_grid_step(a.sync, gstep++, &s_ok)) return give_up();
-  RUN_STAMP(3);
-  for (int iter = 0;; ++iter) {
-    const int par = iter & 1;
-    double *__restrict__ d_new = par ? a.d1 : a.d0;
-    const double *__restrict__ d_old = par ? a.d0 : a.d1;
-    {
-      constexpr int kRunGB = 24;
-      double ga[kRunGB], gz[kRunGB];
-      double z_own = 0;
-      if (own) {
-        z_own = ld_coh(a.z + oown);
-#pragma unroll
-        for (int q = 0; q < kRunGB; ++q) {
-          const bool ok = myb + q < mye;
-          const size_t oo = ok ? (size_t)s_ci[myb + q] * r + t : 0;
-          gz[q] = ld_coh(a.z + oo);
-          ga[q] = (iter > 0) ? ld_coh(d_old + oo) : 0.0;
-        }
-      }
-      const int np3 = gridDim.x;
-      const int l = lane;
-      const double pa = (l < np3) ? ld_coh(a.p3 + l) : 0.0, pb = (l + 64 < np3) ? ld_coh(a.p3 + l + 64) : 0.0;
-      const double pcc = (l + 128 < np3) ? ld_coh(a.p3 + l + 128) : 0.0, pd = (l + 192 < np3) ? ld_coh(a.p3 + l + 192) : 0.0;
-      const double z_r_new = wave_sum((pa + pb) + (pcc + pd));
-      double beta = 0;
-      if (iter > 0) beta = tcg_beta(z_r_new, zr);
-      const TcgDir dir = iter == 0 ? tcg_dir_start(z_r_new) : tcg_dir_next(z_r_new, beta, alpha, dPd, ePd);
-      zr = dir.z_r;
-      ePd = dir.e_Pd;
-      dPd = dir.d_Pd;
-      ePe = iter == 0 ? 0.0 : ePen;
-      double accw = 0, dn = 0;
-      if (own) {
-#pragma unroll
-        for (int q = 0; q < kRunGB; ++q) {
-          const double w = (myb + q < mye) ? s_v[myb + q] : 0.0;
-          accw += w * (beta * ga[q] - gz[q]);
-        }
-        for (int p = myb + kRunGB; p < mye; p += 8) {
-          double a8[8], b8[8], w8[8];
-#pragma unroll
-          for (int q = 0; q < 8; ++q) {
-            const bool ok = p + q < mye;
-            const size_t oo = ok ? (size_t)s_ci[p + q] * r + t : 0;
-            w8[q] = ok ? s_v[p + q] : 0.0;
-            b8[q] = ld_coh(a.z + oo);
-            a8[q] = (iter > 0) ? ld_coh(d_old + oo) : 0.0;
-          }
-#pragma unroll
-          for (int q = 0; q < 8; ++q) accw += w8[q] * (beta * a8[q] - b8[q]);
-        }
-        dn = (iter > 0) ? beta * o_d - z_own : -z_own;
-        st_coh(d_new + oown, dn);
-        o_d = dn;
-        s_W[e] = accw;
-        s_D[e] = dn;
-      }
-      __syncthreads();
-      if (wave == 0) {
-        Row<D> V, W;
-#pragma unroll
-        for (int aa = 0; aa < DH; ++aa) {
-          W.e[aa] = pact ? s_W[(g * DH + aa) * r + tt] : 0.0;
-          V.e[aa] = pact ? s_D[(g * DH + aa) * r + tt] : 0.0;
-        }
-        row_sub_AS<D>(W, V, S);
-        row_tangent<D>(Y, W);
-        if (pact)
-#pragma unroll
-          for (int aa = 0; aa < DH; ++aa) {
-            st_coh(a.Hd + o + aa * r + tt, W.e[aa]);
-            s_H[(g * DH + aa) * r + tt] = W.e[aa];
-          }
-        double dacc = 0;
-#pragma unroll
-        for (int aa = 0; aa < DH; ++aa) dacc += V.e[aa] * W.e[aa];
-        if (!pact) dacc = 0;
-        const double rs = row16_sum_dpp(dacc);
-        if (lane == 0) st_coh(a.p1r + blockIdx.x, rs);
-      }
-      __syncthreads();
-      if (own) o_h = s_H[e];
-    }
-    RUN_STAMP(4 + 7 * iter);
-    if (!run_grid_step(a.sync, gstep++, &s_ok)) return give_up();
-    RUN_STAMP(5 + 7 * iter);
-    double2 xh[kPcSB];
-#pragma unroll
-    for (int u = 0; u < kPcSB; ++u) xh[u] = pc_ld16_coh(rs_h, voff_t, (unsigned)u * kPcBlock * 16u);
-    double d_Hd;
-    {
-      const int rows_per = a.pbA / 2, nrows = gridDim.x, nblk = (nrows + rows_per - 1) / rows_per;
-      double part = 0;
-      if (lane < nblk) {
-        const int b0 = lane * rows_per;
-        double wsum[4] = {0, 0, 0, 0};
-#pragma unroll
-        for (int w = 0; w < 4; ++w) {
-          double rs4[4];
-#pragma unroll
-          for (int q = 0; q < 4; ++q) {
-            const int ri = w * 4 + q;
-            rs4[q] = (ri < rows_per && b0 + ri < nrows) ? ld_coh(a.p1r + b0 + ri) : 0.0;
-          }
-          wsum[w] = (rs4[0] + rs4[1]) + (rs4[2] + rs4[3]);
-        }
-        double tsum = 0;
-#pragma unroll
-        for (int w = 0; w < 4; ++w) tsum += wsum[w];
-        part = tsum;
-      }
-      d_Hd = wave_sum(part);
-    }
-    const double c_zr = zr, c_dPd = dPd, c_ePe = ePe, c_ePd = ePd;
-    alpha = tcg_alpha(c_zr, d_Hd);
-    const double e_Pe_new = tcg_e_Pe_new(alpha, c_dPd, c_ePe, c_ePd);
-    const bool boundary = tcg_boundary(d_Hd, e_Pe_new, c_Delta);
-    const double step = boundary ? tcg_tau(c_dPd, c_ePe, c_ePd, c_Delta) : alpha;
-    ePen = e_Pe_new;
-    if (own) {
-      o_eta = o_eta + step * o_d;
-      o_Heta = o_Heta + step * o_h;
-    }
-    if (boundary) {
-      status = tcg_boundary_status(d_Hd);
-      iters_done = iter + 1;
-      finish();
-      return;
-    }
-    if (own) {
-      const double rr = fma(alpha, o_h, o_r);
-      o_r = rr;
-      s_R[lc * RM + t] = rr;
-    }
-    RUN_STAMP(6 + 7 * iter);
-    nrm2 = 0;
-#pragma unroll
-    for (int u = 0; u < kPcSB; ++u) {
-      const int i = u * kPcBlock + (int)threadIdx.x;
-      if (i < npair) {
-        double2 x = reinterpret_cast<double2 *>(s_res)[i];
-        x.x = fma(alpha, xh[u].x, x.x);
-        x.y = fma(alpha, xh[u].y, x.y);
-        nrm2 = fma(x.x, x.x, nrm2);
-        nrm2 = fma(x.y, x.y, nrm2);
-        reinterpret_cast<double2 *>(s_res)[i] = x;
-      }
-    }
-    __syncthreads();
-    RUN_STAMP(7 + 7 * iter);
-    product();
-    RUN_STAMP(8 + 7 * iter);
-    {
-      if (tcg_residual_done(sqrt(s_Z[NR * RM]), n0)) {
-        status = tcg_residual_status(n0);
-        iters_done = iter + 1;
-        finish();
-        return;
-      }
-    }
-    project_z();
-    if (iter + 1 >= c_max_inner) {
-      iters_done = iter + 1;
-      finish();
-      return;
-    }
-    RUN_STAMP(9 + 7 * iter);
-    if (!run_grid_step(a.sync, gstep++, &s_ok)) return give_up();
-    RUN_STAMP(10 + 7 * iter);
-  }
+  RUN_STAMP(kRunStampTail + 1);
+  const int nG = (m.n + a.pbA - 1) / a.pbA;
+  if ((int)blockIdx.x < nG) {
+    char *const lds = reinterpret_cast<char *>(s_res);
+    fused_grad_block<D, true>(m, a.Q, a.X.p[cur ^ 1], a.G, a.EG.p[cur ^ 1], a.grad.p[cur ^ 1], a.S.p[cur ^ 1], a.pA,
+                              a.pB, nullptr, blockIdx.x, reinterpret_cast<int *>(lds),
+                              reinterpret_cast<double *>(lds + kHessTile * sizeof(int)),
+                              reinterpret_cast<double *>(lds + kHessTile * (sizeof(int) + sizeof(double))),
+                              reinterpret_cast<double *>(lds + kHessTile * (sizeof(int) + sizeof(double)) +
+                                                         kBlock * sizeof(double)),
+                              s_red);
+  }
+  RUN_STAMP(kRunStampTail + 2);
+  if (a.fault == 3 && blockIdx.x == 0) return;
+  if (!run_grid_step(a.sync, gstep++, &s_ok)) return give_up();
+  if (blockIdx.x != 0) return;
+  const double *const ps[5] = {a.pA, a.pA, a.pB, a.pC, a.pC};
+  const int nps[5] = {nG, nG, nG, (int)gridDim.x, (int)gridDim.x}, sts[5] = {2, 2, 1, 2, 2}, offs[5] = {0, 1, 0, 0, 1};
+  double sums[5];
+  sum_partials_n<5, true>(ps, nps, sts, offs, s_red, sums);
+  if (threadIdx.x == 0) {
+    end_run();
+    rtr_decide(ctl, a.hf, seq, sums, status);
+  }
+  RUN_STAMP(kRunStampTail + 3);
 }
 
 
@@ -2356,6 +2409,7 @@
 int tcg_run_sync_words() { return kRunSyncWords; }
 std::atomic<int> g_tcg_run_fault{0};
 std::atomic<int> g_tcg_run_fault_skip{0};
+std::atomic<int> g_tcg_run_fault_phase{0};
 int tcg_run_max_rows_nnz(const ManiDesc &m, const int *rp) {
   const int dh = m.d + 1;
   int worst = 0;
@@ -2392,7 +2446,7 @@
     tried.fetch_or(bit, std::memory_order_release);
   }
   const int cpad = ((a.m.k + 127) / 128) * 128;
-  const size_t lds = (size_t)cpad * R * sizeof(double);
+  const size_t lds = std::max((size_t)cpad * R * sizeof(double), kFusedGradLds);
   if (!(ok.load(std::memory_order_acquire) & bit) && lds > 40 * 1024) return -1;
   const int grid = (a.m.n + 1) / 2;
   hipLaunchKernelGGL((k_tcg_run<3, R, kRunNS>), dim3(grid), dim3(kPcBlock), lds, st, a);
@@ -2401,7 +2455,8 @@
 }
 int launch_tcg_run(hipStream_t st, const ManiDesc &m, int ldm, const double *Minv, const CsrDev &Q, Buf2 grad, Buf2 X,
                    Buf2 S, double *d0, double *d1, double *Hd, double *eta, double *Heta, double *z, double *p1r,
-                   double *p3, double *pC, unsigned *sync, SolverCtl *ctl, HostFlags *hf, int seq) {
+                   double *p3, double *pC, const double *G, Buf2 EG, double *pA, double *pB, unsigned *sync,
+                   unsigned *sync_next, SolverCtl *ctl, HostFlags *hf, int seq, bool decide) {
   int fault = 0;
   bool skipped = false;
   for (int sk = g_tcg_run_fault_skip.load(); sk > 0;)
@@ -2411,11 +2466,11 @@
     }
   for (int left = skipped ? 0 : g_tcg_run_fault.load(); left > 0;)
     if (g_tcg_run_fault.compare_exchange_weak(left, left - 1)) {
-      fault = 1;
+      fault = 1 + std::min(std::max(g_tcg_run_fault_phase.load(), 0), 2);
       break;
     }
-  TcgRunArgs a{m, ldm, Minv, Q, grad, X, S, d0, d1, Hd, eta, Heta, z, p1r, p3, pC, sync, ctl, hf, seq,
-               fused_pb(m.r, m.d + 1), fault};
+  TcgRunArgs a{m,  ldm, Minv,   Q,   grad, X,         S,   d0, d1, Hd, eta, Heta, z, p1r, p3, pC, G, EG, pA,
+               pB, sync, sync_next, ctl, hf, seq, fused_pb(m.r, m.d + 1), decide ? 1 : 0, fault};
 #ifdef DCORA_RUN_STAMPS
   {
     static long long *buf = nullptr;
@@ -2429,11 +2484,19 @@
         for (int i = 0; i < 40; ++i) acc[i] += (double)(buf[i] - s0) * 0.01;
         ++n;
       }
+      static double tail[3];
+      static int nt = 0;
+      if (buf[kRunStampTail + 3] > buf[kRunStampTail] && buf[kRunStampTail] > 0) {
+        for (int i = 0; i < 3; ++i) tail[i] += (double)(buf[kRunStampTail + 1 + i] - buf[kRunStampTail + i]) * 0.01;
+        ++nt;
+      }
       for (int i = 0; i < 64; ++i) buf[i] = 0;
       if (n == 500) {
         fprintf(stderr, "k_tcg_run stamps (us from start, workgroup 0, mean of %d runs with >= 4 iterations):", n);
         for (int i = 0; i < 34; ++i) fprintf(stderr, " %.2f", acc[i] / n);
         fprintf(stderr, "\n");
+        fprintf(stderr, "k_tcg_run RTR boundary (us, workgroup 0, mean of %d launches): grid step %.2f, evaluation %.2f, "
+                "grid step + decision %.2f\n", nt, tail[0] / nt, tail[1] / nt, tail[2] / nt);
         n = -1000000;
       }
     }
diff --git a/dcora_amd/csrc/tcg_rules.h b/dcora_amd/csrc/tcg_rules.h
--- a/dcora_amd/csrc/tcg_rules.h
+++ b/dcora_amd/csrc/tcg_rules.h
@@ -76,4 +76,65 @@
   c->max_inner = ci.max_inner;
 }
 
+template <int N, bool Coh = false>
+__device__ __forceinline__ void sum_partials_n(const double *const (&p)[N], const int (&np)[N], const int (&st)[N],
+                                               const int (&off)[N], double *sm, double (&out)[N]) {
+  const auto ld = [](const double *a) {
+    if constexpr (Coh)
+      return __hip_atomic_load(a, __ATOMIC_RELAXED, __HIP_MEMORY_SCOPE_AGENT);
+    else
+      return *a;
+  };
+  double v[N];
+#pragma unroll
+  for (int q = 0; q < N; ++q) v[q] = ((int)threadIdx.x < np[q]) ? ld(p[q] + (size_t)threadIdx.x * st[q] + off[q]) : 0.0;
+#pragma unroll
+  for (int q = 0; q < N; ++q)
+    for (int i = threadIdx.x + blockDim.x; i < np[q]; i += blockDim.x) v[q] += ld(p[q] + (size_t)i * st[q] + off[q]);
+#pragma unroll
+  for (int q = 0; q < N; ++q) v[q] = wave_sum(v[q]);
+  const int w = threadIdx.x >> 6, nw = (blockDim.x + 63) >> 6;
+  __syncthreads();
+  if ((threadIdx.x & 63) == 0)
+#pragma unroll
+    for (int q = 0; q < N; ++q) sm[q * 4 + w] = v[q];
+  __syncthreads();
+#pragma unroll
+  for (int q = 0; q < N; ++q) {
+    double t = 0;
+    for (int i = 0; i < nw; ++i) t += sm[q * 4 + i];
+    out[q] = t;
+  }
 }
+__device__ __forceinline__ void rtr_decide(SolverCtl *ctl, HostFlags *hf, int seq, const double (&sums)[5],
+                                           int tcg_status) {
+  const double fq = sums[0], fg = sums[1], g2 = sums[2], eg = sums[3], eh = sums[4];
+  const double f2 = 0.5 * fq + fg;
+  const double rho = (ctl->f1 - f2) / (-(eg + 0.5 * eh));
+  ctl->f2 = f2;
+  ctl->rho = rho;
+  if (rho > 0.75) {
+    if (tcg_status == TR_NEGCURVTURE || tcg_status == TR_EXCREGION) ctl->Delta = fmin(2.0 * ctl->Delta, ctl->maxDelta);
+  } else if (rho < 0.25) {
+    ctl->Delta *= 0.25;
+  }
+  const bool accept = (rho > 0.1) && isfinite(rho);
+  if (accept) {
+    ctl->cur ^= 1;
+    ctl->f1 = f2;
+    ctl->ngf = sqrt(g2);
+    ctl->accepted += 1;
+    ctl->last_accepted = 1;
+  } else {
+    ctl->last_accepted = 0;
+    host_store(&hf->reject_seq, seq);
+  }
+  ctl->outer_it += 1;
+  if (ctl->ngf < ctl->tol || ctl->outer_it >= ctl->max_outer || (ctl->stop_on_accept && accept)) {
+    ctl->outer_done_stamp = seq;
+    host_store(&hf->outer_done_seq, seq);
+  }
+  host_store(&hf->last_seq_done, seq);
+}
+
+}
diff --git a/include/dcora_hip.h b/include/dcora_hip.h
--- a/include/dcora_hip.h
+++ b/include/dcora_hip.h
@@ -69,6 +69,7 @@
 int dcora_problem_solver_info(dcora_problem_t p, double *info);
 int dcora_debug_tcg_run_fault(int runs);
 int dcora_debug_tcg_run_fault_at(int skip, int runs);
+int dcora_debug_tcg_run_fault_phase_at(int skip, int runs, int phase);
 int dcora_problem_precondition(dcora_problem_t p, const double *X, const double *V, double *out);
 int dcora_problem_retract(dcora_problem_t p, const double *X, const double *V, double *out);
 int dcora_problem_tangent_project(dcora_problem_t p, const double *X, const double *V, double *out);
```

Result: no change. 4287 (median of 6 runs) (+0.5%).
